# zju3dv/Mirror-NeRF

Hardware: AMD Instinct MI355X
Metric: rendered rays/sec (primary+reflected) (higher is better)
Workload: dtype f32 carried as hi/lo f16 pairs (f16 MFMA, f32 accumulate; max |diff| to the fp32 chain 3e-6)

## Files before the change

### include/mnrf.h

```cpp
#ifndef MNRF_H
#define MNRF_H

#include <stdint.h>

#ifdef __cplusplus
extern "C" {
#endif

#define MNRF_HOST

#define MNRF_OK 0
#define MNRF_ERR_ARG (-1)
#define MNRF_ERR_LAUNCH (-2)
#define MNRF_ERR_UNSUPPORTED (-3)

#define MNRF_N_PARAMS 32

#define MNRF_SIGMA_ONLY 1u
#define MNRF_GRAD_NORMAL 2u
#define MNRF_SPLIT_F16 4u

#define MNRF_TCNN_GRAD_F16 16u
#define MNRF_TCNN_GRAD_FIXED 512u
#define MNRF_TCNN_F16 256u
// ... 69 lines not shown
int mnrf_object_rays(const float* rays, int64_t n_rays, MNRF_HOST const float* pose, float scale, float tx, float ty, float tz,
                     float* out, void* stream);

int mnrf_object_merge(const float* obj_rgb, const float* obj_depth, const float* obj_opacity, int64_t n_rays, float scale,
                      float pose_scale0, float near, float* rgb, float* depth, float* mask, int32_t* n_used, void* stream);

#define MNRF_OBJECT_MAX_RES 1024

int mnrf_occupancy_bits(const float* volume, int Rx, int Ry, int Rz, float sigma_min, int dilate, uint32_t* bits,
                        int32_t* n_set, void* stream);

int mnrf_object_cull(const float* rays, int64_t n_rays, MNRF_HOST const float* pose, float scale, float tx, float ty, float tz,
                     MNRF_HOST const float* box_lo, MNRF_HOST const float* box_hi, int Rx, int Ry, int Rz, const uint32_t* bits,
                     float* out_rays, int32_t* index, int32_t* count, void* stream);

int mnrf_object_merge_indexed(const float* obj_rgb, const float* obj_depth, const float* obj_opacity, const int32_t* index,
                              const int32_t* count, int64_t capacity, float scale, float pose_scale0, float near, float* rgb,
                              float* depth, float* mask, int32_t* n_used, void* stream);

int mnrf_composite_backward(const float* rays, int64_t n_rays, int S, const float* sigma, const float* z_vals,
                            const float* noise, const float* rgb, const float* is_mirror,
                            const float* pred_normal, const float* normal, int white_back,
                            const float* weights, const float* depth,
                            const float* g_weights, const float* g_opacity, const float* g_rgb_map,
                            const float* g_depth, const float* g_mirror_mask, const float* g_surf_normal,
                            const float* g_surf_normal_grad, const float* g_normal_dif, const float* g_x_surface,
                            float* d_sigma, float* d_rgb, float* d_is_mirror, float* d_pred_normal,
                            float* d_normal, float* d_rays,
                            int detach ,
                            const float* keep_mirror ,
                            void* stream);

int mnrf_ray_grads(const float* d_xyz, const float* z_vals, const float* d_dir, int64_t n_rays, int spr, float* g_rays,
                   float* g_de, void* stream);

int mnrf_reflect_backward(const float* rays, const float* normal, const int32_t* index, int64_t n_sec,
                          const float* g_sec, int64_t n_rays, float* g_x_surface, float* g_normal, float* g_rays,
                          void* stream);
int mnrf_blend_backward(const float* g_out, const float* mask, const int32_t* index, int64_t n_sec, int64_t n, int c,
                        float* g_base, float* g_sec, void* stream);
int mnrf_embed_backward(const float* x, const float* g_out, int64_t n, int c, int n_freqs, float* g_x, void* stream);

int64_t mnrf_train_save_floats(int64_t B);
int64_t mnrf_train_mask_words(int64_t B);
int64_t mnrf_train_workspace_floats(int64_t B);

int mnrf_field_forward_train(float* packed, int64_t B, const float* xyz, int64_t xyz_stride,
                             const float* rays, const float* z_vals, int spr, const float* dir_emb,
                             int64_t dir_stride, float* sigma, float* rgb, float* pred_normal,
                             float* is_mirror, float* normal, float* save_x, uint64_t* save_mask,
                             float* save_inv, float* save_invj, unsigned flags , void* stream);

int mnrf_field_backward(float* packed, int64_t B, const float* xyz, int64_t xyz_stride,
                        const float* rays, const float* z_vals, int spr,
                        const float* g_sigma, const float* g_rgb, const float* g_pred_normal,
                        const float* g_is_mirror, const float* rgb, const float* pred_normal,
                        const float* is_mirror, const float* save_x, const uint64_t* save_mask,
                        const float* save_inv, float* workspace, float* const* d_params, float* d_xyz,
                        float* d_dir,
                        const float* keep_mirror ,
                        unsigned flags ,
                        void* stream);

int64_t mnrf_train_workspace2_floats(int64_t B);
int mnrf_field_backward2(float* packed, int64_t B, const float* xyz, int64_t xyz_stride,
                         const float* rays, const float* z_vals, int spr, const float* g_normal,
                         const float* normal, const float* save_invj, const uint64_t* save_mask,
                         float* workspace, float* const* d_params, float* d_xyz, unsigned flags , void* stream);

int mnrf_tcnn_encode(const float* table, MNRF_HOST const int64_t* offsets17_host, double log2_per_level_scale, int base_resolution,
                     float bound, int64_t B, const float* xyz, int64_t xyz_stride, const float* rays, const float* z_vals,
                     int spr, float* planes, void* stream);

int mnrf_tcnn_encode_flags(const float* table, MNRF_HOST const int64_t* offsets17_host, double log2_per_level_scale, int base_resolution,
                           float bound, int64_t B, const float* xyz, int64_t xyz_stride, const float* rays, const float* z_vals,
                           int spr, float* planes, unsigned flags, void* stream);
int mnrf_tcnn_table_half(const float* table, int64_t entries, void* table_half, void* stream);

int mnrf_bench_gather(const void* table, int64_t table_bytes, int bytes_per_gather, int64_t n_threads, int iters, float* out,
                      void* stream);

#define MNRF_FUSED_WHITE_BACK 1u
#define MNRF_FUSED_RGB_DEPTH 2u
int mnrf_fused_samples_per_ray(void);
int mnrf_field_composite_fused(float* packed, int64_t n_rays, const float* rays, const float* z_vals,
                               const float* dir_emb, int64_t dir_stride, int flags,
                               float* weights, float* opacity, float* rgb_map, float* depth, float* mirror_mask,
                               float* surf_normal, float* x_surface, void* stream);

#define MNRF_TRAIN_PLANES 256u
#define MNRF_PLANES_Y_HALF 0x100000u
int64_t mnrf_train_planes_bytes(int64_t B);
int64_t mnrf_train_dy_planes_bytes(int64_t B);

int mnrf_field_backward_planes(float* packed, int64_t B, const float* xyz, int64_t xyz_stride,
                               const float* rays, const float* z_vals, int spr,
                               const float* g_sigma, const float* g_rgb, const float* g_pred_normal,
                               const float* g_is_mirror, const float* rgb, const float* pred_normal,
                               const float* is_mirror, const uint64_t* save_mask, const float* save_inv,
                               void* dy_planes, uint32_t* seedmax, float* d_xyz, float* d_dir, const float* keep_mirror,
                               unsigned flags ,
                               void* stream);

int64_t mnrf_dw_planes_workspace_floats(int n_eval, MNRF_HOST const int64_t* B);
int mnrf_dw_planes(int n_eval, const void* const* x_planes, const void* const* dy_planes, MNRF_HOST const int64_t* B,
                   const uint32_t* const* seedmax, float* workspace, float* const* d_params, int accumulate, void* stream);

int64_t mnrf_train_planes2_bytes(int64_t B);
int64_t mnrf_train_dy_planes2_bytes(int64_t B);
int mnrf_field_backward2_planes(float* packed, int64_t B, const float* xyz, int64_t xyz_stride,
                                const float* rays, const float* z_vals, int spr, const float* g_normal,
                                const float* normal, const float* save_invj, const uint64_t* save_mask,
                                void* x2_planes, void* y2_planes, uint32_t* jmax, float* d_xyz, void* stream);
int64_t mnrf_dw_planes2_workspace_floats(int n_eval, MNRF_HOST const int64_t* B, MNRF_HOST const int* kinds);
int mnrf_dw_planes2(int n_eval, const void* const* x_planes, const void* const* dy_planes, MNRF_HOST const int64_t* B,
                    const uint32_t* const* seedmax, MNRF_HOST const int* kinds, float* workspace, float* const* d_params, int accumulate,
                    void* stream);

int mnrf_adam_step(float* param, const float* grad, float* exp_avg, float* exp_avg_sq, int64_t n, float lr, double beta1,
                   double beta2, float eps, float weight_decay, int64_t step, int32_t* skipped, const float* grad_scale,
                   const float* found_inf, void* stream);

int mnrf_embed_n(const float* x, int64_t n, int c, int n_freqs, float* out, const int32_t* n_live, void* stream);
int mnrf_embed_backward_n(const float* x, const float* g_out, int64_t n, int c, int n_freqs, float* g_x, const int32_t* n_live, void* stream);
int mnrf_sample_coarse_n(const float* rays, int64_t n_rays, const float* z_steps, int n_samples, int use_disp, float perturb,
                         const float* perturb_rand, float* z_vals, const int32_t* n_live, void* stream);
int mnrf_ray_prologue_n(const float* rays, int64_t n_rays, int n_freqs_dir, const float* z_steps, int n_samples, int use_disp,
                        float perturb, const float* perturb_rand, float* dir_emb, float* z_vals, const int32_t* n_live, void* stream);
int mnrf_ray_fan_backward_n(const float* g0, const float* g1, const float* g2, const float* g3, const float* rays,
                            const float* g_dir_a, const float* g_dir_b, int64_t n_rays, int n_freqs_dir, float* g_rays,
                            const int32_t* n_live, void* stream);
int mnrf_composite_n(const float* rays, int64_t n_rays, int S, const float* sigma, const float* z_vals,
                     const float* noise, const float* rgb, const float* is_mirror,
                     const float* pred_normal, const float* normal, int white_back,
                     float* weights, float* opacity, float* rgb_map, float* depth, float* mirror_mask,
                     float* surf_normal, float* surf_normal_grad, float* normal_dif, float* x_surface,
                     const int32_t* n_live, void* stream);
int mnrf_composite_sample_n(const float* rays, int64_t n_rays, int S, const float* sigma, const float* z_vals,
                            const float* noise, const float* rgb, const float* is_mirror,
                            const float* pred_normal, const float* normal, int white_back,
                            float* weights, float* opacity, float* rgb_map, float* depth, float* mirror_mask,
                            float* surf_normal, float* surf_normal_grad, float* normal_dif, float* x_surface,
                            const float* u, int u_per_ray, int n_importance, float* z_fine,
                            const int32_t* n_live, void* stream);
int mnrf_composite_backward_n(const float* rays, int64_t n_rays, int S, const float* sigma, const float* z_vals,
                              const float* noise, const float* rgb, const float* is_mirror,
                              const float* pred_normal, const float* normal, int white_back,
                              const float* weights, const float* depth,
                              const float* g_weights, const float* g_opacity, const float* g_rgb_map,
                              const float* g_depth, const float* g_mirror_mask, const float* g_surf_normal,
                              const float* g_surf_normal_grad, const float* g_normal_dif, const float* g_x_surface,
                              float* d_sigma, float* d_rgb, float* d_is_mirror, float* d_pred_normal,
                              float* d_normal, float* d_rays, int detach, const float* keep_mirror,
                              const int32_t* n_live, void* stream);
int mnrf_sample_fine_n(const float* z_coarse, const float* weights, int64_t n_rays, int S,
                       const float* u, int u_per_ray, int n_importance, float* z_fine, const int32_t* n_live, void* stream);
int mnrf_threshold_mask_n(float* mask, int64_t n, int32_t* any, const int32_t* n_live, void* stream);
int mnrf_reflect_compact_n(const float* rays, const float* x_surface, const float* normal,
                           const float* normal_noise, float noise_std, const float* mask,
                           int64_t n_rays, int compact, float near2, float* sec_rays, int32_t* index,
                           int32_t* count, float* reflect_dir, const int32_t* n_live,
                           int32_t* slot ,
                           void* stream);
int mnrf_reflect_backward_gather_n(const float* rays, const float* normal, const int32_t* slot, const float* g_sec, int64_t n_rays,
                                   float* g_x_surface, float* g_normal, float* g_rays, const int32_t* n_live, void* stream);
int mnrf_blend2_n(const float* base_a, const float* sec_a, const float* base_b, const float* sec_b, const int32_t* slot,
                  const float* mask, int64_t n, int c, float* out_a, float* out_b, const int32_t* n_live, void* stream);
int mnrf_blend2_backward_n(const float* g_out_a, const float* g_out_b, const int32_t* slot, const float* mask, int64_t n, int c,
                           float* g_base_a, float* g_sec_a, float* g_base_b, float* g_sec_b, const int32_t* n_live, void* stream);
int mnrf_blend_scatter_n(const float* base, const float* sec, const int32_t* index, int64_t n_sec,
                         const float* mask, int64_t n, int c, float* out, float* reflect_out,
// ... 218 lines not shown
```

### mirror_nerf_amd/csrc/mnrf_composite.inc

```
struct CompMaps {
    float* weights;
    float* opacity; float* rgb_map; float* depth; float* mirror_mask;
    float* surf_normal; float* surf_normal_grad; float* normal_dif; float* x_surface;
    const float* rays;
    int white_back;
};

template <class Src>
__device__ __forceinline__ void composite_ray(const Src& src, int S, int lane, long long ray, const CompMaps& A) {
    float carry = 1.f;
    float a_op = 0.f, a_d = 0.f, a_m = 0.f, a_nd = 0.f;
    float a_c[3] = {0.f, 0.f, 0.f}, a_n[3] = {0.f, 0.f, 0.f}, a_g[3] = {0.f, 0.f, 0.f};
    for (int base = 0; base < S; base += 64) {
        const int s = base + lane;
        const bool in = s < S;
        float alpha = 0.f, zv = 0.f;
        if (in) {
            zv = src.z(s);
            const float delta = s + 1 < S ? src.z(s + 1) - zv : 1e10f;
            float sv = src.sigma(s);
            if (src.has_noise()) sv = sv + src.noise(s);
            alpha = 1.f - expf(-delta * fmaxf(sv, 0.f));
        }
        const float t = in ? (1.f - alpha) + 1e-10f : 1.f;
        float incl = t;
#pragma unroll
        for (int o = 1; o < 64; o <<= 1) {
            const float up = __shfl_up(incl, o);
            if (lane >= o) incl *= up;
        }
        float excl = __shfl_up(incl, 1);
        if (lane == 0) excl = 1.f;
        const float w = alpha * (carry * excl);
        carry = carry * __shfl(incl, 63);
        if (in) {
            if (A.weights) A.weights[s] = w;
            a_op += w;
            a_d += w * zv;
            if (src.has_rgb()) { a_c[0] += w * src.rgb(s, 0); a_c[1] += w * src.rgb(s, 1); a_c[2] += w * src.rgb(s, 2); }
            if (src.has_mirror()) a_m += w * src.mirror(s);
            float pn[3] = {0.f, 0.f, 0.f}, gn[3] = {0.f, 0.f, 0.f};
            if (src.has_pn()) {
#pragma unroll
                for (int k = 0; k < 3; ++k) { pn[k] = src.pn(s, k); a_n[k] += pn[k] * w; }
            }
            if (src.has_gn()) {
#pragma unroll
                for (int k = 0; k < 3; ++k) { gn[k] = src.gn(s, k); a_g[k] += gn[k] * w; }
            }
            if (src.has_pn() && src.has_gn()) {
                const float d0 = gn[0] - pn[0], d1 = gn[1] - pn[1], d2 = gn[2] - pn[2];
                a_nd += w * (d0 * d0 + d1 * d1 + d2 * d2);
            }
        }
    }
    a_op = wave_sum(a_op);
    a_d = wave_sum(a_d);
    if (src.has_mirror()) a_m = wave_sum(a_m);
    if (src.has_pn() && src.has_gn()) a_nd = wave_sum(a_nd);
#pragma unroll
    for (int k = 0; k < 3; ++k) {
        if (src.has_rgb()) a_c[k] = wave_sum(a_c[k]);
        if (src.has_pn()) a_n[k] = wave_sum(a_n[k]);
        if (src.has_gn()) a_g[k] = wave_sum(a_g[k]);
    }
    if (lane == 0) {
        if (A.opacity) A.opacity[ray] = a_op;
        if (A.rgb_map) {
#pragma unroll
            for (int k = 0; k < 3; ++k) A.rgb_map[ray * 3 + k] = A.white_back ? a_c[k] + (1.f - a_op) : a_c[k];
        }
        if (A.depth) A.depth[ray] = a_d;
        if (A.mirror_mask) A.mirror_mask[ray] = a_m;
        if (A.surf_normal) { for (int k = 0; k < 3; ++k) A.surf_normal[ray * 3 + k] = a_n[k]; }
        if (A.surf_normal_grad) { for (int k = 0; k < 3; ++k) A.surf_normal_grad[ray * 3 + k] = a_g[k]; }
        if (A.normal_dif) A.normal_dif[ray] = a_nd;
        if (A.x_surface) {
            const float* r = A.rays + ray * 8;
            for (int k = 0; k < 3; ++k) A.x_surface[ray * 3 + k] = r[k] + r[3 + k] * a_d;
        }
    }
}
```

### mirror_nerf_amd/csrc/mnrf_field.hip

```cpp
#include <hip/hip_runtime.h>
#include <stdint.h>
#include <stdlib.h>

#include "mnrf_layout.h"
#include "mnrf_field_args.h"

namespace mnrf {

extern __shared__ __attribute__((aligned(16))) char smem[];

namespace s2 {
constexpr int S = 2;
constexpr int MIN_WAVES_PER_SIMD = 1;
constexpr int CHUNK_TILES = 16;
#include "mnrf_field_impl.inc"
#include "mnrf_field_bwd.inc"
}
namespace s1 {
constexpr int S = 1;
constexpr int MIN_WAVES_PER_SIMD = 2;
constexpr int CHUNK_TILES = 16;
#include "mnrf_field_impl.inc"
}

struct PackArgs {
    const float* params[32];
    float* packed;
};
constexpr int PACK_BATCH = 4;
struct PackBatch {
    PackArgs m[PACK_BATCH];
};

__global__ void pack_kernel(PackBatch PB, PartTable T) {
    const PackArgs& P = PB.m[blockIdx.y];
    const long long p = (long long)blockIdx.x * blockDim.x + threadIdx.x;
    if (p < DEVICE_STATE_WORDS) P.packed[OFF_REDUCE_PAIR + p] = 0.f;
    if (p >= PACKED_F32_FLOATS) return;
    float v = 0.f;
    if (p < OFF_BIAS) {
        const int tile = (int)(p / TILE_FLOATS);
        const int within = (int)(p % TILE_FLOATS);
        const int lane = within >> 2, j = within & 3, g = lane >> 4, i = lane & 15;
        int k = 0;
        while (k + 1 < N_FWD_PARTS && T.fwd[k + 1].tile0 <= tile) ++k;
        const Part pt = T.fwd[k];
        const int lt = tile - pt.tile0;
        const int tq = lt / pt.nb, nb = lt % pt.nb;
        const int n = 16 * nb + i;
        const int t = 4 * tq + j;
        int col;
        if (pt.kind == KIND_ENC) col = enc_col(t, g);
        else {
            col = 16 * (t >> 2) + 4 * g + (t & 3);
            if (pt.kind == KIND_DIR && col >= ENC_DIR) col = -1;
        }
        if (tq < pt.ntq && n < pt.n_true && col >= 0) v = P.params[pt.param][(long long)n * pt.ld + pt.col_off + col];
    } else if (p < OFF_BWD) {
        const int b = (int)(p - OFF_BIAS);
        if (b < 2048) v = P.params[2 * (b / 256) + 1][b % 256];
        else if (b < BIAS_FIN) { if (b - BIAS_SIG < 1) v = P.params[21][0]; }
        else if (b < BIAS_DIR) v = P.params[17][b - BIAS_FIN];
        else if (b < BIAS_RGB) v = P.params[19][b - BIAS_DIR];
        else if (b < BIAS_NRM1) { if (b - BIAS_RGB < 3) v = P.params[23][b - BIAS_RGB]; }
        else if (b < BIAS_NRM2) v = P.params[25][b - BIAS_NRM1];
        else if (b < BIAS_MIR1) { if (b - BIAS_NRM2 < 3) v = P.params[27][b - BIAS_NRM2]; }
        else if (b < BIAS_MIR2) v = P.params[29][b - BIAS_MIR1];
        else if (b < BIAS_WSIG) { if (b - BIAS_MIR2 < 1) v = P.params[31][0]; }
        else if (b < BIAS_WSIG + 256) v = P.params[20][b - BIAS_WSIG];
    } else {
        const bool heads = p >= OFF_HBWD;
        const long long q = p - (heads ? OFF_HBWD : OFF_BWD);
        const int tile = (int)(q / TILE_FLOATS);
        const int within = (int)(q % TILE_FLOATS);
        const int lane = within >> 2, j = within & 3, g = lane >> 4, i = lane & 15;
        const Part* parts = heads ? T.hbwd : T.bwd;
        const int nparts = heads ? N_HBWD_PARTS - 1 : N_BWD_PARTS;
        int k = 0;
        while (k + 1 < nparts && parts[k + 1].tile0 <= tile) ++k;
        const Part pt = parts[k];
        const int lt = tile - pt.tile0;
        const int tq = lt / pt.nb, nb = lt % pt.nb;
        const int rho = 16 * nb + i;
        const int c = 16 * tq + 4 * g + j;
// ... 15 lines not shown

#include "../../include/mnrf.h"
#include "mnrf_dw.h"
#include "mnrf_error.h"
#include "mnrf_fill.h"

using namespace mnrf;

extern "C" int64_t mnrf_packed_floats(void) { return PACKED_FLOATS; }

extern "C" int mnrf_pack_weights_n(int n_models, const float* const* params, float* const* packed, void* stream) {
    if (n_models < 0) return mnrf_fail(MNRF_ERR_ARG, "mnrf_pack_weights_n: negative model count");
    if (n_models == 0) return MNRF_OK;
    if (!params || !packed) return mnrf_fail(MNRF_ERR_ARG, "mnrf_pack_weights: null pointer");
    for (int i = 0; i < n_models * MNRF_N_PARAMS; ++i)
        if (!params[i]) return mnrf_fail(MNRF_ERR_ARG, "mnrf_pack_weights: null parameter pointer");
    for (int m = 0; m < n_models; ++m)
        if (!packed[m]) return mnrf_fail(MNRF_ERR_ARG, "mnrf_pack_weights: null image pointer");
    PartTable T;
    build_parts(T);
    const int threads = 256;
    const int blocks = (int)((PACKED_F32_FLOATS + threads - 1) / threads);
    for (int m0 = 0; m0 < n_models; m0 += PACK_BATCH) {
        const int nb = n_models - m0 < PACK_BATCH ? n_models - m0 : PACK_BATCH;
        PackBatch PB{};
        float* images[PACK_BATCH] = {};
        for (int m = 0; m < nb; ++m) {
            for (int i = 0; i < MNRF_N_PARAMS; ++i) PB.m[m].params[i] = params[(m0 + m) * MNRF_N_PARAMS + i];
            PB.m[m].packed = images[m] = packed[m0 + m];
        }
        hipLaunchKernelGGL(pack_kernel, dim3(blocks, nb), dim3(threads), 0, (hipStream_t)stream, PB, T);
        launch_split_pack(images, nb, (hipStream_t)stream);
    }
    return mnrf_check_launch("mnrf_pack_weights");
}

extern "C" int mnrf_fold_weights_n(int n_models, const float* const* params, float* const* packed, void* stream) {
    if (n_models < 0) return mnrf_fail(MNRF_ERR_ARG, "mnrf_fold_weights_n: negative model count");
    if (n_models == 0) return MNRF_OK;
    if (!params || !packed) return mnrf_fail(MNRF_ERR_ARG, "mnrf_fold_weights_n: null pointer");
    for (int i = 0; i < n_models * MNRF_N_PARAMS; ++i)
        if (!params[i]) return mnrf_fail(MNRF_ERR_ARG, "mnrf_fold_weights_n: null parameter pointer");
    for (int m = 0; m < n_models; ++m)
        if (!packed[m]) return mnrf_fail(MNRF_ERR_ARG, "mnrf_fold_weights_n: null image pointer");
    for (int m0 = 0; m0 < n_models; m0 += PACK_BATCH) {
        const int nb = n_models - m0 < PACK_BATCH ? n_models - m0 : PACK_BATCH;
        launch_split_fold(params + m0 * MNRF_N_PARAMS, packed + m0, nb, (hipStream_t)stream);
    }
    return mnrf_check_launch("mnrf_fold_weights");
}

extern "C" int mnrf_pack_weights(const float* const* params, float* packed, void* stream) {
    if (!params || !packed) return mnrf_fail(MNRF_ERR_ARG, "mnrf_pack_weights: null pointer");
    return mnrf_pack_weights_n(1, params, &packed, stream);
}

extern "C" int mnrf_field_forward(float* packed, unsigned flags, int64_t B, const float* xyz,
                                  int64_t xyz_stride, const float* rays, const float* z_vals, int spr,
                                  const float* dir_emb, int64_t dir_stride, float* sigma, float* rgb,
                                  float* pred_normal, float* is_mirror, float* normal, float* geo_feat,
                                  void* stream) {
    if (!packed) return mnrf_fail(MNRF_ERR_ARG, "mnrf_field_forward: packed weights are null");
    if (B < 0) return mnrf_fail(MNRF_ERR_ARG, "mnrf_field_forward: negative sample count");
    if (B == 0) return MNRF_OK;
    const bool sigma_only = flags & MNRF_SIGMA_ONLY;
    const bool grad = flags & MNRF_GRAD_NORMAL;
    if (!xyz && (!rays || !z_vals)) return mnrf_fail(MNRF_ERR_ARG, "mnrf_field_forward: need xyz or rays+z_vals");
    if (xyz && xyz_stride < 3) return mnrf_fail(MNRF_ERR_ARG, "mnrf_field_forward: xyz_stride < 3");
    if (spr < 1) return mnrf_fail(MNRF_ERR_ARG, "mnrf_field_forward: samples per ray must be >= 1");
    if (!xyz && B % spr != 0) return mnrf_fail(MNRF_ERR_ARG, "mnrf_field_forward: B not a multiple of spr");
    if (!sigma_only && !dir_emb) return mnrf_fail(MNRF_ERR_ARG, "mnrf_field_forward: dir_emb required unless SIGMA_ONLY");
    if (grad && !normal) return mnrf_fail(MNRF_ERR_ARG, "mnrf_field_forward: GRAD_NORMAL needs the normal output");
    FieldArgs A{packed, flags, (long long)B, xyz, (long long)xyz_stride, rays, z_vals, spr, dir_emb,
                (long long)dir_stride, sigma, rgb, pred_normal, is_mirror, normal, geo_feat};
    const int rc = (flags & MNRF_SPLIT_F16) ? launch_split(A, sigma_only, grad, (hipStream_t)stream)
                 : grad ? s1::launch(A, sigma_only, grad, (hipStream_t)stream)
                        : s2::launch(A, sigma_only, grad, (hipStream_t)stream);
    if (rc != 0) return mnrf_fail(MNRF_ERR_ARG, "mnrf_field_forward: too many samples for one launch");
    return mnrf_check_launch("mnrf_field_forward");
}

extern "C" int mnrf_fused_samples_per_ray(void) { return split48_ray_samples(); }

extern "C" int mnrf_field_composite_fused(float* packed, int64_t n_rays, const float* rays, const float* z_vals,
                                          const float* dir_emb, int64_t dir_stride, int flags,
                                          float* weights, float* opacity, float* rgb_map, float* depth, float* mirror_mask,
                                          float* surf_normal, float* x_surface, void* stream) {
    if (!packed || !rays || !z_vals || !dir_emb) return mnrf_fail(MNRF_ERR_ARG, "mnrf_field_composite_fused: null pointer");
    if (n_rays < 0) return mnrf_fail(MNRF_ERR_ARG, "mnrf_field_composite_fused: negative ray count");
    if (flags & ~(int)(MNRF_FUSED_WHITE_BACK | MNRF_FUSED_RGB_DEPTH)) return mnrf_fail(MNRF_ERR_ARG, "mnrf_field_composite_fused: unknown flag bits");
    const bool rgb_depth = flags & MNRF_FUSED_RGB_DEPTH;
    if (rgb_depth && (mirror_mask || surf_normal))
        return mnrf_fail(MNRF_ERR_ARG, "mnrf_field_composite_fused: MNRF_FUSED_RGB_DEPTH evaluates neither the mirror head nor the normal map");
    if (n_rays == 0) return MNRF_OK;
    if (!split48_enabled())
        return mnrf_fail(MNRF_ERR_UNSUPPORTED, "mnrf_field_composite_fused: needs the 48-samples-per-wave tuning (MNRF_SPLIT48 != 0)");
    const int spr = split48_ray_samples();
    FieldArgs A{packed, MNRF_SPLIT_F16, (long long)n_rays * spr, nullptr, 3, rays, z_vals, spr, dir_emb, (long long)dir_stride,
                nullptr, nullptr, nullptr, nullptr, nullptr, nullptr};
    A.fuse = rgb_depth ? 2 : 1;
    A.white_back = (flags & MNRF_FUSED_WHITE_BACK) != 0;
    A.f_weights = weights; A.f_opacity = opacity; A.f_rgb_map = rgb_map; A.f_depth = depth; A.f_mirror_mask = mirror_mask;
    A.f_surf_normal = surf_normal; A.f_x_surface = x_surface;
    if (launch_split48(A, false, (hipStream_t)stream) != 0)
        return mnrf_fail(MNRF_ERR_ARG, "mnrf_field_composite_fused: too many samples for one launch");
    return mnrf_check_launch("mnrf_field_composite_fused");
}

static inline int64_t train_tiles(int64_t B) { return (B + s2::WG_SAMPLES - 1) / s2::WG_SAMPLES; }

extern "C" int64_t mnrf_train_save_floats(int64_t B) { return (int64_t)SAVE_FLOATS * B; }
extern "C" int64_t mnrf_train_mask_words(int64_t B) { return train_tiles(B) * N_MASKS * s2::S * s2::WG_THREADS; }
extern "C" int64_t mnrf_train_workspace_floats(int64_t B) { return (int64_t)DY_FLOATS * B + dw_workspace_floats(B); }

static int field_forward_train_impl(float* packed, int64_t B, const float* xyz, int64_t xyz_stride,
                                    const float* rays, const float* z_vals, int spr, const float* dir_emb,
                                    int64_t dir_stride, float* sigma, float* rgb, float* pred_normal,
                                    float* is_mirror, float* normal, float* save_x, uint64_t* save_mask,
                                    float* save_inv, float* save_invj, unsigned flags, const int32_t* n_live, void* stream) {
    if (n_live && !(flags & MNRF_TRAIN_PLANES))
        return mnrf_fail(MNRF_ERR_UNSUPPORTED, "mnrf_field_forward_train_n: a live row count needs MNRF_TRAIN_PLANES (the fp32-row layout depends on B)");
    if (!packed || !save_x || !save_mask || !save_inv) return mnrf_fail(MNRF_ERR_ARG, "mnrf_field_forward_train: null pointer");
    const bool planes = flags & MNRF_TRAIN_PLANES;
    if (planes && !(flags & MNRF_SPLIT_F16))
        return mnrf_fail(MNRF_ERR_ARG, "mnrf_field_forward_train: MNRF_TRAIN_PLANES needs MNRF_SPLIT_F16 (the planes are the split kernel's operands)");
    if (B <= 0) return B == 0 ? MNRF_OK : mnrf_fail(MNRF_ERR_ARG, "mnrf_field_forward_train: negative sample count");
    if (!xyz && (!rays || !z_vals)) return mnrf_fail(MNRF_ERR_ARG, "mnrf_field_forward_train: need xyz or rays+z_vals");
    if (spr < 1 || !dir_emb) return mnrf_fail(MNRF_ERR_ARG, "mnrf_field_forward_train: bad spr / dir_emb");
    if (!sigma || !rgb || !pred_normal || !is_mirror)
        return mnrf_fail(MNRF_ERR_ARG, "mnrf_field_forward_train: the four head outputs are required (the backward reads them)");
    FieldArgs A{packed, MNRF_GRAD_NORMAL, (long long)B, xyz, (long long)xyz_stride, rays, z_vals, spr, dir_emb,
                (long long)dir_stride, sigma, rgb, pred_normal, is_mirror, normal, nullptr,
                planes ? nullptr : save_x, (unsigned long long*)save_mask, save_inv, save_invj, planes ? (char*)save_x : nullptr};
    A.n_live = n_live;
    const int rc = (flags & MNRF_SPLIT_F16) ? launch_split(A, false, true, (hipStream_t)stream)
                                            : s2::launch(A, false, true, (hipStream_t)stream);
    if (rc != 0)
        return mnrf_fail(MNRF_ERR_ARG, "mnrf_field_forward_train: too many samples for one launch");
    return mnrf_check_launch("mnrf_field_forward_train");
}
extern "C" int mnrf_field_forward_train(float* packed, int64_t B, const float* xyz, int64_t xyz_stride,
                                        const float* rays, const float* z_vals, int spr, const float* dir_emb,
                                        int64_t dir_stride, float* sigma, float* rgb, float* pred_normal,
                                        float* is_mirror, float* normal, float* save_x, uint64_t* save_mask,
                                        float* save_inv, float* save_invj, unsigned flags, void* stream) {
    return field_forward_train_impl(packed, B, xyz, xyz_stride, rays, z_vals, spr, dir_emb, dir_stride, sigma, rgb, pred_normal, is_mirror,
                                    normal, save_x, save_mask, save_inv, save_invj, flags, nullptr, stream);
}
extern "C" int mnrf_field_forward_train_n(float* packed, int64_t B, const float* xyz, int64_t xyz_stride,
                                          const float* rays, const float* z_vals, int spr, const float* dir_emb,
                                          int64_t dir_stride, float* sigma, float* rgb, float* pred_normal,
                                          float* is_mirror, float* normal, float* save_x, uint64_t* save_mask,
                                          float* save_inv, float* save_invj, unsigned flags, const int32_t* n_live, void* stream) {
    return field_forward_train_impl(packed, B, xyz, xyz_stride, rays, z_vals, spr, dir_emb, dir_stride, sigma, rgb, pred_normal, is_mirror,
                                    normal, save_x, save_mask, save_inv, save_invj, flags, n_live, stream);
}

extern "C" int mnrf_field_backward(float* packed, int64_t B, const float* xyz, int64_t xyz_stride,
                                   const float* rays, const float* z_vals, int spr,
                                   const float* g_sigma, const float* g_rgb, const float* g_pred_normal,
                                   const float* g_is_mirror, const float* rgb, const float* pred_normal,
                                   const float* is_mirror, const float* save_x, const uint64_t* save_mask,
                                   const float* save_inv, float* workspace, float* const* d_params, float* d_xyz,
                                   float* d_dir, const float* keep_mirror, unsigned flags, void* stream) {
    if (!packed || !save_x || !save_mask || !save_inv || !workspace || !d_params)
        return mnrf_fail(MNRF_ERR_ARG, "mnrf_field_backward: null pointer");
    if (B <= 0) return B == 0 ? MNRF_OK : mnrf_fail(MNRF_ERR_ARG, "mnrf_field_backward: negative sample count");
    if (!g_sigma || !g_rgb || !g_pred_normal || !g_is_mirror)
        return mnrf_fail(MNRF_ERR_ARG, "mnrf_field_backward: all four upstream gradients are required (pass zeros)");
    if (!rgb || !pred_normal || !is_mirror) return mnrf_fail(MNRF_ERR_ARG, "mnrf_field_backward: forward outputs missing");
    if (!xyz && (!rays || !z_vals)) return mnrf_fail(MNRF_ERR_ARG, "mnrf_field_backward: need xyz or rays+z_vals");
    for (int i = 0; i < MNRF_N_PARAMS; ++i)
        if (!d_params[i]) return mnrf_fail(MNRF_ERR_ARG, "mnrf_field_backward: null gradient pointer");
    float* dY = workspace;
    float* ws = workspace + (int64_t)DY_FLOATS * B;
    FieldBwdArgs A{packed, (long long)B, xyz, (long long)xyz_stride, rays, z_vals, spr, g_sigma, g_rgb, g_pred_normal,
                       g_is_mirror, rgb, pred_normal, is_mirror, (const unsigned long long*)save_mask, save_inv, dY, d_xyz, d_dir,
                       flags & (MNRF_CUT_NORMAL_HEAD | MNRF_CUT_MIRROR_HEAD), keep_mirror, nullptr, nullptr, 6};
    hipStream_t s = (hipStream_t)stream;
    if (((flags & MNRF_SPLIT_F16) ? launch_split_bwd(A, s) : s2::launch_bwd(A, s)) != 0)
        return mnrf_fail(MNRF_ERR_ARG, "mnrf_field_backward: too many samples for one launch");
    int rc = mnrf_check_launch("mnrf_field_backward (activation gradients)");
    if (rc != MNRF_OK) return rc;
    if (launch_dw(save_x, dY, g_sigma, (long long)B, ws, d_params, (flags & MNRF_DW_ACCUMULATE) ? 1 : 0, s) != 0)
        return mnrf_fail(MNRF_ERR_ARG, "mnrf_field_backward: workspace accounting error");
    return mnrf_check_launch("mnrf_field_backward (weight gradients)");
}

extern "C" int64_t mnrf_train_planes_bytes(int64_t B) { return B <= 0 ? 0 : dwp_sample_blocks(B) * PLX_SB_BYTES; }
// ... 173 lines not shown
```

### mirror_nerf_amd/csrc/mnrf_field_split.hip

```cpp
#include <hip/hip_runtime.h>
#include <stdint.h>
#include <type_traits>
#include <stdlib.h>

#include "mnrf_layout.h"
#include "mnrf_field_args.h"

namespace mnrf {

extern __shared__ __attribute__((aligned(16))) char smem[];

namespace h2 {
constexpr int S = 2;
constexpr int MIN_WAVES_PER_SIMD = 1;
constexpr int CHUNK_PAIRS = 8;
constexpr int RING_SLOTS = 4;
#include "mnrf_field_split.inc"
}
namespace h2x {
constexpr int S = 2;
constexpr int MIN_WAVES_PER_SIMD = 1;
constexpr int CHUNK_PAIRS = 16;
constexpr int RING_SLOTS = 3;
#include "mnrf_field_split.inc"
// ... 14 lines not shown
};
__global__ void split_pack_kernel(SplitPackImages I, PartTable T) {
    float* packed = I.packed[blockIdx.y];
    const long long q = (long long)blockIdx.x * blockDim.x + threadIdx.x;
    constexpr long long FWD_LANES = (long long)SPLIT_FWD_PAIRS * 64;
    constexpr long long BWD_LANES = (long long)SPLIT_BWD_PAIRS * 64;
    constexpr long long HBWD_LANES = (long long)SPLIT_HBWD_PAIRS * 64;
    if (q >= FWD_LANES + BWD_LANES + HBWD_LANES) return;
    const int region = q >= FWD_LANES + BWD_LANES ? 2 : (q >= FWD_LANES ? 1 : 0);
    const bool bwd = region != 0;
    const long long r = q - (region == 2 ? FWD_LANES + BWD_LANES : (region == 1 ? FWD_LANES : 0));
    const int pair = (int)(r >> 6);
    const int lane = (int)(r & 63);
    const Part* parts = region == 2 ? T.hbwd : (region == 1 ? T.bwd : T.fwd);
    int k = 0, half = -1, pair0 = 0;
    if (bwd) {
        const int nparts = region == 2 ? N_HBWD_PARTS - 1 : N_BWD_PARTS;
        for (;;) {
            const int np = (parts[k].ntq + 1) / 2 * parts[k].nb;
            if (k + 1 >= nparts || pair < pair0 + np) break;
            pair0 += np;
            ++k;
        }
    } else {
        const signed char seg_part[27] = {0, 0, 1, 1, 2, 2, 3, 3, 4, 5, 4, 5, 6, 6, 7, 7, 8, 8, 9, 10, 11, 12, 13, 14, 15, 16, 17};
        const signed char seg_half[27] = {0, 1, 0, 1, 0, 1, 0, 1, 0, 0, 1, 1, 0, 1, 0, 1, 0, 1, -1, -1, -1, -1, -1, -1, -1, -1, -1};
        for (int sg = 0;; ++sg) {
            k = seg_part[sg];
            half = seg_half[sg];
            const int np = parts[k].ntq / 2 * (half >= 0 ? 8 : parts[k].nb);
            if (sg + 1 >= 27 || pair < pair0 + np) break;
            pair0 += np;
        }
    }
    const Part pt = parts[k];
    const int lp = pair - pair0;
    const int rows = half >= 0 ? 8 : pt.nb;
    const int Tq = lp / rows, nb = (half >= 0 ? 8 * half : 0) + lp % rows;
    const float* src = packed + (region == 2 ? OFF_HBWD : (region == 1 ? OFF_BWD : OFF_FWD));
    float w[8];
#pragma unroll
    for (int h = 0; h < 2; ++h) {
        f32x4 v = f32x4{0.f, 0.f, 0.f, 0.f};
        if (2 * Tq + h < pt.ntq)
            v = *(const f32x4*)(src + (pt.tile0 + (long long)(2 * Tq + h) * pt.nb + nb) * TILE_FLOATS + lane * 4);
#pragma unroll
        for (int c = 0; c < 4; ++c) w[4 * h + c] = v[c];
    }
    typedef _Float16 h8v __attribute__((ext_vector_type(8)));
    h8v hi, lo;
    bool bad = false;
#pragma unroll
    for (int jj = 0; jj < 8; ++jj) {
        hi[jj] = (_Float16)w[jj];
        lo[jj] = (_Float16)(w[jj] - (float)hi[jj]);
        bad |= !(fabsf(w[jj]) < 65504.f);
    }
    if (bad) atomicOr((unsigned*)(packed + PACKED_FLOATS - 1), MNRF_GUARD_WEIGHT);
    char* dst = (char*)(packed + (region == 2 ? OFF_SPLIT_HBWD : (region == 1 ? OFF_SPLIT_BWD : OFF_SPLIT_FWD))) + (long long)pair * PAIR_BYTES + lane * 16;
    *(h8v*)dst = hi;
    *(h8v*)(dst + PAIR_BYTES / 2) = lo;
}

void launch_split_pack(float* const* packed, int n_images, hipStream_t s) {
    PartTable T;
    build_parts(T);
    SplitPackImages I{};
    for (int m = 0; m < n_images; ++m) I.packed[m] = packed[m];
    const long long n = (long long)(SPLIT_FWD_PAIRS + SPLIT_BWD_PAIRS + SPLIT_HBWD_PAIRS) * 64;
    hipLaunchKernelGGL(split_pack_kernel, dim3((unsigned)((n + 255) / 256), n_images), dim3(256), 0, s, I, T);
}

struct FoldImages {
    float* packed[4];
    const float* wfin[4];
    const float* wdir[4];
    const float* wn1[4];
    const float* wn2[4];
};
__global__ void split_fold_kernel(FoldImages I) {
    float* packed = I.packed[blockIdx.y];
    const long long q = (long long)blockIdx.x * blockDim.x + threadIdx.x;
    constexpr long long FOLD_LANES = (long long)SPLIT_FOLD_PAIRS * 64;
    if (q >= FOLD_LANES + BIAS_FLOATS) return;
    const float* bias = packed + OFF_BIAS;
    if (q >= FOLD_LANES) {
        const int b = (int)(q - FOLD_LANES);
        float v = bias[b];
        if (b > BIAS_SIG && b <= BIAS_SIG + 3) {
            const int i = b - BIAS_SIG - 1;
            const float* w2 = I.wn2[blockIdx.y] + i * 128;
            double a = 0.0;
            for (int k = 0; k < 128; ++k) a = fma((double)w2[k], (double)bias[BIAS_NRM1 + k], a);
            v = (float)(a + (double)bias[BIAS_NRM2 + i]);
        } else if (b >= BIAS_DIR && b < BIAS_DIR + 128) {
            const float* wd = I.wdir[blockIdx.y] + (b - BIAS_DIR) * (W + ENC_DIR);
            double a = 0.0;
            for (int k = 0; k < W; ++k) a = fma((double)wd[k], (double)bias[BIAS_FIN + k], a);
            v = (float)(a + (double)bias[b]);
        }
        packed[OFF_FOLD_BIAS + b] = v;
        return;
    }
    const int pair = (int)(q >> 6);
    const int lane = (int)(q & 63);
    const int row = lane & 15;
    typedef _Float16 h8v __attribute__((ext_vector_type(8)));
    h8v hi, lo;
    for (int j = 0; j < 8; ++j) hi[j] = lo[j] = (_Float16)0.f;
    const int sp = pair < FOLD_POS_DIR ? pair
                 : pair < FOLD_POS_VIEW ? -1
                 : pair < FOLD_POS_MIR1 ? pair + (1296 - FOLD_POS_VIEW)
                 : pair < SPLIT_FOLD_USED ? pair + (1036 - FOLD_POS_MIR1) : -1;
    if (sp >= 0) {
        const char* src = (const char*)(packed + OFF_SPLIT_FWD) + (long long)sp * PAIR_BYTES + lane * 16;
        hi = *(const h8v*)src;
        lo = *(const h8v*)(src + PAIR_BYTES / 2);
    }
    const bool fold_nrm = pair >= 960 && pair < 968 && row >= 1 && row <= 3;
    const bool fold_dir = pair >= FOLD_POS_DIR && pair < FOLD_POS_VIEW;
    if (fold_nrm || fold_dir) {
        const int T = fold_nrm ? pair - 960 : (pair - FOLD_POS_DIR) / 8;
        const int c0 = 32 * T + 4 * (lane >> 4);
        const float* a = fold_nrm ? I.wn2[blockIdx.y] + (row - 1) * 128 : I.wdir[blockIdx.y] + (16 * ((pair - FOLD_POS_DIR) % 8) + row) * (W + ENC_DIR);
        const float* bm = fold_nrm ? I.wn1[blockIdx.y] : I.wfin[blockIdx.y];
        const int K = fold_nrm ? 128 : W;
        double acc[8];
        for (int j = 0; j < 8; ++j) acc[j] = 0.0;
        for (int k = 0; k < K; ++k) {
            const double ak = (double)a[k];
            const float* bk = bm + (long long)k * W + c0;
#pragma unroll
            for (int c = 0; c < 4; ++c) {
                acc[c] = fma(ak, (double)bk[c], acc[c]);
                acc[4 + c] = fma(ak, (double)bk[16 + c], acc[4 + c]);
            }
        }
        bool bad = false;
#pragma unroll
        for (int j = 0; j < 8; ++j) {
            hi[j] = (_Float16)acc[j];
            lo[j] = (_Float16)(acc[j] - (double)hi[j]);
            bad |= !(fabs(acc[j]) < 65504.0);
        }
        if (bad) atomicOr((unsigned*)(packed + PACKED_FLOATS - 1), MNRF_GUARD_WEIGHT);
    }
    char* dst = (char*)(packed + OFF_FOLD_FWD) + (long long)pair * PAIR_BYTES + lane * 16;
    *(h8v*)dst = hi;
    *(h8v*)(dst + PAIR_BYTES / 2) = lo;
}

void launch_split_fold(const float* const* params, float* const* packed, int n_images, hipStream_t s) {
    FoldImages I{};
    for (int m = 0; m < n_images; ++m) {
        const float* const* p = params + m * 32;
        I.packed[m] = packed[m];
        I.wfin[m] = p[16];
        I.wdir[m] = p[18];
        I.wn1[m] = p[24];
        I.wn2[m] = p[26];
    }
    const long long n = (long long)SPLIT_FOLD_PAIRS * 64 + BIAS_FLOATS;
    hipLaunchKernelGGL(split_fold_kernel, dim3((unsigned)((n + 255) / 256), n_images), dim3(256), 0, s, I);
}

}
```

### mirror_nerf_amd/csrc/mnrf_field_split.inc

```
constexpr int CHUNK_BYTES = CHUNK_PAIRS * PAIR_BYTES;
constexpr int WAVES = 4;
constexpr int WG_THREADS = 64 * WAVES;
constexpr int WG_SAMPLES = WAVES * S * 16;
constexpr int PIECES = CHUNK_BYTES / TILE_BYTES / WAVES;
constexpr int U = 2;
constexpr int PF = S == 3 ? 2 : 4;
constexpr int NBUF = PF + U;
typedef unsigned u32x4 __attribute__((ext_vector_type(4)));
typedef unsigned u32x2 __attribute__((ext_vector_type(2)));
typedef _Float16 h2v __attribute__((ext_vector_type(2)));
struct StoreCtx {
    __amdgpu_buffer_rsrc_t rsrc;
    __amdgpu_buffer_rsrc_t rsrc_lo;
    char* base;
    int lane;
    int soff;
    h2v fac[S];
};
__device__ __forceinline__ __amdgpu_buffer_rsrc_t plane_rsrc(char* sample_block) {
    return __builtin_amdgcn_make_buffer_rsrc(sample_block, 0, 0x7fffffff, 0x00020000);
}
static_assert(CHUNK_PAIRS / U == PIECES, "one LDS-DMA piece per wave per unit");
constexpr int LDS_RING = RING_SLOTS * CHUNK_BYTES;
constexpr int LDS_BIAS = LDS_RING;
constexpr int LDS_MASK = LDS_BIAS + BIAS_FLOATS * 4;
constexpr int LDS_PARK = LDS_MASK;
constexpr int HEAD_PARK = 6;
constexpr int LDS_PARK_BYTES = S == 3 ? HEAD_PARK * S * WG_THREADS * 16 : 0;
static_assert(S != 3 || HEAD_PARK * S >= 2 * S * 2, "the encoding operands fit the same region");
constexpr int LDS_TILEQ = LDS_MASK + LDS_PARK_BYTES;
constexpr int LDS_BYTES = LDS_TILEQ + 16;
constexpr int LDS_BYTES_GRAD = LDS_MASK + 8 * S * WG_THREADS * 8;
static_assert(LDS_BYTES_GRAD <= 160 * 1024, "LDS budget");
constexpr int LDS_FUSE = LDS_BYTES;
constexpr int LDS_BYTES_FUSE = LDS_BYTES + 9 * WG_SAMPLES * 4;
static_assert(LDS_BYTES_FUSE <= 160 * 1024, "LDS budget");

#include "mnrf_field_split_common.inc"

__device__ __forceinline__ float wave_sum(float v) {
#pragma unroll
    for (int o = 32; o > 0; o >>= 1) v += __shfl_xor(v, o);
    return v;
}
#include "mnrf_composite.inc"
struct CompLdsSrc {
    const float* f;
    bool pn_on, mir_on;
    __device__ __forceinline__ bool has_noise() const { return false; }
    __device__ __forceinline__ bool has_rgb() const { return true; }
    __device__ __forceinline__ bool has_mirror() const { return mir_on; }
    __device__ __forceinline__ bool has_pn() const { return pn_on; }
    __device__ __forceinline__ bool has_gn() const { return false; }
    __device__ __forceinline__ float z(int s) const { return f[8 * WG_SAMPLES + s]; }
    __device__ __forceinline__ float sigma(int s) const { return f[s]; }
    __device__ __forceinline__ float noise(int) const { return 0.f; }
    __device__ __forceinline__ float rgb(int s, int k) const { return f[(1 + k) * WG_SAMPLES + s]; }
    __device__ __forceinline__ float mirror(int s) const { return f[7 * WG_SAMPLES + s]; }
    __device__ __forceinline__ float pn(int s, int k) const { return f[(4 + k) * WG_SAMPLES + s]; }
    __device__ __forceinline__ float gn(int, int) const { return 0.f; }
};
struct CompLdsSrcRgbDepth : CompLdsSrc {
    __device__ __forceinline__ bool has_mirror() const { return false; }
    __device__ __forceinline__ bool has_pn() const { return false; }
};

__device__ __forceinline__ unsigned long long enc_out_of_range(const float (&x)[S][3]) {
    bool big = false;
#pragma unroll
    for (int s = 0; s < S; ++s) big |= !(fabsf(x[s][0]) < ENC_RANGE_LIMIT && fabsf(x[s][1]) < ENC_RANGE_LIMIT && fabsf(x[s][2]) < ENC_RANGE_LIMIT);
    return __builtin_amdgcn_ballot_w64(big);
}

template <int N>
__device__ __forceinline__ void split_b(const float (&x)[S][N], u32x4 (&hi)[S][N / 8], u32x4 (&lo)[S][N / 8],
                                        unsigned long long& sat, float limit = F16_MAX) {
    float tmax = 0.f;
#pragma unroll
    for (int s = 0; s < S; ++s)
#pragma unroll
        for (int T = 0; T < N / 8; ++T)
#pragma unroll
            for (int e = 0; e < 4; ++e) {
                unsigned h, l;
                split2(x[s][8 * T + 2 * e], x[s][8 * T + 2 * e + 1], h, l);
                sat_track<false>(tmax, x[s][8 * T + 2 * e], x[s][8 * T + 2 * e + 1]);
                hi[s][T][e] = h;
                lo[s][T][e] = l;
            }
    sat_flush(sat, tmax, limit);
}

__device__ __forceinline__ f32x4 mfma_f16(const u32x4& a, const u32x4& b, const f32x4& c) {
    return __builtin_amdgcn_mfma_f32_16x16x32_f16(__builtin_bit_cast(h8, a), __builtin_bit_cast(h8, b), c, 0, 0, 0);
}

__device__ __forceinline__ float relu_(float x) {
    const int i = __builtin_bit_cast(int, x);
    return __builtin_bit_cast(float, i > 0 ? i : 0);
}

constexpr int NTASKS = 16 * S;
template <int ACT, bool WANT_MASK>
__device__ __forceinline__ void conv_task(int q, const f32x4 (&pacc)[S][8], u32x4 (&oh)[S][8], u32x4 (&ol)[S][8],
                                          int t0, int half, uint64_t (&mk)[S], float& tmax) {
    const int trel = q / (4 * S), s = (q / 4) % S, nb = 2 * trel + ((q >> 1) & 1), rp = q & 1;
    const float a0 = pacc[s][nb][2 * rp], a1 = pacc[s][nb][2 * rp + 1];
    if (WANT_MASK) {
        mk[s] |= (uint64_t)(a0 > 0.f) << (4 * (8 * half + nb) + 2 * rp);
        mk[s] |= (uint64_t)(a1 > 0.f) << (4 * (8 * half + nb) + 2 * rp + 1);
    }
    const float v0 = ACT == 1 ? relu_(a0) : a0, v1 = ACT == 1 ? relu_(a1) : a1;
    unsigned h, l;
    split2(v0, v1, h, l);
    sat_track<ACT == 1>(tmax, v0, v1);
    oh[s][t0 + trel][2 * (nb & 1) + rp] = h;
    ol[s][t0 + trel][2 * (nb & 1) + rp] = l;
}

template <int NT, int NB, int NACC, int NTA, int JOB, bool WANT_MASK, int USTART, int TPU, int POS, int NPARK = 0, int STB = -1,
          int STN = 4, bool SSCALE = false>
__device__ __forceinline__ void gemm_part_impl(f32x4 (&acc)[S][NACC], const u32x4 (&bh)[S][NTA], const u32x4 (&bl)[S][NTA],
                                               Stream& st, int wave, int lane16, const f32x4 (&pacc)[S][8],
                                               u32x4 (&oh)[S][8], u32x4 (&ol)[S][8], int t0, int half, uint64_t (&mk)[S],
                                               const StoreCtx& sc = StoreCtx{}) {
    static_assert(STB < 0 || (S == 2 && NT * NB / U >= 8 * STN && STB + STN <= NTA), "8 store tasks per operand ride on the part's first units");
    static_assert(NT <= NTA, "B operand count");
    static_assert(JOB < 0 || NTASKS % TPU == 0, "tasks per unit");
    static_assert(JOB < 0 || USTART + NTASKS / TPU <= NT * NB / U, "the job fits the part");
    constexpr int NPAIRS = NT * NB;
    static_assert(NPAIRS % U == 0, "pairs come in units");
    const unsigned ring = (unsigned)(size_t)(__attribute__((address_space(3))) char*)smem + (unsigned)lane16;
    u32x4 ah[NBUF], al[NBUF];
    constexpr int START = POS % CHUNK_PAIRS;
    static_assert(POS % U == 0, "parts start on a unit");
    static_assert(NPAIRS >= PF, "a part is at least as long as the read-ahead");
    unsigned base = ring + st.rd_slot * CHUNK_BYTES;
#pragma unroll
    for (int i = 0; i < PF; ++i) {
        ah[i] = st.ch[i];
        al[i] = st.cl[i];
    }
    constexpr int NUNITS = NPAIRS / U;
    constexpr int INNER = NUNITS < 16 ? NUNITS : 16;
    static_assert(NUNITS % INNER == 0, "unit count");
    constexpr int NSLOT = NB == 1 ? 4 : 2;
    u32x4 pk[NSLOT][S];
    const u32x4* const park = (const u32x4*)(smem + LDS_PARK + wave * 1024 + lane16);
    const auto park_load = [&](int T) {
#pragma unroll
        for (int s = 0; s < S; ++s) pk[T % NSLOT][s] = park[(T * S + s) * WG_THREADS];
    };
    if (NPARK > 0) {
        park_load(0);
        if (NB == 1 && NT > 1) park_load(1);
    }
#pragma unroll
    for (int uo = 0; uo < NUNITS / INNER; ++uo) {
#pragma unroll
    for (int ui = 0; ui < INNER; ++ui) {
        const int t = (uo * INNER + ui) * U;
        if (NPARK > 0) {
#pragma unroll
            for (int u = 0; u < U; ++u) {
                const int pnext = t + U + u;
                if (pnext < NPAIRS && pnext % NB == 0 && pnext / NB < NPARK) park_load(pnext / NB);
            }
        }
        __builtin_amdgcn_sched_barrier(0);
        const int younger = PF - U;
        u32x4& x0 = ah[t % NBUF];
        u32x4& y0 = al[t % NBUF];
        u32x4& x1 = ah[(t + 1) % NBUF];
        u32x4& y1 = al[(t + 1) % NBUF];
        if (younger == 0) wait_lds_reads_but<0>(x0, y0, x1, y1);
        else if (younger == 1) wait_lds_reads_but<2>(x0, y0, x1, y1);
        else wait_lds_reads_but<4>(x0, y0, x1, y1);
#pragma unroll
        for (int sg = 0; sg < 6; ++sg) {
            const int ph = sg / 2, u = sg % 2;
            const int T = (t + u) / NB, nb = (t + u) % NB;
#pragma unroll
            for (int s = 0; s < S; ++s) {
                const u32x4& a = ph == 1 ? al[(t + u) % NBUF] : ah[(t + u) % NBUF];
                const u32x4& b = ph == 2 ? (T < NPARK ? pk[T % NSLOT][s] : bl[s][T]) : bh[s][T];
                acc[s][nb] = mfma_f16(a, b, acc[s][nb]);
            }
            if (JOB >= 0 && (sg == 0 || sg == 2) && TPU == 2) {
                const int unit = t / U - USTART;
                if (unit >= 0 && unit < NTASKS / TPU) {
                    conv_task<(JOB < 0 ? 0 : JOB), WANT_MASK>(unit * TPU + sg / 2, pacc, oh, ol, t0, half, mk, st.tmax);
#pragma unroll
                    for (int k = 0; k < S; ++k) {
                        __builtin_amdgcn_sched_group_barrier(0x008, 1, 0);
                        __builtin_amdgcn_sched_group_barrier(0x002, 6, 0);
                    }
                }
            } else if (JOB >= 0 && TPU != 2 && sg < TPU) {
                const int unit = t / U - USTART;
                if (unit >= 0 && unit < NTASKS / TPU) {
                    conv_task<(JOB < 0 ? 0 : JOB), WANT_MASK>(unit * TPU + sg, pacc, oh, ol, t0, half, mk, st.tmax);
                    static_assert(JOB < 0 || TPU == 2 || TPU == 3 || TPU == 4 || TPU == 6, "one task behind each of the first TPU sub-groups");
                }
            }
            if (STB >= 0 && sg == 5 && t / U < 8 * STN) {
                const int k = t / U;
                const int T = (STB < 0 ? 0 : STB) + k / 8, h = (k / 4) & 1, sgp = (k / 2) & 1;
                const u32x4& w = (k & 1) ? bl[sgp][T < NTA ? T : 0] : bh[sgp][T < NTA ? T : 0];
                __builtin_amdgcn_sched_barrier(0);
                unsigned w0 = w[2 * h], w1 = w[2 * h + 1];
                if (SSCALE) {
                    w0 = __builtin_bit_cast(unsigned, __builtin_bit_cast(h2v, w0) * sc.fac[sgp]);
                    w1 = __builtin_bit_cast(unsigned, __builtin_bit_cast(h2v, w1) * sc.fac[sgp]);
                }
                __builtin_amdgcn_raw_buffer_store_b64(u32x2{w0, w1}, (k & 1) ? sc.rsrc_lo : sc.rsrc, sc.lane,
                                                      sc.soff + ((2 * (T - (STB < 0 ? 0 : STB)) + h) * PL_FB_BYTES + (k & 1) * PL_TILE_BYTES + sgp * 512), PL_STORE_AUX);
                __builtin_amdgcn_sched_barrier(0);
            }
            if (sg < 5) {
                __builtin_amdgcn_sched_barrier(0);
                if (sg < 4) {
                    const int r = t + PF + sg / 2;
                    if (sg % 2 == 0 && (START + r) % CHUNK_PAIRS == 0) {
                        constexpr int Y = PIECES - PF / U;
                        const int lu = t / U;
                        const int hi_u = lu < 8 * STN ? lu : 8 * STN, lo_u = lu - Y - 1 > 0 ? lu - Y - 1 : 0;
                        const int nst = STB >= 0 && hi_u > lo_u ? hi_u - lo_u : 0;
                        if (nst == 0) seam<Y>(st);
                        else if (nst == 1) seam<Y + 1>(st);
                        else if (nst == 2) seam<Y + 2>(st);
                        else if (nst == 3) seam<Y + 3>(st);
                        else if (nst == 4) seam<Y + 4>(st);
                        else if (nst == 5) seam<Y + 5>(st);
                        else if (nst == 6) seam<Y + 6>(st);
                        else if (nst == 7) seam<Y + 7>(st);
                        else seam<Y + 7>(st);
                        static_assert(PIECES - PF / U + 1 <= 7, "store tasks younger than a chunk");
                        base = ring + st.rd_slot * CHUNK_BYTES;
                    }
                    u32x4& d_ = sg % 2 == 0 ? (r < NPAIRS ? ah[r % NBUF] : st.ch[(r - NPAIRS) % PF])
                                            : (r < NPAIRS ? al[r % NBUF] : st.cl[(r - NPAIRS) % PF]);
                    lds_read_half_tile(d_, base, ((START + r) % CHUNK_PAIRS) * PAIR_BYTES + (sg % 2) * TILE_BYTES);
                } else {
                    const int piece = ((POS + t) / U) % PIECES;
                    if (piece == 0) issue_piece<0>(st);
                    else if (piece == 1) issue_piece<1>(st);
                    else if (piece == 2) issue_piece<2>(st);
                    else if (piece == 3) issue_piece<3>(st);
                    else if (piece == 4) issue_piece<(PIECES == 8 ? 4 : 0)>(st);
                    else if (piece == 5) issue_piece<(PIECES == 8 ? 5 : 0)>(st);
                    else if (piece == 6) issue_piece<(PIECES == 8 ? 6 : 0)>(st);
                    else issue_piece<(PIECES == 8 ? 7 : 0)>(st);
                }
                __builtin_amdgcn_sched_barrier(0);
            }
        }
    }
    }
    carry_wait(st, std::integral_constant<int, PF>{});
    if (JOB >= 0) sat_flush(st.sat, st.tmax);
}

template <int NT, int NB, int POS, int NPARK = 0, int STB = -1, int STN = 4, bool SSCALE = false, int NACC, int NTA>
__device__ __forceinline__ void gemm_part(f32x4 (&acc)[S][NACC], const u32x4 (&bh)[S][NTA], const u32x4 (&bl)[S][NTA],
                                          Stream& st, int wave, int lane16, const StoreCtx& sc = StoreCtx{}) {
    f32x4 pacc[S][8];
    u32x4 oh[S][8], ol[S][8];
    uint64_t mk[S];
    gemm_part_impl<NT, NB, NACC, NTA, -1, false, 0, S, POS, NPARK, STB, STN, SSCALE>(acc, bh, bl, st, wave, lane16, pacc, oh, ol, 0, 0,
                                                                                      mk, sc);
}

template <int NT, int NTA, bool WANT_MASK, int USTART, int TPU, int POS, int STB = -1>
__device__ __forceinline__ void gemm_half(f32x4 (&acc)[S][8], const u32x4 (&bh)[S][NTA], const u32x4 (&bl)[S][NTA], Stream& st,
                                          int wave, int lane16, const f32x4 (&pacc)[S][8], u32x4 (&hh)[S][8], u32x4 (&hl)[S][8],
                                          int t0, int half, uint64_t (&mk)[S], const StoreCtx& sc = StoreCtx{}) {
    gemm_part_impl<NT, 8, 8, NTA, 1, WANT_MASK, USTART, TPU, POS, 0, STB>(acc, bh, bl, st, wave, lane16, pacc, hh, hl, t0, half, mk, sc);
}

template <bool WANT_MASK>
__device__ __forceinline__ void conv_half(const f32x4 (&pacc)[S][8], u32x4 (&hh)[S][8], u32x4 (&hl)[S][8], int t0, int half,
                                          uint64_t (&mk)[S], unsigned long long& sat) {
    float tmax = 0.f;
#pragma unroll
    for (int q = 0; q < NTASKS; ++q) conv_task<1, WANT_MASK>(q, pacc, hh, hl, t0, half, mk, tmax);
    sat_flush(sat, tmax);
}

__device__ __forceinline__ void init_bias_half(f32x4 (&acc)[S][8], int bias_off, int half, int g) {
    const f32x4* bl = (const f32x4*)(smem + LDS_BIAS) + (bias_off >> 2) + 32 * half;
#pragma unroll
    for (int nb = 0; nb < 8; ++nb) {
        const f32x4 v = bl[nb * 4 + g];
#pragma unroll
        for (int s = 0; s < S; ++s) acc[s][nb] = v;
    }
}

__device__ __forceinline__ void store_mask(const uint64_t (&mk)[S], int layer, int tid, unsigned long long* gmask) {
#pragma unroll
    for (int s = 0; s < S; ++s) {
        ((uint64_t*)(smem + LDS_MASK))[(layer * S + s) * WG_THREADS + tid] = mk[s];
        if (gmask) gmask[(layer * S + s) * WG_THREADS + tid] = mk[s];
    }
}

__device__ __forceinline__ void out_store(float* p, float v) {
    *p = v;
}

__device__ __forceinline__ void row_store(f32x4* p, const f32x4 v) {
    __builtin_nontemporal_store(v, p);
}

template <int NT>
__device__ __forceinline__ void save_bform(float* sec, int width, const float (&x)[S][NT], const int (&idx)[S],
                                           const bool (&valid)[S], int g) {
#pragma unroll
    for (int s = 0; s < S; ++s) {
        if (!valid[s]) continue;
        f32x4* o = (f32x4*)(sec + (long long)idx[s] * width);
#pragma unroll
        for (int nb = 0; nb < NT / 4; ++nb)
            row_store(o + nb * 4 + g, f32x4{x[s][4 * nb], x[s][4 * nb + 1], x[s][4 * nb + 2], x[s][4 * nb + 3]});
    }
}

template <int NB, int ACT>
__device__ __forceinline__ void save_acc(float* sec, int width, int nb0, const f32x4 (&acc)[S][NB], const int (&idx)[S],
                                         const bool (&valid)[S], int g, uint64_t (&bits)[S]) {
#pragma unroll
    for (int s = 0; s < S; ++s) {
        uint64_t m = 0;
        f32x4* o = (f32x4*)(sec + (long long)idx[s] * width);
#pragma unroll
        for (int nb = 0; nb < NB; ++nb) {
            f32x4 v;
#pragma unroll
            for (int r = 0; r < 4; ++r) {
                const float a = acc[s][nb][r];
                m |= (uint64_t)(a > 0.f) << (4 * nb + r);
                v[r] = ACT == 1 ? relu_(a) : (ACT == 2 ? (a > 0.f ? a : 0.01f * a) : a);
            }
            if (valid[s]) row_store(o + (nb0 + nb) * 4 + g, v);
        }
        bits[s] = m;
    }
}

template <int NT, int NTA>
__device__ __forceinline__ void store_planes(const StoreCtx& sc, int fb0, const u32x4 (&hi)[S][NTA], const u32x4 (&lo)[S][NTA]) {
    static_assert(S == 2, "a sample block is one wave of two 16-sample groups");
#pragma unroll
    for (int T = 0; T < NT; ++T)
#pragma unroll
        for (int h = 0; h < 2; ++h)
#pragma unroll
            for (int s = 0; s < S; ++s) {
                const int off = (fb0 + 2 * T + h) * PL_FB_BYTES + s * 512;
                __builtin_amdgcn_raw_buffer_store_b64(u32x2{hi[s][T][2 * h], hi[s][T][2 * h + 1]}, sc.rsrc, sc.lane, off, PL_STORE_AUX);
                __builtin_amdgcn_raw_buffer_store_b64(u32x2{lo[s][T][2 * h], lo[s][T][2 * h + 1]}, sc.rsrc_lo, sc.lane, off + PL_TILE_BYTES, PL_STORE_AUX);
            }
}

template <int NB>
__device__ __forceinline__ void store_sign_mask(const f32x4 (&acc)[S][NB], unsigned long long* dst) {
#pragma unroll
    for (int s = 0; s < S; ++s) {
        uint64_t m = 0;
#pragma unroll
        for (int nb = 0; nb < NB; ++nb)
#pragma unroll
            for (int r = 0; r < 4; ++r) m |= (uint64_t)(acc[s][nb][r] > 0.f) << (4 * nb + r);
        dst[s * WG_THREADS] = m;
    }
}

template <int NB, int NACC>
__device__ __forceinline__ void init_bias(f32x4 (&acc)[S][NACC], int bias_off, int g) {
    const f32x4* bl = (const f32x4*)(smem + LDS_BIAS) + (bias_off >> 2);
#pragma unroll
    for (int nb = 0; nb < NB; ++nb) {
        const f32x4 v = bl[nb * 4 + g];
#pragma unroll
        for (int s = 0; s < S; ++s) acc[s][nb] = v;
    }
}

template <int NB, int NACC>
__device__ __forceinline__ void zero_acc(f32x4 (&acc)[S][NACC]) {
#pragma unroll
    for (int nb = 0; nb < NB; ++nb)
#pragma unroll
        for (int s = 0; s < S; ++s) acc[s][nb] = f32x4{0.f, 0.f, 0.f, 0.f};
}

template <int NB, int ACT, bool WANT_MASK>
__device__ __forceinline__ void acc_to_b(u32x4 (&hi)[S][NB / 2], u32x4 (&lo)[S][NB / 2], const f32x4 (&acc)[S][NB],
                                         int layer, int tid, unsigned long long& sat) {
    float tmax = 0.f;
#pragma unroll
    for (int s = 0; s < S; ++s) {
        uint64_t m = 0;
#pragma unroll
        for (int nb = 0; nb < NB; ++nb) {
            float v[4];
#pragma unroll
            for (int r = 0; r < 4; ++r) {
                const float a = acc[s][nb][r];
                if (WANT_MASK) m |= (uint64_t)(a > 0.f) << (4 * nb + r);
                v[r] = ACT == 1 ? relu_(a) : (ACT == 2 ? (a > 0.f ? a : 0.01f * a) : a);
            }
            unsigned h0, l0, h1, l1;
            split2(v[0], v[1], h0, l0);
            split2(v[2], v[3], h1, l1);
            sat_track<ACT == 1>(tmax, v[0], v[1]);
            sat_track<ACT == 1>(tmax, v[2], v[3]);
            hi[s][nb >> 1][2 * (nb & 1)] = h0;
            hi[s][nb >> 1][2 * (nb & 1) + 1] = h1;
            lo[s][nb >> 1][2 * (nb & 1)] = l0;
            lo[s][nb >> 1][2 * (nb & 1) + 1] = l1;
        }
        if (WANT_MASK) ((uint64_t*)(smem + LDS_MASK))[(layer * S + s) * WG_THREADS + tid] = m;
    }
    sat_flush(sat, tmax);
}

__device__ __forceinline__ float sigmoidf_(float x) { return 1.f / (1.f + expf(-x)); }



template <bool SIGMA_ONLY, bool GRAD, bool PLANES, bool FUSE, bool RGB_DEPTH>
__device__ __forceinline__ void field_split_body(FieldArgs A) {
    static_assert(!PLANES || (GRAD && !SIGMA_ONLY && S == 2), "operand planes: the training forward (32 samples per wave)");
    static_assert(!FUSE || (S == 3 && !SIGMA_ONLY && !GRAD), "ray-fused compositing: the 192-sample fine pass");
    static_assert(!RGB_DEPTH || FUSE, "rgb / depth only: a variant of the ray-fused pass");
    constexpr bool FOLD = !SIGMA_ONLY && !GRAD;
    float* const fz = (float*)(smem + LDS_FUSE);
    constexpr bool PERSIST = S == 3;
    if constexpr (PLANES) {
        if (A.n_live) {
            long long bl = (long long)*A.n_live * A.spr;
            bl = bl < 0 ? 0 : bl;
            if (bl < A.B) A.B = bl;
        }
        if ((long long)blockIdx.x * WG_SAMPLES >= A.B) return;
    }
    const bool queued = PERSIST && A.tile_queue != nullptr;
    const int wave = __builtin_amdgcn_readfirstlane(threadIdx.x >> 6);
    int tile = blockIdx.x;
    int round = 0;
    unsigned long long sat_all = 0, enc_all = 0;
    {
        const f32x4* src = (const f32x4*)(A.packed + (FOLD ? OFF_FOLD_BIAS : OFF_BIAS));
        f32x4* dst = (f32x4*)(smem + LDS_BIAS);
        for (int i = threadIdx.x; i < BIAS_FLOATS / 4; i += WG_THREADS) dst[i] = src[i];
    }
    for (;;) {
    int lane_;
    if (PERSIST) asm volatile("v_mbcnt_lo_u32_b32 %0, -1, 0\n\tv_mbcnt_hi_u32_b32 %0, -1, %0" : "=v"(lane_));
    else lane_ = threadIdx.x & 63;
    const int lane = lane_;
    const int tid = PERSIST ? wave * 64 + lane : (int)threadIdx.x;
    const int g = lane >> 4;
    const int m = lane & 15;
    const int lane16 = lane * 16;
    constexpr int HP = (S == 3 && !SIGMA_ONLY && !GRAD) ? HEAD_PARK : 0;
    char* const pl = (PLANES || (GRAD && S == 2 && A.save_planes))
                         ? A.save_planes + ((long long)blockIdx.x * WAVES + wave) * PLX_SB_BYTES : nullptr;
    constexpr bool WEAVE = PLANES;
    constexpr int ST0 = WEAVE ? 0 : -1, ST4 = WEAVE ? 4 : -1;
    StoreCtx sc;
    sc.rsrc = plane_rsrc(pl);
    sc.rsrc_lo = sc.rsrc;
    sc.base = pl;
    sc.lane = 32 * m + 8 * g;
    sc.soff = 0;
    const auto at_h = [&](int sec, int T0) -> const StoreCtx& {
        sc.soff = (SEC_H / 16 + 16 * sec + 2 * T0) * PL_FB_BYTES;
        return sc;
    };

    Stream st;
    st.sat = 0;
    st.tmax = 0.f;
    open_stream<true>(st, A.packed + (FOLD ? OFF_FOLD_FWD : OFF_SPLIT_FWD), wave, lane);
    int next_tile = 0;
    if (queued && tid == 0) next_tile = (int)gridDim.x + atomicAdd(A.tile_queue, 1);

    int idx[S];
    bool valid[S];
#pragma unroll
    for (int s = 0; s < S; ++s) {
        long long i = (long long)tile * WG_SAMPLES + wave * (S * 16) + s * 16 + m;
        valid[s] = i < A.B;
        if (!valid[s]) i = A.B - 1;
        idx[s] = (int)i;
    }
    const auto m15 = [&]() -> unsigned {
        unsigned r;
        asm volatile("v_mbcnt_lo_u32_b32 %0, -1, 0\n\tv_mbcnt_hi_u32_b32 %0, -1, %0\n\tv_and_b32 %0, 15, %0" : "=v"(r));
        return r;
    };
    const auto gq = [&]() -> int {
        if (S != 3) return g;
        unsigned r;
        asm volatile("v_mbcnt_lo_u32_b32 %0, -1, 0\n\tv_mbcnt_hi_u32_b32 %0, -1, %0\n\tv_lshrrev_b32 %0, 4, %0" : "=v"(r));
        return (int)r;
    };
    const auto sidx = [&](int s) -> int {
        if (S != 3) return idx[s];
        const unsigned i = tile * (unsigned)WG_SAMPLES + (unsigned)(wave * (S * 16) + s * 16) + m15();
        const unsigned last = (unsigned)A.B - 1u;
        return (int)(i < last ? i : last);
    };
    const auto sval = [&](int s) -> bool {
        if (S != 3) return valid[s];
        return tile * (unsigned)WG_SAMPLES + (unsigned)(wave * (S * 16) + s * 16) + m15() < (unsigned)A.B;
    };
// ... 66 lines not shown
                }
        }
    }
    unsigned long long* gmask = (GRAD && A.save_mask) ? A.save_mask + (long long)tile * (N_MASKS * S * WG_THREADS) : nullptr;
    const bool keep = !PLANES && GRAD && A.save_x != nullptr;
    uint64_t unused_bits[S];

    u32x4 hh[S][8], hl[S][8];
    f32x4 accA[S][8], accB[S][8];
    {
        uint64_t mk[S];
        const auto zero_mask = [&]() {
#pragma unroll
            for (int s = 0; s < S; ++s) mk[s] = 0;
        };
        __syncthreads();
        prime_stream(st, lane16);
        zero_mask();
        init_bias_half(accA, BIAS_L, 0, gq());
        gemm_part<2, 8, 0>(accA, eh, el, st, wave, lane16);
        if (keep) save_acc<8, 1>(A.save_x + (long long)SEC_H * A.B, 256, 0, accA, idx, valid, g, unused_bits);
        init_bias_half(accB, BIAS_L, 1, gq());
        gemm_half<2, 2, GRAD, 0, 2 * S, 16>(accB, eh, el, st, wave, lane16, accA, hh, hl, 0, 0, mk);
        if (keep) save_acc<8, 1>(A.save_x + (long long)SEC_H * A.B, 256, 8, accB, idx, valid, g, unused_bits);
#pragma unroll 1
        for (int l = 0; l < 3; ++l) {
            init_bias_half(accA, BIAS_L + 256 * (1 + l), 0, gq());
            gemm_half<8, 8, GRAD, 0, S, 32, ST0>(accA, hh, hl, st, wave, lane16, accB, hh, hl, 4, 1, mk, at_h(l, 0));
            if (GRAD) { store_mask(mk, l, tid, gmask); zero_mask(); }
            if (keep) save_acc<8, 1>(A.save_x + (long long)(SEC_H + 256 * (1 + l)) * A.B, 256, 0, accA, idx, valid, g, unused_bits);
            if constexpr (S == 2 && !WEAVE) { if (pl) store_planes<8, 8>(sc, SEC_H / 16 + 16 * l, hh, hl); }
            init_bias_half(accB, BIAS_L + 256 * (1 + l), 1, gq());
            gemm_half<8, 8, GRAD, 4, S, 96, ST4>(accB, hh, hl, st, wave, lane16, accA, hh, hl, 0, 0, mk, at_h(l, 4));
            if (keep) save_acc<8, 1>(A.save_x + (long long)(SEC_H + 256 * (1 + l)) * A.B, 256, 8, accB, idx, valid, g, unused_bits);
        }
        init_bias_half(accA, BIAS_L + 256 * 4, 0, gq());
        if (S == 3) {
#pragma unroll
            for (int T = 0; T < 2; ++T) {
                u32x4 ph[S][1], pl[S][1];
                const u32x4* park = (const u32x4*)(smem + LDS_PARK);
#pragma unroll
                for (int s = 0; s < S; ++s) {
                    ph[s][0] = park[((T * S + s) * 2 + 0) * WG_THREADS + tid];
                    pl[s][0] = park[((T * S + s) * 2 + 1) * WG_THREADS + tid];
                }
                if (T == 0) gemm_part<1, 8, 416>(accA, ph, pl, st, wave, lane16);
                else gemm_part<1, 8, 424>(accA, ph, pl, st, wave, lane16);
            }
        } else {
            gemm_part<2, 8, 416>(accA, eh, el, st, wave, lane16);
        }
        gemm_half<8, 8, GRAD, 0, S, 432, ST0>(accA, hh, hl, st, wave, lane16, accB, hh, hl, 4, 1, mk, at_h(3, 0));
        if (GRAD) { store_mask(mk, 3, tid, gmask); zero_mask(); }
        if (keep) save_acc<8, 1>(A.save_x + (long long)(SEC_H + 256 * 4) * A.B, 256, 0, accA, idx, valid, g, unused_bits);
        if constexpr (S == 2 && !WEAVE) { if (pl) store_planes<8, 8>(sc, SEC_H / 16 + 16 * 3, hh, hl); }
        init_bias_half(accB, BIAS_L + 256 * 4, 1, gq());
        if (S == 3) {
#pragma unroll
            for (int T = 0; T < 2; ++T) {
                u32x4 ph[S][1], pl[S][1];
                const u32x4* park = (const u32x4*)(smem + LDS_PARK);
#pragma unroll
                for (int s = 0; s < S; ++s) {
                    ph[s][0] = park[((T * S + s) * 2 + 0) * WG_THREADS + tid];
                    pl[s][0] = park[((T * S + s) * 2 + 1) * WG_THREADS + tid];
                }
                if (T == 0) gemm_part<1, 8, 496>(accB, ph, pl, st, wave, lane16);
                else gemm_part<1, 8, 504>(accB, ph, pl, st, wave, lane16);
            }
        } else {
            gemm_part<2, 8, 496>(accB, eh, el, st, wave, lane16);
        }
        gemm_half<8, 8, GRAD, 4, S, 512, ST4>(accB, hh, hl, st, wave, lane16, accA, hh, hl, 0, 0, mk, at_h(3, 4));
        if (keep) save_acc<8, 1>(A.save_x + (long long)(SEC_H + 256 * 4) * A.B, 256, 8, accB, idx, valid, g, unused_bits);
#pragma unroll 1
        for (int l = 0; l < 3; ++l) {
            init_bias_half(accA, BIAS_L + 256 * (5 + l), 0, gq());
            gemm_half<8, 8, GRAD, 0, S, 576, ST0>(accA, hh, hl, st, wave, lane16, accB, hh, hl, 4, 1, mk, at_h(4 + l, 0));
            if (GRAD) { store_mask(mk, 4 + l, tid, gmask); zero_mask(); }
            if (keep) save_acc<8, 1>(A.save_x + (long long)(SEC_H + 256 * (5 + l)) * A.B, 256, 0, accA, idx, valid, g, unused_bits);
            if constexpr (S == 2 && !WEAVE) { if (pl) store_planes<8, 8>(sc, SEC_H / 16 + 16 * (4 + l), hh, hl); }
            init_bias_half(accB, BIAS_L + 256 * (5 + l), 1, gq());
            gemm_half<8, 8, GRAD, 4, S, 640, ST4>(accB, hh, hl, st, wave, lane16, accA, hh, hl, 0, 0, mk, at_h(4 + l, 4));
            if (keep) save_acc<8, 1>(A.save_x + (long long)(SEC_H + 256 * (5 + l)) * A.B, 256, 8, accB, idx, valid, g, unused_bits);
        }
        conv_half<GRAD>(accB, hh, hl, 4, 1, mk, st.sat);
        if constexpr (S == 2 && !WEAVE) { if (pl) store_planes<8, 8>(sc, SEC_H / 16 + 16 * 7, hh, hl); }
        if (HP > 0) {
            u32x4* park = (u32x4*)(smem + LDS_PARK);
#pragma unroll
            for (int T = 0; T < HP; ++T)
#pragma unroll
                for (int s = 0; s < S; ++s) park[(T * S + s) * WG_THREADS + tid] = hl[s][T];
        }
        if (GRAD) store_mask(mk, 7, tid, gmask);
        if (S != 3 && A.geo_feat) {
#pragma unroll
            for (int s = 0; s < S; ++s) {
                if (valid[s]) {
                    f32x4* o = (f32x4*)(A.geo_feat + (long long)idx[s] * 256);
#pragma unroll
                    for (int nb = 0; nb < 16; ++nb) {
                        const f32x4 v = nb < 8 ? accA[s][nb & 7] : accB[s][nb & 7];
                        o[nb * 4 + g] = f32x4{fmaxf(v[0], 0.f), fmaxf(v[1], 0.f), fmaxf(v[2], 0.f), fmaxf(v[3], 0.f)};
                    }
                }
            }
        }
    }
    const auto put_normal = [&](const f32x4 (&acc)[S][1], auto r0) {
        constexpr int R0 = decltype(r0)::value;
        if (FUSE) {
            if (gq() == 0) {
#pragma unroll
                for (int s = 0; s < S; ++s) {
                    const float a0 = acc[s][0][R0], a1 = acc[s][0][R0 + 1], a2 = acc[s][0][R0 + 2];
                    const float inv = 1.f / sqrtf(fmaxf(a0 * a0 + a1 * a1 + a2 * a2, 1.1920928955078125e-07f));
                    const int q = wave * (S * 16) + s * 16 + (int)m15();
                    fz[4 * WG_SAMPLES + q] = a0 * inv; fz[5 * WG_SAMPLES + q] = a1 * inv; fz[6 * WG_SAMPLES + q] = a2 * inv;
                }
            }
        } else if (A.pred_normal && g == 0) {
#pragma unroll
            for (int s = 0; s < S; ++s)
                if (sval(s)) {
                    const float a0 = acc[s][0][R0], a1 = acc[s][0][R0 + 1], a2 = acc[s][0][R0 + 2];
                    const float inv = 1.f / sqrtf(fmaxf(a0 * a0 + a1 * a1 + a2 * a2, 1.1920928955078125e-07f));
                    float* o = A.pred_normal + (long long)sidx(s) * 3;
                    out_store(o, a0 * inv); out_store(o + 1, a1 * inv); out_store(o + 2, a2 * inv);
                    if (GRAD && A.save_inv)
                        A.save_inv[idx[s]] = (a0 * a0 + a1 * a1 + a2 * a2) > 1.1920928955078125e-07f ? inv : -inv;
                }
        }
    };
    {
        f32x4 acc[S][1];
        init_bias<1>(acc, BIAS_SIG, gq());
        gemm_part<8, 1, 960, HP>(acc, hh, hl, st, wave, lane16);
        if (FUSE) {
            if (gq() == 0) {
#pragma unroll
                for (int s = 0; s < S; ++s) fz[wave * (S * 16) + s * 16 + m15()] = acc[s][0][0];
            }
        } else if (A.sigma && g == 0) {
#pragma unroll
            for (int s = 0; s < S; ++s)
                if (sval(s)) out_store(A.sigma + sidx(s), acc[s][0][0]);
        }
        if constexpr (FOLD && !RGB_DEPTH) put_normal(acc, std::integral_constant<int, 1>{});
    }

    if (!SIGMA_ONLY) {
        if constexpr (!FOLD) {
            u32x4 nh[S][4], nl[S][4];
            {
                f32x4 acc[S][8];
                init_bias<8>(acc, BIAS_NRM1, gq());
                gemm_part<8, 8, 968, HP, ST0>(acc, hh, hl, st, wave, lane16, at_h(7, 0));
                if (keep) save_acc<8, 0>(A.save_x + (long long)SEC_HN * A.B, 128, 0, acc, idx, valid, g, unused_bits);
                acc_to_b<8, 0, false>(nh, nl, acc, 0, tid, st.sat);
                if constexpr (S == 2) { if (pl) store_planes<4, 4>(sc, SEC_HN / 16, nh, nl); }
            }
            f32x4 acc[S][1];
            init_bias<1>(acc, BIAS_NRM2, gq());
            gemm_part<4, 1, 1032>(acc, nh, nl, st, wave, lane16);
            put_normal(acc, std::integral_constant<int, 0>{});
        }
        const auto mirror_head = [&]() {
            u32x4 mh[S][4], ml[S][4];
            {
                f32x4 acc[S][8];
                init_bias<8>(acc, BIAS_MIR1, gq());
                gemm_part<8, 8, FOLD ? FOLD_POS_MIR1 : 1036, HP, ST4>(acc, hh, hl, st, wave, lane16, at_h(7, 4));
                if (keep) {
                    uint64_t bits[S];
                    save_acc<8, 2>(A.save_x + (long long)SEC_HM * A.B, 128, 0, acc, idx, valid, g, bits);
#pragma unroll
                    for (int s = 0; s < S; ++s) gmask[(9 * S + s) * WG_THREADS + tid] = bits[s];
                } else if (GRAD && pl) {
                    store_sign_mask<8>(acc, gmask + (9 * S) * WG_THREADS + tid);
                }
                acc_to_b<8, 2, false>(mh, ml, acc, 0, tid, st.sat);
                if constexpr (S == 2) { if (pl) store_planes<4, 4>(sc, SEC_HM / 16, mh, ml); }
            }
            f32x4 acc[S][1];
            init_bias<1>(acc, BIAS_MIR2, gq());
            gemm_part<4, 1, FOLD ? FOLD_POS_MIR2 : 1100>(acc, mh, ml, st, wave, lane16);
            if (FUSE) {
                if (gq() == 0) {
#pragma unroll
                    for (int s = 0; s < S; ++s) fz[7 * WG_SAMPLES + wave * (S * 16) + s * 16 + m15()] = sigmoidf_(acc[s][0][0]);
                }
            } else if (A.is_mirror && g == 0) {
#pragma unroll
                for (int s = 0; s < S; ++s)
                    if (sval(s)) out_store(A.is_mirror + sidx(s), sigmoidf_(acc[s][0][0]));
            }
        };
        if constexpr (!FOLD) mirror_head();
        const auto view_operands = [&](u32x4 (&vh)[S][1], u32x4 (&vl)[S][1]) {
            float de[S][8];
            const int gv = gq();
            const int spr = opaque_spr();
#pragma unroll
            for (int s = 0; s < S; ++s) {
                const float* dp = A.dir_emb + (long long)(sidx(s) / spr) * A.dir_stride;
#pragma unroll
                for (int t = 0; t < 8; ++t) {
                    const int e = 16 * (t >> 2) + 4 * gv + (t & 3);
                    de[s][t] = e < ENC_DIR ? dp[e] : 0.f;
                }
            }
            if (keep) save_bform<8>(A.save_x + (long long)SEC_DIRE * A.B, 32, de, idx, valid, g);
            split_b<8>(de, vh, vl, st.sat);
            if constexpr (S == 2) { if (pl) store_planes<1, 1>(sc, SEC_DIRE / 16, vh, vl); }
        };
        {
            u32x4 dh[S][4], dl[S][4];
            if constexpr (FOLD) {
                u32x4 vh[S][1], vl[S][1];
                view_operands(vh, vl);
                f32x4 acc[S][8];
                init_bias<8>(acc, BIAS_DIR, gq());
                gemm_part<8, 8, FOLD_POS_DIR, HP>(acc, hh, hl, st, wave, lane16);
                gemm_part<1, 8, FOLD_POS_VIEW>(acc, vh, vl, st, wave, lane16);
                acc_to_b<8, 1, false>(dh, dl, acc, 0, tid, st.sat);
            } else {
                u32x4 fh[S][8], fl[S][8];
                {
                    f32x4 acc[S][16];
                    init_bias<16>(acc, BIAS_FIN, gq());
                    gemm_part<8, 16, 1104, HP>(acc, hh, hl, st, wave, lane16);
                    if (keep) save_acc<16, 0>(A.save_x + (long long)SEC_FIN * A.B, 256, 0, acc, idx, valid, g, unused_bits);
                    acc_to_b<16, 0, false>(fh, fl, acc, 0, tid, st.sat);
                    if constexpr (S == 2) { if (pl) store_planes<8, 8>(sc, SEC_FIN / 16, fh, fl); }
                }
                u32x4 vh[S][1], vl[S][1];
                view_operands(vh, vl);
                f32x4 acc[S][8];
                init_bias<8>(acc, BIAS_DIR, gq());
                gemm_part<8, 8, 1232>(acc, fh, fl, st, wave, lane16);
                gemm_part<1, 8, 1296>(acc, vh, vl, st, wave, lane16);
                if (keep) {
                    uint64_t bits[S];
                    save_acc<8, 1>(A.save_x + (long long)SEC_HD * A.B, 128, 0, acc, idx, valid, g, bits);
#pragma unroll
                    for (int s = 0; s < S; ++s) gmask[(8 * S + s) * WG_THREADS + tid] = bits[s];
                } else if (GRAD && pl) {
                    store_sign_mask<8>(acc, gmask + (8 * S) * WG_THREADS + tid);
                }
                acc_to_b<8, 1, false>(dh, dl, acc, 0, tid, st.sat);
                if constexpr (S == 2) { if (pl) store_planes<4, 4>(sc, SEC_HD / 16, dh, dl); }
            }
            f32x4 acc[S][1];
            init_bias<1>(acc, BIAS_RGB, gq());
            gemm_part<4, 1, FOLD ? FOLD_POS_RGB : 1304>(acc, dh, dl, st, wave, lane16);
            if (FUSE) {
                if (gq() == 0) {
#pragma unroll
                    for (int s = 0; s < S; ++s) {
                        const int q = wave * (S * 16) + s * 16 + (int)m15();
                        fz[1 * WG_SAMPLES + q] = sigmoidf_(acc[s][0][0]);
                        fz[2 * WG_SAMPLES + q] = sigmoidf_(acc[s][0][1]);
                        fz[3 * WG_SAMPLES + q] = sigmoidf_(acc[s][0][2]);
                    }
                }
            } else if (A.rgb && g == 0) {
#pragma unroll
                for (int s = 0; s < S; ++s)
                    if (sval(s)) {
                        float* o = A.rgb + (long long)sidx(s) * 3;
                        out_store(o, sigmoidf_(acc[s][0][0]));
                        out_store(o + 1, sigmoidf_(acc[s][0][1]));
                        out_store(o + 2, sigmoidf_(acc[s][0][2]));
                    }
            }
        }
        if constexpr (FOLD && !RGB_DEPTH) mirror_head();
    }

    if (GRAD) {
        open_stream<false>(st, A.packed + OFF_SPLIT_BWD, wave, lane);
        prime_stream(st, lane16);
        float gr[S][64];
        {
            const f32x4* ws = (const f32x4*)(smem + LDS_BIAS) + (BIAS_WSIG >> 2);
#pragma unroll
            for (int nb = 0; nb < 16; ++nb) {
                const f32x4 v = ws[nb * 4 + g];
#pragma unroll
                for (int s = 0; s < S; ++s)
#pragma unroll
                    for (int r = 0; r < 4; ++r) gr[s][4 * nb + r] = v[r];
            }
        }
        float genc[S][16];
#pragma unroll
        for (int s = 0; s < S; ++s)
#pragma unroll
            for (int t = 0; t < 16; ++t) genc[s][t] = 0.f;

#pragma unroll 1
        for (int layer = 7; layer >= 0; --layer) {
            u32x4 gh[S][8], gl[S][8];
#pragma unroll
            for (int s = 0; s < S; ++s) {
                const uint64_t mk = ((const uint64_t*)(smem + LDS_MASK))[(layer * S + s) * WG_THREADS + tid];
#pragma unroll
                for (int t = 0; t < 64; ++t) gr[s][t] = ((mk >> t) & 1ull) ? gr[s][t] : 0.f;
            }
            split_b<64>(gr, gh, gl, st.sat);
            if (layer == 4 || layer == 0) {
                f32x4 acc[S][4];
                zero_acc<4>(acc);
                gemm_part<8, 4, 0>(acc, gh, gl, st, wave, lane16);
#pragma unroll
                for (int s = 0; s < S; ++s)
#pragma unroll
                    for (int nb = 0; nb < 4; ++nb)
#pragma unroll
                        for (int r = 0; r < 4; ++r) genc[s][4 * nb + r] += acc[s][nb][r];
            }
            if (layer != 0) {
                f32x4 acc[S][16];
                zero_acc<16>(acc);
                gemm_part<8, 16, 0>(acc, gh, gl, st, wave, lane16);
#pragma unroll
                for (int s = 0; s < S; ++s)
#pragma unroll
                    for (int nb = 0; nb < 16; ++nb)
#pragma unroll
                        for (int r = 0; r < 4; ++r) gr[s][4 * nb + r] = acc[s][nb][r];
            }
        }
        float x[S][3];
        fetch_positions(x);
#pragma unroll
        for (int s = 0; s < S; ++s) {
            float d0 = 0.f, d1 = 0.f, d2 = 0.f;
#pragma unroll
            for (int pp = 0; pp < 8; ++pp) {
                const int P = 8 * g + pp;
                const int f = P / 3;
                const int a = P - 3 * f;
                const float gs = genc[s][2 * pp], gc = genc[s][2 * pp + 1];
                if (P < 30) {
                    const float xa = a == 0 ? x[s][0] : (a == 1 ? x[s][1] : x[s][2]);
                    float sn, cs;
                    fast_sincos(ldexpf(xa, f), sn, cs);
                    const float c = ldexpf(gs * cs - gc * sn, f);
                    d0 += a == 0 ? c : 0.f;
                    d1 += a == 1 ? c : 0.f;
                    d2 += a == 2 ? c : 0.f;
                } else if (P == 30) {
                    d0 += gs;
                    d1 += gc;
                } else {
                    d2 += gs;
                }
            }
            d0 += __shfl_xor(d0, 16); d1 += __shfl_xor(d1, 16); d2 += __shfl_xor(d2, 16);
            d0 += __shfl_xor(d0, 32); d1 += __shfl_xor(d1, 32); d2 += __shfl_xor(d2, 32);
            if (A.normal && g == 0 && valid[s]) {
                const float n0 = -d0, n1 = -d1, n2 = -d2;
                const float sq = n0 * n0 + n1 * n1 + n2 * n2;
                const float inv = 1.f / sqrtf(fmaxf(sq, 1.1920928955078125e-07f));
                float* o = A.normal + (long long)idx[s] * 3;
                o[0] = n0 * inv; o[1] = n1 * inv; o[2] = n2 * inv;
                if (A.save_invj) A.save_invj[idx[s]] = sq > 1.1920928955078125e-07f ? inv : -inv;
            }
        }
    }
    sat_all |= st.sat;
    enc_all |= enc_range;
    if (FUSE) {
        __syncthreads();
        if (wave == 0) {
            const long long ray = tile;
            int cl;
            asm volatile("v_mbcnt_lo_u32_b32 %0, -1, 0\n\tv_mbcnt_hi_u32_b32 %0, -1, %0" : "=v"(cl));
            if constexpr (RGB_DEPTH) {
                const CompMaps out{A.f_weights ? A.f_weights + ray * WG_SAMPLES : nullptr, A.f_opacity, A.f_rgb_map, A.f_depth, nullptr,
                                   nullptr, nullptr, nullptr, A.f_x_surface, A.rays, A.white_back};
                composite_ray(CompLdsSrcRgbDepth{fz, false, false}, WG_SAMPLES, cl, ray, out);
            } else {
                const CompLdsSrc src{fz, A.f_surf_normal != nullptr, A.f_mirror_mask != nullptr};
                const CompMaps out{A.f_weights ? A.f_weights + ray * WG_SAMPLES : nullptr, A.f_opacity, A.f_rgb_map, A.f_depth, A.f_mirror_mask,
                                   A.f_surf_normal, nullptr, nullptr, A.f_x_surface, A.rays, A.white_back};
                composite_ray(src, WG_SAMPLES, cl, ray, out);
            }
        }
    }
    if (!queued) break;
    close_stream();
    __syncthreads();
    tile = __builtin_amdgcn_readfirstlane(((volatile int*)(smem + LDS_TILEQ))[round & 1]);
    ++round;
    if (tile >= A.n_tiles) break;
    }
    guard_report(A.packed, sat_all, enc_all, MNRF_GUARD_IN_FORWARD);
    close_stream();
    int last_lane;
    asm volatile("v_mbcnt_lo_u32_b32 %0, -1, 0\n\tv_mbcnt_hi_u32_b32 %0, -1, %0" : "=v"(last_lane));
    if (queued && wave == 0 && last_lane == 0) {
        if (atomicAdd(A.tile_queue + 1, 1) == (int)gridDim.x - 1) {
            atomicExch(A.tile_queue, 0);
            atomicExch(A.tile_queue + 1, 0);
        }
    }
}

template <bool SIGMA_ONLY, bool GRAD, bool PLANES = false, bool FUSE = false>
__global__ __launch_bounds__(WG_THREADS, MIN_WAVES_PER_SIMD) void field_split_kernel(FieldArgs A) {
    field_split_body<SIGMA_ONLY, GRAD, PLANES, FUSE, false>(A);
}
template <bool ON = true>
__global__ __launch_bounds__(WG_THREADS, MIN_WAVES_PER_SIMD) void field_split_kernel_rgb_depth(FieldArgs A) {
    field_split_body<false, false, false, ON, ON>(A);
}

template <bool UNUSED = false>
inline int launch(const FieldArgs& A, bool sigma_only, bool grad, hipStream_t s) {
    const long long blocks64 = (A.B + WG_SAMPLES - 1) / WG_SAMPLES;
    if (blocks64 > 0x7fffffff || A.B > 0x7fffffffLL) return -1;
    dim3 grid((unsigned)blocks64);
    const dim3 block(WG_THREADS);
    if (S == 3 && A.tile_queue) {
        if (A.n_tiles != (int)blocks64 || A.resident < 1 || A.resident > A.n_tiles) return -1;
        grid = dim3((unsigned)A.resident);
    }
    if (sigma_only && !grad) hipLaunchKernelGGL((field_split_kernel<true, false>), grid, block, LDS_BYTES, s, A);
    else if (!sigma_only && !grad && S == 3 && A.fuse == 2) {
        if constexpr (S == 3) hipLaunchKernelGGL((field_split_kernel_rgb_depth<>), grid, block, LDS_BYTES_FUSE, s, A);
    } else if (!sigma_only && !grad && S == 3 && A.fuse)
        hipLaunchKernelGGL((field_split_kernel<false, false, false, S == 3>), grid, block, LDS_BYTES_FUSE, s, A);
    else if (!sigma_only && !grad) hipLaunchKernelGGL((field_split_kernel<false, false>), grid, block, LDS_BYTES, s, A);
#ifndef MNRF_SPLIT_NO_GRAD
    else if (sigma_only && grad) hipLaunchKernelGGL((field_split_kernel<true, true>), grid, block, LDS_BYTES_GRAD, s, A);
    else if (S == 2 && A.save_planes) hipLaunchKernelGGL((field_split_kernel<false, true, S == 2>), grid, block, LDS_BYTES_GRAD, s, A);
    else hipLaunchKernelGGL((field_split_kernel<false, true>), grid, block, LDS_BYTES_GRAD, s, A);
#else
    else return -1;
#endif
    return 0;
}
```

### mirror_nerf_amd/csrc/mnrf_field_split3.hip

```cpp
#include <hip/hip_runtime.h>
#include <stdint.h>
#include <type_traits>
#include <stdlib.h>

#include "mnrf_layout.h"
#include "mnrf_field_args.h"

namespace mnrf {

extern __shared__ __attribute__((aligned(16))) char smem[];

namespace h3 {
constexpr int S = 3;
constexpr int MIN_WAVES_PER_SIMD = 1;
constexpr int CHUNK_PAIRS = 8;
constexpr int RING_SLOTS = 4;
#define MNRF_SPLIT_NO_GRAD
#include "mnrf_field_split.inc"
#undef MNRF_SPLIT_NO_GRAD
}

bool split48_enabled() {
    static const bool v = [] { const char* e = getenv("MNRF_SPLIT48"); return !(e && atoi(e) == 0); }();
    return v;
}

namespace {
constexpr int TQ_DEVICES = 64;
int g_resident[TQ_DEVICES];
unsigned g_next_pair = 0;
}

static bool tile_queue_slot(FieldArgs& A) {
    int dev = 0;
    if (hipGetDevice(&dev) != hipSuccess || dev < 0 || dev >= TQ_DEVICES) return false;
    int resident = __atomic_load_n(&g_resident[dev], __ATOMIC_RELAXED);
    if (!resident) {
        if (hipDeviceGetAttribute(&resident, hipDeviceAttributeMultiprocessorCount, dev) != hipSuccess || resident <= 0) return false;
        __atomic_store_n(&g_resident[dev], resident, __ATOMIC_RELAXED);
    }
    const long long tiles = (A.B + h3::WG_SAMPLES - 1) / h3::WG_SAMPLES;
    if (tiles <= resident || tiles > 0x7fffffff) return false;
    A.tile_queue = (int*)(const_cast<float*>(A.packed) + OFF_TILE_QUEUE) + 2 * (__atomic_fetch_add(&g_next_pair, 1u, __ATOMIC_RELAXED) % TQ_PAIRS);
    A.n_tiles = (int)tiles;
    A.resident = resident;
    return true;
}

int launch_split48(const FieldArgs& A0, bool sigma_only, hipStream_t s) {
    FieldArgs A = A0;
    A.tile_queue = nullptr;
    if (tile_queue_slot(A)) {
        if (hipMemsetAsync(A.tile_queue, 0, 2 * sizeof(int), s) != hipSuccess) A.tile_queue = nullptr;
    }
    static const bool once = [] {
        (void)hipFuncSetAttribute((const void*)h3::field_split_kernel<true, false>, hipFuncAttributeMaxDynamicSharedMemorySize, h3::LDS_BYTES);
        (void)hipFuncSetAttribute((const void*)h3::field_split_kernel<false, false>, hipFuncAttributeMaxDynamicSharedMemorySize, h3::LDS_BYTES);
        (void)hipFuncSetAttribute((const void*)h3::field_split_kernel<false, false, false, true>, hipFuncAttributeMaxDynamicSharedMemorySize,
                                   h3::LDS_BYTES_FUSE);
        (void)hipFuncSetAttribute((const void*)h3::field_split_kernel_rgb_depth<>, hipFuncAttributeMaxDynamicSharedMemorySize, h3::LDS_BYTES_FUSE);
        return true;
    }();
    (void)once;
    return h3::launch(A, sigma_only, false, s);
}

int split48_ray_samples() { return h3::WG_SAMPLES; }

}
```

### mirror_nerf_amd/csrc/mnrf_layout.h

```cpp
#pragma once
#include <stdint.h>

namespace mnrf {

constexpr int W = 256;
constexpr int ENC_XYZ = 63;
constexpr int ENC_DIR = 27;
constexpr int NFREQ_XYZ = 10;
constexpr int NFREQ_DIR = 4;

constexpr int TILE_FLOATS = 256;
constexpr int TILE_BYTES = 1024;
constexpr int PAD_TILES = 16;

enum PartKind : int {
    KIND_H = 0,
    KIND_ENC = 1,
    KIND_DIR = 2,
};

__host__ __device__ inline int enc_col(int t, int g) {
    const int P = 8 * g + (t >> 1);
    const int s = t & 1;
    if (P < 30) return 3 + 6 * (P / 3) + 3 * s + (P % 3);
    if (P == 30) return s;
    return s == 0 ? 2 : -1;
}

struct Part {
    int param;
    int n_true;
    int ld;
    int ntq;
    int nb;
    int col_off;
    int kind;
    int tile0;
};

__host__ __device__ constexpr int padded_tiles(int n) { return (n + PAD_TILES - 1) / PAD_TILES * PAD_TILES; }

constexpr int N_FWD_PARTS = 18;
constexpr int N_BWD_PARTS = 9;
constexpr int FWD_TILES_SIGMA = 64 + 3 * 256 + 320 + 3 * 256 + 16;
constexpr int FWD_TILES = FWD_TILES_SIGMA + 128 + 16 + 128 + 16 + 256 + 144 + 16;
constexpr int BWD_TILES = 3 * 256 + 320 + 3 * 256 + 64;

constexpr int BIAS_L = 0;
constexpr int BIAS_SIG = 2048;
constexpr int BIAS_FIN = 2064;
constexpr int BIAS_DIR = 2320;
constexpr int BIAS_RGB = 2448;
constexpr int BIAS_NRM1 = 2464;
constexpr int BIAS_NRM2 = 2592;
constexpr int BIAS_MIR1 = 2608;
constexpr int BIAS_MIR2 = 2736;
constexpr int BIAS_WSIG = 2752;
constexpr int BIAS_FLOATS = 3072;

constexpr int N_HBWD_PARTS = 9;
constexpr int HBWD_TILES = 16 + 128 + 16 + 256 + 16 + 128 + 16 + 128;

constexpr int64_t OFF_FWD = 0;
constexpr int64_t OFF_BIAS = (int64_t)FWD_TILES * TILE_FLOATS;
constexpr int64_t OFF_BWD = OFF_BIAS + BIAS_FLOATS;
constexpr int64_t OFF_HBWD = OFF_BWD + (int64_t)BWD_TILES * TILE_FLOATS;
constexpr int64_t PACKED_F32_FLOATS = OFF_HBWD + (int64_t)HBWD_TILES * TILE_FLOATS;

constexpr int PAIR_BYTES = 2048;
constexpr int SPLIT_END_PAD = 16;
__host__ __device__ constexpr int padded_pairs(int n) { return (n + SPLIT_END_PAD - 1) / SPLIT_END_PAD * SPLIT_END_PAD; }
constexpr int SPLIT_FWD_USED_SIGMA = 960 + 8;
constexpr int SPLIT_FWD_USED = SPLIT_FWD_USED_SIGMA + 64 + 4 + 64 + 4 + 128 + 64 + 8 + 4;
constexpr int SPLIT_FWD_PAIRS = padded_pairs(SPLIT_FWD_USED);
constexpr int SPLIT_BWD_PAIRS = 3 * 128 + 32 + 128 + 3 * 128 + 32;
constexpr int SPLIT_HBWD_PAIRS = padded_pairs(8 + 64 + 8 + 128 + 8 + 64 + 8 + 64);
constexpr int64_t OFF_SPLIT_FWD = PACKED_F32_FLOATS;
constexpr int64_t OFF_SPLIT_BWD = OFF_SPLIT_FWD + (int64_t)SPLIT_FWD_PAIRS * (PAIR_BYTES / 4);
constexpr int64_t OFF_SPLIT_HBWD = OFF_SPLIT_BWD + (int64_t)SPLIT_BWD_PAIRS * (PAIR_BYTES / 4);
constexpr int64_t SPLIT_TAIL_FLOATS = 2 * 16 * (PAIR_BYTES / 4);
constexpr int FOLD_REGION_PAIRS = 1328;
constexpr int FOLD_POS_DIR = 960 + 8;
constexpr int FOLD_POS_VIEW = FOLD_POS_DIR + 64;
constexpr int FOLD_POS_RGB = FOLD_POS_VIEW + 8;
constexpr int FOLD_POS_MIR1 = FOLD_POS_RGB + 4;
constexpr int FOLD_POS_MIR2 = FOLD_POS_MIR1 + 64;
constexpr int SPLIT_FOLD_USED = FOLD_POS_MIR2 + 4;
constexpr int SPLIT_FOLD_PAIRS = padded_pairs(SPLIT_FOLD_USED);
static_assert(SPLIT_FOLD_USED == 960 + 8 + 64 + 4 + 64 + 8 + 4, "the folded stream holds every folded part once");
constexpr int64_t OFF_FOLD_FWD = OFF_SPLIT_HBWD + (int64_t)SPLIT_HBWD_PAIRS * (PAIR_BYTES / 4);
constexpr int64_t OFF_FOLD_BIAS = OFF_FOLD_FWD + (int64_t)SPLIT_FOLD_PAIRS * (PAIR_BYTES / 4) + SPLIT_TAIL_FLOATS;
constexpr int64_t PACKED_FLOATS = OFF_FOLD_FWD + (int64_t)FOLD_REGION_PAIRS * (PAIR_BYTES / 4) + SPLIT_TAIL_FLOATS;
constexpr int TQ_PAIRS = 8;
constexpr int64_t OFF_TILE_QUEUE = PACKED_FLOATS - 1 - 2 * TQ_PAIRS;
constexpr int64_t OFF_REDUCE_PAIR = OFF_TILE_QUEUE - 2;
constexpr int DEVICE_STATE_WORDS = 2 + 2 * TQ_PAIRS + 1;
static_assert(OFF_FOLD_BIAS + BIAS_FLOATS <= OFF_REDUCE_PAIR, "the folded stream, its read-ahead tail and its bias block fit the reserved region");

constexpr int SEC_ENC = 0;
constexpr int SEC_H = 64;
constexpr int SEC_FIN = 2112;
constexpr int SEC_DIRE = 2368;
constexpr int SEC_HD = 2400;
constexpr int SEC_HN = 2528;
constexpr int SEC_HM = 2656;
constexpr int SAVE_FLOATS = 2784;
constexpr int N_MASKS = 10;
constexpr int DY_L = 0;
constexpr int DY_FIN = 2048;
constexpr int DY_DIR = 2304;
constexpr int DY_NRM1 = 2432;
constexpr int DY_MIR1 = 2560;
constexpr int DY_RGB = 2688;
constexpr int DY_NRM2 = 2704;
constexpr int DY_MIR2 = 2720;
constexpr int DY_FLOATS = 2736;
constexpr int TA_ENC = 0;
constexpr int TA_H = 64;
constexpr int BS_L = 2112;
constexpr int SO_FLOATS = 4160;
constexpr int TRUNK_FWD_TILES = 64 + 3 * 256 + 320 + 3 * 256;

static_assert(FWD_TILES % PAD_TILES == 0 && FWD_TILES_SIGMA % PAD_TILES == 0, "chunking");
static_assert(BWD_TILES % PAD_TILES == 0 && HBWD_TILES % PAD_TILES == 0, "chunking");

struct PartTable {
    Part fwd[N_FWD_PARTS];
    Part bwd[N_BWD_PARTS];
    Part hbwd[N_HBWD_PARTS];
};

__host__ __device__ inline void build_parts(PartTable& T) {
    int n = 0, tile = 0;
    auto add = [&](Part* arr, int& cnt, int param, int n_true, int ld, int ntq, int nb, int col_off, int kind) {
        arr[cnt] = Part{param, n_true, ld, ntq, nb, col_off, kind, tile};
        tile += padded_tiles(ntq * nb);
        cnt++;
    };
    add(T.fwd, n, 0, 256, 63, 4, 16, 0, KIND_ENC);
    for (int i = 1; i < 4; ++i) add(T.fwd, n, 2 * i, 256, 256, 16, 16, 0, KIND_H);
    add(T.fwd, n, 8, 256, 319, 4, 16, 0, KIND_ENC);
    add(T.fwd, n, 8, 256, 319, 16, 16, 63, KIND_H);
    for (int i = 5; i < 8; ++i) add(T.fwd, n, 2 * i, 256, 256, 16, 16, 0, KIND_H);
    add(T.fwd, n, 20, 1, 256, 16, 1, 0, KIND_H);
    add(T.fwd, n, 24, 128, 256, 16, 8, 0, KIND_H);
    add(T.fwd, n, 26, 3, 128, 8, 1, 0, KIND_H);
    add(T.fwd, n, 28, 128, 256, 16, 8, 0, KIND_H);
    add(T.fwd, n, 30, 1, 128, 8, 1, 0, KIND_H);
    add(T.fwd, n, 16, 256, 256, 16, 16, 0, KIND_H);
    add(T.fwd, n, 18, 128, 283, 16, 8, 0, KIND_H);
    add(T.fwd, n, 18, 128, 283, 2, 8, 256, KIND_DIR);
    add(T.fwd, n, 22, 3, 128, 8, 1, 0, KIND_H);
    n = 0;
    tile = 0;
    for (int i = 7; i >= 5; --i) add(T.bwd, n, 2 * i, 256, 256, 16, 16, 0, KIND_H);
    add(T.bwd, n, 8, 256, 319, 16, 4, 0, KIND_ENC);
    add(T.bwd, n, 8, 256, 319, 16, 16, ENC_XYZ, KIND_H);
    for (int i = 3; i >= 1; --i) add(T.bwd, n, 2 * i, 256, 256, 16, 16, 0, KIND_H);
    add(T.bwd, n, 0, 256, 63, 16, 4, 0, KIND_ENC);
    n = 0;
    tile = 0;
    add(T.hbwd, n, 22, 3, 128, 1, 8, 0, KIND_H);
    add(T.hbwd, n, 18, 128, 283, 8, 16, 0, KIND_H);
    add(T.hbwd, n, 18, 128, 283, 8, 2, 256, KIND_DIR);
    add(T.hbwd, n, 16, 256, 256, 16, 16, 0, KIND_H);
    add(T.hbwd, n, 26, 3, 128, 1, 8, 0, KIND_H);
    add(T.hbwd, n, 24, 128, 256, 8, 16, 0, KIND_H);
    add(T.hbwd, n, 30, 1, 128, 1, 8, 0, KIND_H);
    add(T.hbwd, n, 28, 128, 256, 8, 16, 0, KIND_H);
}

}
```

### mirror_nerf_amd/csrc/mnrf_render.hip

```cpp
#include <hip/hip_runtime.h>
#include <stdint.h>
#include <stdio.h>
#include <string.h>

#include "../../include/mnrf.h"
#include "mnrf_error.h"
#include "mnrf_fill.h"
#include "mnrf_rays.h"

static thread_local char g_err[512] = "";

int mnrf_fail(int code, const char* msg) {
    snprintf(g_err, sizeof(g_err), "%s", msg);
    return code;
}

int mnrf_check_launch(const char* where) {
    hipError_t e = hipGetLastError();
    if (e != hipSuccess) {
        snprintf(g_err, sizeof(g_err), "%s: %s", where, hipGetErrorString(e));
        return MNRF_ERR_LAUNCH;
    }
    return MNRF_OK;
}

extern "C" const char* mnrf_last_error(void) { return g_err; }
extern "C" int mnrf_version(void) { return 1; }

namespace {

constexpr float EPS32 = 1.1920928955078125e-07f;

__device__ __forceinline__ long long live_rows(long long cap, const int* __restrict__ n_live) {
    if (!n_live) return cap;
    const long long v = *n_live;
    return v < 0 ? 0 : (v < cap ? v : cap);
}

__device__ __forceinline__ float wave_sum(float v) {
#pragma unroll
    for (int o = 32; o > 0; o >>= 1) v += __shfl_xor(v, o);
    return v;
}
#include "mnrf_composite.inc"

__global__ void embed_kernel(const float* __restrict__ x, long long n, int c, int n_freqs, float* __restrict__ out,
                             const int* __restrict__ n_live) {
    const long long i = (long long)blockIdx.x * blockDim.x + threadIdx.x;
    if (i >= live_rows(n, n_live) * c) return;
    const long long row = i / c;
    const int ch = (int)(i % c);
    const int ld = c * (2 * n_freqs + 1);
    const float v = x[i];
    float* o = out + row * ld;
    o[ch] = v;
    for (int f = 0; f < n_freqs; ++f) {
        float s, co;
        sincosf(ldexpf(v, f), &s, &co);
        o[c * (1 + 2 * f) + ch] = s;
        o[c * (2 + 2 * f) + ch] = co;
    }
}

__global__ void sample_coarse_kernel(const float* __restrict__ rays, long long n_rays, const float* __restrict__ z_steps,
                                     int ns, int use_disp, float perturb, const float* __restrict__ prand,
                                     float* __restrict__ z_out, const int* __restrict__ n_live) {
    const long long i = (long long)blockIdx.x * blockDim.x + threadIdx.x;
    if (i >= live_rows(n_rays, n_live) * ns) return;
    const long long r = i / ns;
    const int s = (int)(i % ns);
    const float near = rays[r * 8 + 6], far = rays[r * 8 + 7];
    auto zat = [&](int k) -> float {
        const float t = z_steps[k];
        if (!use_disp) return near * (1.f - t) + far * t;
        return 1.f / (1.f / near * (1.f - t) + 1.f / far * t);
    };
    float z = zat(s);
    if (perturb > 0.f) {
        const float lower = s == 0 ? z : 0.5f * (zat(s - 1) + z);
        const float upper = s == ns - 1 ? z : 0.5f * (z + zat(s + 1));
        z = lower + (upper - lower) * (perturb * prand[i]);
    }
    z_out[i] = z;
}

struct CompArgs {
    const float* rays; long long n_rays; int S;
    const float* sigma; const float* z; const float* noise; const float* rgb; const float* is_mirror;
    const float* pred_normal; const float* normal; int white_back;
    float* weights; float* opacity; float* rgb_map; float* depth; float* mirror_mask;
    float* surf_normal; float* surf_normal_grad; float* normal_dif; float* x_surface;
    const int* n_live;
};

struct CompGlobalSrc {
    const CompArgs& A;
    long long ray;
    __device__ __forceinline__ bool has_noise() const { return A.noise != nullptr; }
    __device__ __forceinline__ bool has_rgb() const { return A.rgb != nullptr; }
    __device__ __forceinline__ bool has_mirror() const { return A.is_mirror != nullptr; }
    __device__ __forceinline__ bool has_pn() const { return A.pred_normal != nullptr; }
    __device__ __forceinline__ bool has_gn() const { return A.normal != nullptr; }
    __device__ __forceinline__ float z(int s) const { return A.z[ray * A.S + s]; }
    __device__ __forceinline__ float sigma(int s) const { return A.sigma[ray * A.S + s]; }
    __device__ __forceinline__ float noise(int s) const { return A.noise[ray * A.S + s]; }
    __device__ __forceinline__ float rgb(int s, int k) const { return A.rgb[(ray * A.S + s) * 3 + k]; }
    __device__ __forceinline__ float mirror(int s) const { return A.is_mirror[ray * A.S + s]; }
    __device__ __forceinline__ float pn(int s, int k) const { return A.pred_normal[(ray * A.S + s) * 3 + k]; }
    __device__ __forceinline__ float gn(int s, int k) const { return A.normal[(ray * A.S + s) * 3 + k]; }
};

__global__ __launch_bounds__(256) void composite_kernel(CompArgs A) {
    const int lane = threadIdx.x & 63;
    const long long ray = (long long)blockIdx.x * 4 + (threadIdx.x >> 6);
    if (ray >= live_rows(A.n_rays, A.n_live)) return;
    const CompGlobalSrc src{A, ray};
    const CompMaps out{A.weights ? A.weights + ray * A.S : nullptr, A.opacity, A.rgb_map, A.depth, A.mirror_mask, A.surf_normal,
                       A.surf_normal_grad, A.normal_dif, A.x_surface, A.rays, A.white_back};
    composite_ray(src, A.S, lane, ray, out);
}


struct CompBwdArgs {
    const float* rays; long long n_rays; int S;
    const float* sigma; const float* z; const float* noise; const float* rgb; const float* is_mirror;
    const float* pred_normal; const float* normal; int white_back;
    const float* depth;
    const float* g_w; const float* g_op; const float* g_rgb; const float* g_depth; const float* g_mask;
    const float* g_sn; const float* g_sng; const float* g_nd; const float* g_xs;
    float* d_sigma; float* d_rgb; float* d_mirror; float* d_pn; float* d_n; float* d_rays;
    int detach;
    const float* keep_mirror;
    const int* n_live;
};
constexpr int CB_MAXB = 4;

__global__ __launch_bounds__(256) void composite_backward_kernel(CompBwdArgs A) {
    const int lane = threadIdx.x & 63;
    const long long ray = (long long)blockIdx.x * 4 + (threadIdx.x >> 6);
    if (ray >= live_rows(A.n_rays, A.n_live)) return;
    const int S = A.S;
    const float* r8 = A.rays ? A.rays + ray * 8 : nullptr;
    float gop = A.g_op ? A.g_op[ray] : 0.f;
    float gc[3] = {0.f, 0.f, 0.f}, gsn[3] = {0.f, 0.f, 0.f}, gsg[3] = {0.f, 0.f, 0.f}, gxs[3] = {0.f, 0.f, 0.f};
    if (A.g_rgb) { for (int k = 0; k < 3; ++k) gc[k] = A.g_rgb[ray * 3 + k]; }
    if (A.g_sn) { for (int k = 0; k < 3; ++k) gsn[k] = A.g_sn[ray * 3 + k]; }
    if (A.g_sng) { for (int k = 0; k < 3; ++k) gsg[k] = A.g_sng[ray * 3 + k]; }
    if (A.g_xs) { for (int k = 0; k < 3; ++k) gxs[k] = A.g_xs[ray * 3 + k]; }
    float gd = A.g_depth ? A.g_depth[ray] : 0.f;
    const float gm = A.g_mask ? A.g_mask[ray] : 0.f;
    const float gnd = A.g_nd ? A.g_nd[ray] : 0.f;
    const bool w_mask = !(A.detach & MNRF_DETACH_W_MASK) && !(A.keep_mirror && A.keep_mirror[ray] == 0.f);
    const bool w_nrm = !(A.detach & MNRF_DETACH_W_NORMAL);
    const float gm_w = w_mask ? gm : 0.f;
    const float gnd_w = w_nrm ? gnd : 0.f;
    float gsn_w[3], gsg_w[3];
    for (int k = 0; k < 3; ++k) { gsn_w[k] = w_nrm ? gsn[k] : 0.f; gsg_w[k] = w_nrm ? gsg[k] : 0.f; }
    if (A.g_xs && r8) gd += gxs[0] * r8[3] + gxs[1] * r8[4] + gxs[2] * r8[5];
    if (A.white_back) gop -= gc[0] + gc[1] + gc[2];
    if (A.d_rays && lane == 0) {
        float* o = A.d_rays + ray * 8;
        const float dep = A.depth ? A.depth[ray] : 0.f;
        for (int k = 0; k < 3; ++k) { o[k] = gxs[k]; o[3 + k] = gxs[k] * dep; }
        o[6] = 0.f; o[7] = 0.f;
    }
    float Tn[CB_MAXB], Gw[CB_MAXB], Gv[CB_MAXB], tv[CB_MAXB], dads[CB_MAXB];
    float carry = 1.f;
#pragma unroll
    for (int blk = 0; blk < CB_MAXB; ++blk) {
        Tn[blk] = 0.f; Gw[blk] = 0.f; Gv[blk] = 0.f; tv[blk] = 1.f; dads[blk] = 0.f;
        if (blk * 64 >= S) continue;
        const int s = blk * 64 + lane;
        const bool in = s < S;
        const long long i1 = ray * S + s, i3 = i1 * 3;
        float alpha = 0.f, G = 0.f, delta = 0.f, sv = 0.f, ex = 1.f;
        float pn[3] = {0.f, 0.f, 0.f}, gn[3] = {0.f, 0.f, 0.f};
        if (in) {
            const float zv = A.z[i1];
            delta = s + 1 < S ? A.z[i1 + 1] - zv : 1e10f;
            sv = A.sigma[i1];
// ... 983 lines not shown
```

### mirror_nerf_amd/recursion.py

```python
import ctypes
import os
from collections import defaultdict
from types import SimpleNamespace

import torch
from torch import nn

from . import _lib
from .mirror_nerf import Embedding, MirrorNeRF
from .dnerf import render_rays_dnerf
from .rendering import render_rays

RAY_FORWARD_OFFSET = 0.1
JITTER_RAYS = 262144

PLACE_MIRROR_PRESETS = {
    "plane_x": (
        ("livingroom", dict(position=0.0, normal=(-1.0, 0.0, 0.0), rect=(-1.0, 1.0, -0.5, 0.5))),
        ("washroom", dict(position=-1.0, normal=(1.0, 0.0, 0.0), rect=(-1.0, 1.0, -1.0, 0.75))),
        ("office", dict(position=1.0, normal=(1.0, 0.0, 0.0), rect=(-1.0, 1.0, -1.0, 0.75))),
        (None, dict(position=-1.0, normal=(1.0, 0.0, 0.0), rect=(-1.0, 1.0, -0.5, 0.5))),
    ),
    "plane_y": (
        ("washroom", dict(position=1.3, normal=(0.0, -1.0, 0.0), rect=(-1.0, 1.0, -1.0, 1.0))),
        ("livingroom", dict(position=1.65, normal=(0.0, -1.0, 0.0), rect=(-0.3, 1.5, -0.5, 1.0))),
        ("office", dict(position=0.0, normal=(0.0, -1.0, 0.0), rect=(-1.0, 1.0, -0.5, 0.5))),
        (None, dict(position=1.0, normal=(0.0, -1.0, 0.0), rect=(-1.0, 1.0, -0.5, 0.5))),
    ),
}
SUBSTITUTION_PRESETS = (
    ("office", dict(rotation=None, scale=1.0, translation=(0.0, 1.0, 0.0))),
    ("market", dict(rotation=((0.0, 1.0, 0.0), (-1.0, 0.0, 0.0), (0.0, 0.0, 1.0)), scale=1.0,
                    translation=(0.0, 0.0, 0.0))),
    (None, dict(rotation=None, scale=1.0, translation=(0.0, 0.0, 0.0))),
)
OBJECT_PRESETS = (
    ("livingroom", dict(pose_align=None, scale=2.0, translation=(0.0, 0.0, 0.0))),
    ("washroom", dict(pose_align=None, scale=2.0, translation=(-0.5, -0.5, 0.0))),
    ("office", dict(pose_align=None, scale=2.0, translation=(0.0, 3.0, 0.5))),
    (None, dict(pose_align=None, scale=1.0, translation=(0.0, 0.0, 0.0))),
)


def _preset(table, root_dir):
    for key, value in table:
        if key is None or key in (root_dir or ""):
            return dict(value)
    raise AssertionError("preset tables end with a default entry")


def resolve_new_mirror(args, new_mirror=None):
    if new_mirror is not None:
        nm = dict(new_mirror)
        missing = {"axis", "position", "normal", "rect"} - set(nm)
        if missing:
            raise ValueError(f"new_mirror needs the keys axis, position, normal, rect (missing: {sorted(missing)})")
        if nm["axis"] not in ("x", "y"):
            raise ValueError(f"new_mirror axis must be 'x' or 'y', not {nm['axis']!r}")
        if len(nm["normal"]) != 3 or len(nm["rect"]) != 4:
            raise ValueError("new_mirror normal has 3 entries and rect 4 (u0, u1, w0, w1)")
        return dict(axis=nm["axis"], position=float(nm["position"]), normal=tuple(float(v) for v in nm["normal"]),
                    rect=tuple(float(v) for v in nm["rect"]))
    plane_pos = getattr(args, "plane_pos", "plane_x")
    if plane_pos not in PLACE_MIRROR_PRESETS:
        raise ValueError(f"args.plane_pos must be 'plane_x' or 'plane_y', not {plane_pos!r}")
    p = _preset(PLACE_MIRROR_PRESETS[plane_pos], getattr(args, "root_dir", ""))
    return dict(axis=plane_pos[-1], **p)


def resolve_substitution(args):
    return _preset(SUBSTITUTION_PRESETS, getattr(args, "root_dir", ""))


def resolve_new_object(args, new_object=None):
    if new_object is not None:
        cfg = dict(new_object)
        missing = {"pose_align", "scale", "translation"} - set(cfg)
        if missing:
            raise ValueError(f"new_object needs the keys pose_align, scale, translation (missing: {sorted(missing)})")
    else:
        cfg = _preset(OBJECT_PRESETS, getattr(args, "root_dir", ""))
    if len(cfg["translation"]) != 3:
        raise ValueError("new_object translation has 3 entries")
    scale = float(cfg["scale"])
    if not scale > 0.0:
        raise ValueError(f"new_object scale must be positive, not {cfg['scale']!r}")
    pose, pose_scale0 = None, 1.0
    if cfg["pose_align"] is not None:
        m = torch.as_tensor(cfg["pose_align"], dtype=torch.float32)
        if tuple(m.shape) not in ((3, 4), (4, 4)):
            raise ValueError(f"new_object pose_align must be None, 3x4 or 4x4, not {tuple(m.shape)}")
        pose = tuple(float(v) for v in m[:3, :4].reshape(-1))
        pose_scale0 = float(torch.norm(m[:3, 0]))
        if not pose_scale0 > 0.0:
            raise ValueError("new_object pose_align: the first column of its 3x3 is zero")
    return dict(pose=pose, scale=scale, translation=tuple(float(v) for v in cfg["translation"]), pose_scale0=pose_scale0)
# ... 426 lines not shown
    def forward(self, rays, extra=dict()):
        out = self._forward(rays, extra)
        from .mirror_nerf import check_guard, release_transient
        if rays.shape[0] and extra.get("_guard", True) and check_guard(self):
            try:
                out = self._forward(rays, extra)
            finally:
                release_transient(self)
        return out

    def _forward(self, rays, extra):
        from .weights import validated
        with validated(self.models.values()):
            return self._forward_chunks(rays, extra)

    def _forward_chunks(self, rays, extra):
        hp = self.hparams
        results = defaultdict(list)
        for i in range(0, rays.shape[0], hp.chunk):
            ex = {k: (v[i:i + hp.chunk] if isinstance(v, torch.Tensor) else v) for k, v in extra.items() if k != "_guard"}
            rc = rays[i:i + hp.chunk].contiguous()
            out = render_rays_chunk_recursively(self.models, self.embeddings, hp, rc, None, 0, ex,
                                                self.white_back, self.train_geometry_stage)
            for k, v in out.items():
                results[k] += [v]
        return {k: (v[0] if len(v) == 1 else torch.cat(v, 0)) for k, v in results.items()}


_COPY_STREAMS, _PINNED = {}, {}


def _copy_stream(device):
    s = _COPY_STREAMS.get(device)
    if s is None:
        s = _COPY_STREAMS[device] = torch.cuda.Stream(device=device)
    return s


def _pinned(key, rows, tail, dtype):
    k = (key, tail, dtype)
    buf = _PINNED.get(k)
    if buf is None or buf.shape[0] < rows:
        buf = _PINNED[k] = torch.empty((rows,) + tail, dtype=dtype).pin_memory()
    return buf


@torch.no_grad()
def batched_inference(models, embeddings, rays, N_samples, N_importance, use_disp, chunk, **kwargs):
    args = kwargs.get("args")
    if isinstance(args, dict):
        args = SimpleNamespace(**args)
    _refuse_apps(args, models, dict(kwargs, _N_importance=N_importance))
    objects = bool(getattr(args, "app_reflect_newly_placed_objects", False))
    obj_xform = resolve_new_object(args, kwargs.get("new_object")) if objects else None
    obj_dnerf = kwargs.get("render_kwargs_test_d_nerf") if objects and getattr(args, "obj_model_type", "d_nerf") == "d_nerf" else None
    obj_models, obj_embeddings = _object_system(kwargs["system_obj"]) if objects and obj_dnerf is None else (None, None)
    frame_time = float(kwargs["frame_time"]) if obj_dnerf is not None else None
    obj_used = kwargs.get("object_used") if objects else None
    obj_bounds = resolve_object_bounds(kwargs, objects, obj_dnerf, frame_time, rays.device)
    if obj_used is not None:
        obj_used.zero_()
    place = bool(getattr(args, "app_place_new_mirror", False))
    subst = bool(getattr(args, "app_reflection_substitution", False))
    plane = resolve_new_mirror(args, kwargs.get("new_mirror")) if place else None
    xform = resolve_substitution(args) if subst else None
    system_sub = kwargs.get("system_substitution") if subst else None
    trace_flag = kwargs.get("trace_secondary_rays", False)
    test_time = kwargs.get("test_time", True)
    white_back = kwargs.get("white_back", False)
    noise_std = kwargs.get("normal_noise_std", 0)
    noise_iter = kwargs.get("_normal_noise")
    if noise_iter is not None and not isinstance(noise_iter, (list, tuple)):
        kwargs = dict(kwargs, _normal_noise=list(noise_iter))
        noise_iter = kwargs["_normal_noise"]
    if noise_iter is not None:
        noise_iter = iter(noise_iter)
    to_cpu = kwargs.get("to_cpu", True)
    maps_only = bool(kwargs.get("maps_only", to_cpu == "maps"))
    rough = getattr(args, "app_control_mirror_roughness", False)
    batch_jitter = kwargs.get("batch_jitter", noise_iter is None)
    one_field = getattr(args, "only_one_field", False)
    fine_epoch = getattr(args, "only_one_field_fine_epoch", 2)
    sel = "fine" if (N_importance > 0 and not one_field) else "coarse"

    def draw(n, dev):
        if noise_iter is not None:
            return next(noise_iter).to(dev).float().contiguous()
        return torch.randn(n, 3, device=dev)

    def stage_a(rays_chunk, level, host_flags=None, slot=0):
        rgb_depth = 1 <= level == args.max_recursive_level and not rough
        r = render_rays(models, embeddings, rays_chunk, N_samples, use_disp, 0, 0, N_importance, chunk,
                        white_back, test_time=test_time,
                        compute_normal=trace_flag and (not args.predict_normal),
                        only_one_field=one_field, only_one_field_fine_epoch=fine_epoch,
                        current_epoch=fine_epoch + 1, _guard=False, _maps_only=maps_only or rgb_depth,
                        _rgb_depth_only=rgb_depth)
        r[f"rgb_{sel}_reflect"] = torch.zeros_like(r[f"rgb_{sel}"])
        r[f"depth_{sel}_reflect"] = torch.zeros_like(r[f"depth_{sel}"])
        if objects:
            _merge_object(r, rays_chunk, obj_xform, args.near, obj_used, render_object, obj_bounds)
        mask = None
        for key in (f"mirror_mask_{sel}", "mirror_mask_fine", "mirror_mask_coarse"):
            if key in r:
                mask = r[key]
                break
        last = level >= args.max_recursive_level or not (trace_flag or place)
        edit = None
        if place and not last:
            edit = lambda flag: _place_mirror(r, rays_chunk, sel, plane, args.near, flag)
        pending, any_mirror = None, False
        if mask is not None:
            if host_flags is not None and not last and rays_chunk.shape[0]:
                pending = _threshold_async(mask, host_flags, slot, edit)
            else:
                any_mirror = _threshold_(mask, want_any=not last, edit=edit)
        return r, rays_chunk, level, mask, any_mirror, pending

    def render_object(obj_rays):
        if obj_dnerf is not None:
            d = obj_rays[:, 3:6]
            batch = torch.cat([obj_rays, torch.full_like(obj_rays[:, :1], frame_time), d / torch.norm(d, dim=-1, keepdim=True)], -1)
            o = render_rays_dnerf(batch, **dict(obj_dnerf, _frame_time=frame_time))
            return {"rgb_fine": o["rgb_map"], "depth_fine": o["depth_map"], "opacity_fine": o["acc_map"]}
        return render_rays(obj_models, obj_embeddings, obj_rays, N_samples, use_disp, 0, 0, N_importance, chunk, white_back,
                           test_time=True, compute_normal=False, _guard=False, _maps_only=True, _rgb_depth_only=True)

    def recurse(rays_chunk, level):
        return stage_b(stage_a(rays_chunk, level))

    def stage_b(state):
        r, rays_chunk, level, mask, any_mirror, pending = state
        if pending is not None:
            any_mirror = _flag_ready(pending)
        N = rays_chunk.shape[0]
        dev = rays_chunk.device
        only_in = not (level < 1)
        trace = bool(mask is not None and any_mirror and (trace_flag or place))
        if level >= args.max_recursive_level:
            trace = False
        if not trace or N == 0:
            return r
        mask = (mask != 0).float()
        normal = _pick_normal(r, sel)
        nn0 = draw(N, dev) if rough else None
        sec, index, rdir = _reflect(rays_chunk, r[f"x_surface_{sel}"], normal, mask, only_in, nn0, noise_std)
        r["reflect_direction"] = rdir
        if sec.shape[0] > 0:
            if subst:
                _transform_rays(sec, xform)
                r2 = render_rays(system_sub.models, system_sub.embeddings, sec.contiguous(), N_samples, use_disp, 0, 0,
                                 N_importance, chunk, white_back, test_time=test_time, compute_normal=False,
                                 only_one_field=one_field, only_one_field_fine_epoch=fine_epoch,
                                 current_epoch=fine_epoch + 1, _guard=False, _maps_only=True, _rgb_depth_only=True)
            else:
                r2 = recurse(sec.contiguous(), level + 1)
            if rough:
                times = args.trace_ray_times
                if batch_jitter and times > 0:
                    mj = max(1, r2[f"rgb_{sel}"].shape[0])
                    g = 0
                    while g < times:
                        n_g = max(1, min(times - g, JITTER_RAYS // mj))
                        secs = [_reflect(rays_chunk, r[f"x_surface_{sel}"], normal, mask, True, draw(N, dev), noise_std,
                                         want_dir=False)[0] for _ in range(n_g)]
                        r3 = recurse(torch.cat(secs, 0).contiguous(), level + 1)
                        for typ in ("coarse", "fine"):
                            if f"rgb_{typ}" in r2:
                                for piece in r3[f"rgb_{typ}"].view(n_g, -1, 3).unbind(0):
                                    r2[f"rgb_{typ}"] = r2[f"rgb_{typ}"] + piece
                        g += n_g
                else:
                    for _ in range(times):
                        s2, _, _ = _reflect(rays_chunk, r[f"x_surface_{sel}"], normal, mask, True, draw(N, dev),
                                            noise_std, want_dir=False)
                        r3 = recurse(s2.contiguous(), level + 1)
                        for typ in ("coarse", "fine"):
                            if f"rgb_{typ}" in r2:
                                r2[f"rgb_{typ}"] = r2[f"rgb_{typ}"] + r3[f"rgb_{typ}"]
                for typ in ("coarse", "fine"):
                    if f"rgb_{typ}" in r2:
                        r2[f"rgb_{typ}"] = r2[f"rgb_{typ}"] / (times + 1)
            r[f"rgb_{sel}"], refl = _blend(r[f"rgb_{sel}"], r2[f"rgb_{sel}"], index, mask, True)
            r[f"rgb_{sel}_reflect"] = refl
            if only_in:
                d = torch.zeros_like(r[f"depth_{sel}"])
                d[index.long()] = r2[f"depth_{sel}"]
                r[f"depth_{sel}_reflect"] = d
            else:
                r[f"depth_{sel}_reflect"] = r2[f"depth_{sel}"]
        return r

    results = defaultdict(list)
    stage_maps = to_cpu == "maps" and rays.is_cuda
    staged, staged_rows, hold = {}, defaultdict(int), []
    copy_stream = _copy_stream(rays.device) if stage_maps else None
    starts = list(range(0, rays.shape[0], chunk))
    pipelined = rays.is_cuda and not rough and len(starts) > 1 and os.environ.get("MNRF_EVAL_PIPELINE", "1") != "0"
    host_flags = torch.zeros(2, dtype=torch.int32).pin_memory() if pipelined else None
    ahead = stage_a(rays[:chunk].contiguous(), 0, host_flags, 0) if (pipelined and starts) else None
    for n_c, i in enumerate(starts):
        if pipelined:
            state = ahead
            ahead = stage_a(rays[starts[n_c + 1]:starts[n_c + 1] + chunk].contiguous(), 0, host_flags, (n_c + 1) % 2) \
                if n_c + 1 < len(starts) else None
            out = stage_b(state)
        else:
            out = recurse(rays[i:i + chunk].contiguous(), 0)
        if stage_maps:
            done = torch.cuda.Event()
            done.record()
            copy_stream.wait_event(done)
        for k, v in out.items():
            if to_cpu == "maps" or maps_only:
                if v.dim() <= 2 and (v.dim() == 1 or v.shape[1] <= 3):
                    if stage_maps:
                        buf = staged.get(k)
                        if buf is None:
                            buf = staged[k] = _pinned(k, rays.shape[0], tuple(v.shape[1:]), v.dtype)
                        r0 = staged_rows[k]
                        with torch.cuda.stream(copy_stream):
                            buf[r0:r0 + v.shape[0]].copy_(v, non_blocking=True)
                        staged_rows[k] = r0 + v.shape[0]
                        hold.append(v)
                    else:
                        results[k] += [v.to("cpu", non_blocking=True) if to_cpu == "maps" else (v.cpu() if to_cpu else v)]
            else:
                results[k] += [v.cpu() if to_cpu else v]
    if stage_maps:
        copy_stream.synchronize()
        hold.clear()
        for k, buf in staged.items():
            results[k] = [buf[:staged_rows[k]].clone()]
    elif to_cpu == "maps" and rays.is_cuda:
        torch.cuda.current_stream().synchronize()
    from .mirror_nerf import check_guard, release_transient
    guarded = list(models.values()) + (list(system_sub.models.values()) if system_sub is not None else []) + \
        (list(obj_models.values()) if obj_models is not None else [])
    if rays.shape[0] and not kwargs.get("_guard_retry") and check_guard(guarded):
        try:
            return batched_inference(models, embeddings, rays, N_samples, N_importance, use_disp, chunk,
                                     **dict(kwargs, _guard_retry=True))
        finally:
            release_transient(guarded)
    return {k: torch.cat(v, 0) for k, v in results.items()}
```

### mirror_nerf_amd/rendering.py

```python
import torch

from . import _lib
from .autograd import CompositeFn, EmbedFn, FieldFn
from .mirror_nerf import field_forward
from .weights import params_of

__all__ = ["render_rays", "sample_pdf"]

_LINSPACE = {}


def _linspace01(n, device):
    key = (n, str(device))
    t = _LINSPACE.get(key)
    if t is None:
        t = torch.linspace(0, 1, n).to(device)
        _LINSPACE[key] = t
    return t


def _n_freqs(emb):
    n = getattr(emb, "N_freqs", None)
    if n is None:
        raise RuntimeError("embeddings must expose N_freqs (Embedding modules)")
# ... 42 lines not shown
        for mdl in models.values():
            if (n_fx, n_fd) != (getattr(mdl, "n_freqs_xyz", 10), getattr(mdl, "n_freqs_dir", 4)):
                raise NotImplementedError(f"embeddings Embedding({n_fx}) / Embedding({n_fd}) do not match the model's "
                                          f"{getattr(mdl, 'in_channels_xyz', 63)} / {getattr(mdl, 'in_channels_dir', 27)} input channels")
        n_fd = 4
    f = lambda *s: torch.empty(*s, dtype=torch.float32, device=dev)

    train = torch.is_grad_enabled() and (rays.requires_grad or any(
        q.requires_grad for mdl in models.values() for q in params_of(mdl)))
    n_live = kwargs.get("_n_live")
    if n_live is not None and (not train or test_time):
        raise NotImplementedError("_n_live (device-side ray count) is a feature of the training path")

    comp_detach, cut_heads, keep_mirror = 0, 0, None
    if train:
        if kwargs.get("detach_density_for_mask_loss", False):
            comp_detach |= _lib.MNRF_DETACH_W_MASK
            cut_heads |= _lib.MNRF_CUT_MIRROR_HEAD
        elif kwargs.get("detach_density_outside_mirror_for_mask_loss", False) and kwargs.get("mirror_mask") is not None:
            mm = kwargs["mirror_mask"]
            gv = kwargs.get("_gt_valid")
            if (gv if gv is not None else not bool((mm < 0).any().item())):
                if mm.shape[0] != N or kwargs.get("_compacted"):
                    raise IndexError(f"detach_density_outside_mirror_for_mask_loss: mirror_mask has {mm.shape[0]} entries "
                                     f"for {N} rays (compacted reflected rays: use only_trace_rays_in_mirrors=False)")
                keep_mirror = mm.bool().float().contiguous()
        if kwargs.get("detach_density_for_normal_loss", False):
            comp_detach |= _lib.MNRF_DETACH_W_NORMAL
            cut_heads |= _lib.MNRF_CUT_NORMAL_HEAD

    fan = bool(train and not test_time and not hashgrid and N and N_samples >= 3 and "view_dir" not in kwargs and rays.shape[1] == 8)
    view = kwargs.get("view_dir", rays[:, 3:6])
    if fan:
        dir_emb = None
    elif hashgrid:
        dir_emb = view.float().contiguous()
    else:
        dir_emb = EmbedFn.apply(view, n_fd, n_live) if (train and view.requires_grad) else _embed(view.detach(), n_fd, n_live)

    z_steps = kwargs.get("_z_steps")
    z_steps = _linspace01(N_samples, dev) if z_steps is None else z_steps.float().contiguous()
    S_fine = N_samples + N_importance
    two_pass = train and N and N_importance > 0 and not kwargs.get("only_one_field", False) and kwargs.get("_z_fine") is None
    pool_u = pool_n = None
    share, box = kwargs.get("_rng_share") or (1, None)

    def pooled(kind, need, make):
        have = box.get(kind) if box is not None else None
        if have is None or have.numel() < need:
            have = make(need * (share if box is not None else 1))
        if box is not None:
            box[kind] = have[need:]
        return have[:need]
    if two_pass and perturb > 0 and kwargs.get("_perturb_rand") is None and kwargs.get("_u") is None:
        pool_u = pooled("u", N * (N_samples + N_importance), lambda k: torch.rand(k, device=dev))
    auto_noise = {}
    if two_pass and noise_std != 0 and kwargs.get("_noise_coarse") is None and kwargs.get("_noise_fine") is None:
        pool_n = pooled("n", N * (N_samples + S_fine), lambda k: torch.randn(k, device=dev))
        if noise_std != 1:
            pool_n = pool_n * noise_std
        auto_noise = {"_noise_coarse": pool_n[:N * N_samples].view(N, N_samples), "_noise_fine": pool_n[N * N_samples:].view(N, S_fine)}
    prand = None
    if perturb > 0:
        prand = kwargs.get("_perturb_rand")
        if prand is None:
            prand = pool_u[:N * N_samples].view(N, N_samples) if pool_u is not None else torch.rand(N, N_samples, device=dev)
        else:
            prand = prand.float().contiguous()
    per_pass = {}
    if fan:
        from .autograd import RayFanFn
        r_cf, r_ff, r_cc, r_fc, de_c, de_f, z_vals = RayFanFn.apply(rays, n_fd, z_steps, N_samples, bool(use_disp), float(perturb),
                                                                   prand, n_live)
        per_pass = {"_noise_coarse": (r_fc, r_cc, de_c), "_noise_fine": (r_ff, r_cf, de_f)}
    else:
        z_vals = f(N, N_samples)
        if N:
            _lib.check(L.mnrf_sample_coarse_n(p(rays), N, p(z_steps), N_samples, int(bool(use_disp)), float(perturb),
                                              p(prand), p(z_vals), p(n_live), _lib.stream()), "mnrf_sample_coarse")

    has_fine = "fine" in models
    results = {}

    def inference_fused(model, typ, z):
        from . import mirror_nerf as _mn
        from .weights import folded_of
        if _mn.precision_of(model) != "split" or z.shape[1] != L.mnrf_fused_samples_per_ray():
            return False
        rgb_depth = bool(kwargs.get("_rgb_depth_only"))
        has_m = not rgb_depth and getattr(model, "predict_mirror_mask", True)
        has_n = not rgb_depth and getattr(model, "predict_normal", True)
        opacity, rgb_map, depth = f(N), f(N, 3), f(N)
        xs = None if rgb_depth else f(N, 3)
        mask = f(N) if has_m else None
        sn = f(N, 3) if has_n else None
        flags = (_lib.MNRF_FUSED_WHITE_BACK if white_back else 0) | (_lib.MNRF_FUSED_RGB_DEPTH if rgb_depth else 0)
        if _mn.LAUNCH_LOG is not None:
            e0, e1 = torch.cuda.Event(enable_timing=True), torch.cuda.Event(enable_timing=True)
            e0.record()
        rc = L.mnrf_field_composite_fused(p(folded_of(model)), N, p(rays), p(z), p(dir_emb), dir_emb.shape[1], flags,
                                          None, p(opacity), p(rgb_map), p(depth), p(mask), p(sn), p(xs), _lib.stream())
        if rc == _lib.MNRF_ERR_UNSUPPORTED:
            return False
        _lib.check(rc, "mnrf_field_composite_fused")
        if _mn.LAUNCH_LOG is not None:
            e1.record()
            _mn.LAUNCH_LOG.append((_lib.MNRF_SPLIT_F16 | 0x2000 | (0x4000 if rgb_depth else 0), N * z.shape[1], e0, e1))
        results[f"opacity_{typ}"] = opacity
        results[f"z_vals_{typ}"] = z
        results[f"rgb_{typ}"] = rgb_map
        results[f"depth_{typ}"] = depth
        if has_m:
            results[f"mirror_mask_{typ}"] = mask
        if has_n:
            results[f"surface_normal_{typ}"] = sn
        if xs is not None:
            results[f"_x_surface_{typ}"] = xs
        return True

    def inference(model, typ, z, noise_key):
        S = z.shape[1]
        sigma_only = typ == "coarse" and test_time and has_fine
        B = N * S
        if train and not sigma_only and N:
            return inference_train(model, typ, z, noise_key)
        if (kwargs.get("_maps_only") and test_time and not sigma_only and N and not hashgrid and not compute_normal
                and noise_std == 0 and kwargs.get(noise_key) is None and inference_fused(model, typ, z)):
            return
        if N and hashgrid:
            o = model.field(B, rays=rays, z_vals=z, spr=S, dirs=dir_emb, sigma_only=sigma_only,
                            grad_normal=compute_normal and not sigma_only)
        elif N:
            o = field_forward(model, B, rays=rays, z_vals=z, spr=S, dir_emb=dir_emb, dir_stride=dir_emb.shape[1],
                              sigma_only=sigma_only, grad_normal=compute_normal and not sigma_only)
        else:
            o = {"sigma": f(0)}
            if not sigma_only:
                o["rgb"] = f(0, 3)
                if getattr(model, "predict_normal", True):
                    o["pred_normal"] = f(0, 3)
                if getattr(model, "predict_mirror_mask", True):
                    o["is_mirror"] = f(0)
                if compute_normal:
                    o["normal"] = f(0, 3)
        noise = kwargs.get(noise_key)
        if noise is not None:
            noise = (noise.float() * noise_std).contiguous()
        elif noise_std != 0:
            noise = torch.randn(N, S, device=dev)
            if noise_std != 1:
                noise = noise * noise_std
        weights, opacity = f(N, S), f(N)
        full = not sigma_only
        has_m, has_n = full and "is_mirror" in o, full and "pred_normal" in o
        rgb_map = f(N, 3) if full else None
        depth = f(N) if full else None
        mask = f(N) if has_m else None
        sn = f(N, 3) if has_n else None
        sng = f(N, 3) if (full and compute_normal) else None
        nd = f(N) if (has_n and compute_normal) else None
        xs = f(N, 3) if full else None
        if N:
            _lib.check(L.mnrf_composite(
                p(rays), N, S, p(o["sigma"]), p(z), p(noise), p(o.get("rgb")), p(o.get("is_mirror")),
                p(o.get("pred_normal")), p(o.get("normal")) if full else None, int(bool(white_back)),
                p(weights), p(opacity), p(rgb_map), p(depth), p(mask), p(sn), p(sng), p(nd), p(xs),
                _lib.stream()), "mnrf_composite")
        results[f"weights_{typ}"] = weights
        results[f"opacity_{typ}"] = opacity
        results[f"z_vals_{typ}"] = z
        if sigma_only:
            return
        results[f"rgb_{typ}"] = rgb_map
        results[f"depth_{typ}"] = depth
        if has_m:
            results[f"mirror_mask_{typ}"] = mask
        if compute_normal:
            results[f"normal_{typ}"] = o["normal"].view(N, S, 3)
            results[f"surface_normal_grad_{typ}"] = sng
        if has_n:
            results[f"pred_normal_{typ}"] = o["pred_normal"].view(N, S, 3)
            results[f"surface_normal_{typ}"] = sn
        if compute_normal and has_n:
            results[f"normal_dif_{typ}"] = nd
        results[f"_x_surface_{typ}"] = xs

    def inference_train(model, typ, z, noise_key):
        S = z.shape[1]
        rays_f, rays_c, dir_emb_p = per_pass.get(noise_key, (rays, rays, dir_emb))
        if hashgrid:
            from .mirror_nerf_tcnn import TcnnFieldFn
            want = bool(compute_normal)
            if cut_heads or keep_mirror is not None or n_live is not None:
                want = (want, cut_heads, keep_mirror, n_live)
            sigma, rgb, pn, mir, normal, _geo = TcnnFieldFn.apply(model, S, None, rays, z, dir_emb, want,
                                                                  model.encoder.embeddings, *model.mlp_params())
        else:
            want = bool(compute_normal)
            if cut_heads or keep_mirror is not None or n_live is not None:
                want = (want, cut_heads, keep_mirror, n_live)
            sigma, rgb, pn, mir, normal = FieldFn.apply(model, S, None, rays_f, z, dir_emb_p, want, *params_of(model))
        noise = kwargs.get(noise_key)
        if noise is not None:
            noise = (noise.float() * noise_std).contiguous()
        elif noise_key in auto_noise and auto_noise[noise_key].shape == (N, S):
            noise = auto_noise[noise_key]
        elif noise_std != 0:
            noise = torch.randn(N, S, device=dev)
            if noise_std != 1:
                noise = noise * noise_std
# ... 80 lines not shown
```

Measured before the change: 1.905 million.

## Add blended-level fused composite that decides per ray from mirror weight

Adds a fused field+composite mode for intermediate recursion levels. The mirror head is evaluated first and its composited mask decides per ray; colour GEMM work is skipped (fill pointer jumps) for rays that do not need it. Mirror-head weights are folded into a new packed region, and the sample weights are kept in LDS so the final composite can reuse them. On the host side the mirror fraction is tracked per level, and the mode is enabled automatically above a break-even fraction. This adds complexity, an extra host sync for counting, and a heuristic threshold.

```diff
diff --git a/include/mnrf.h b/include/mnrf.h
--- a/include/mnrf.h
+++ b/include/mnrf.h
@@ -175,11 +175,16 @@
 
 #define MNRF_FUSED_WHITE_BACK 1u
 #define MNRF_FUSED_RGB_DEPTH 2u
+#define MNRF_FUSED_BLENDED_LEVEL 8u
 int mnrf_fused_samples_per_ray(void);
 int mnrf_field_composite_fused(float* packed, int64_t n_rays, const float* rays, const float* z_vals,
                                const float* dir_emb, int64_t dir_stride, int flags,
                                float* weights, float* opacity, float* rgb_map, float* depth, float* mirror_mask,
                                float* surf_normal, float* x_surface, void* stream);
+int mnrf_field_composite_fused_pn(float* packed, int64_t n_rays, const float* rays, const float* z_vals,
+                                  const float* dir_emb, int64_t dir_stride, int flags,
+                                  float* weights, float* opacity, float* rgb_map, float* depth, float* mirror_mask,
+                                  float* surf_normal, float* x_surface, float* pred_normal, void* stream);
 
 #define MNRF_TRAIN_PLANES 256u
 #define MNRF_PLANES_Y_HALF 0x100000u
diff --git a/mirror_nerf_amd/csrc/mnrf_composite.inc b/mirror_nerf_amd/csrc/mnrf_composite.inc
--- a/mirror_nerf_amd/csrc/mnrf_composite.inc
+++ b/mirror_nerf_amd/csrc/mnrf_composite.inc
@@ -7,6 +7,49 @@
 };
 
 template <class Src>
+__device__ __forceinline__ float composite_weight(const Src& src, int S, int s, bool in, int lane, float& carry, float& zv) {
+    float alpha = 0.f;
+    zv = 0.f;
+    if (in) {
+        zv = src.z(s);
+        const float delta = s + 1 < S ? src.z(s + 1) - zv : 1e10f;
+        float sv = src.sigma(s);
+        if (src.has_noise()) sv = sv + src.noise(s);
+        alpha = 1.f - expf(-delta * fmaxf(sv, 0.f));
+    }
+    const float t = in ? (1.f - alpha) + 1e-10f : 1.f;
+    float incl = t;
+#pragma unroll
+    for (int o = 1; o < 64; o <<= 1) {
+        const float up = __shfl_up(incl, o);
+        if (lane >= o) incl *= up;
+    }
+    float excl = __shfl_up(incl, 1);
+    if (lane == 0) excl = 1.f;
+    const float w = alpha * (carry * excl);
+    carry = carry * __shfl(incl, 63);
+    return w;
+}
+
+template <class Src>
+__device__ __forceinline__ float composite_mirror_value(const Src& src, int S, int lane, float* w_keep) {
+    float carry = 1.f;
+    float a_m = 0.f;
+#pragma unroll
+    for (int base = 0; base < S; base += 64) {
+        const int s = base + lane;
+        const bool in = s < S;
+        float zv;
+        const float w = composite_weight(src, S, s, in, lane, carry, zv);
+        if (in) {
+            if (w_keep) w_keep[s] = w;
+            a_m += w * src.mirror(s);
+        }
+    }
+    return wave_sum(a_m);
+}
+
+template <class Src>
 __device__ __forceinline__ void composite_ray(const Src& src, int S, int lane, long long ray, const CompMaps& A) {
     float carry = 1.f;
     float a_op = 0.f, a_d = 0.f, a_m = 0.f, a_nd = 0.f;
@@ -14,25 +57,13 @@
     for (int base = 0; base < S; base += 64) {
         const int s = base + lane;
         const bool in = s < S;
-        float alpha = 0.f, zv = 0.f;
-        if (in) {
-            zv = src.z(s);
-            const float delta = s + 1 < S ? src.z(s + 1) - zv : 1e10f;
-            float sv = src.sigma(s);
-            if (src.has_noise()) sv = sv + src.noise(s);
-            alpha = 1.f - expf(-delta * fmaxf(sv, 0.f));
+        float zv, w;
+        if (src.has_w()) {
+            zv = in ? src.z(s) : 0.f;
+            w = in ? src.w(s) : 0.f;
+        } else {
+            w = composite_weight(src, S, s, in, lane, carry, zv);
         }
-        const float t = in ? (1.f - alpha) + 1e-10f : 1.f;
-        float incl = t;
-#pragma unroll
-        for (int o = 1; o < 64; o <<= 1) {
-            const float up = __shfl_up(incl, o);
-            if (lane >= o) incl *= up;
-        }
-        float excl = __shfl_up(incl, 1);
-        if (lane == 0) excl = 1.f;
-        const float w = alpha * (carry * excl);
-        carry = carry * __shfl(incl, 63);
         if (in) {
             if (A.weights) A.weights[s] = w;
             a_op += w;
diff --git a/mirror_nerf_amd/csrc/mnrf_field.hip b/mirror_nerf_amd/csrc/mnrf_field.hip
--- a/mirror_nerf_amd/csrc/mnrf_field.hip
+++ b/mirror_nerf_amd/csrc/mnrf_field.hip
@@ -1,5 +1,6 @@
 #include <hip/hip_runtime.h>
 #include <stdint.h>
+#include <stdio.h>
 #include <stdlib.h>
 
 #include "mnrf_layout.h"
@@ -181,29 +182,53 @@
 
 extern "C" int mnrf_fused_samples_per_ray(void) { return split48_ray_samples(); }
 
+static int composite_fused(const char* who, float* packed, int64_t n_rays, const float* rays, const float* z_vals,
+                           const float* dir_emb, int64_t dir_stride, int flags,
+                           float* weights, float* opacity, float* rgb_map, float* depth, float* mirror_mask,
+                           float* surf_normal, float* x_surface, float* pred_normal, void* stream) {
+    const auto fail = [&](int code, const char* what) {
+        static thread_local char msg[256];
+        snprintf(msg, sizeof msg, "%s: %s", who, what);
+        return mnrf_fail(code, msg);
+    };
+    if (!packed || !rays || !z_vals || !dir_emb) return fail(MNRF_ERR_ARG, "null pointer");
+    if (n_rays < 0) return fail(MNRF_ERR_ARG, "negative ray count");
+    if (flags & ~(int)(MNRF_FUSED_WHITE_BACK | MNRF_FUSED_RGB_DEPTH | MNRF_FUSED_BLENDED_LEVEL)) return fail(MNRF_ERR_ARG, "unknown flag bits");
+    const bool rgb_depth = flags & MNRF_FUSED_RGB_DEPTH;
+    const bool blended = flags & MNRF_FUSED_BLENDED_LEVEL;
+    if (rgb_depth && (mirror_mask || surf_normal || pred_normal))
+        return fail(MNRF_ERR_ARG, "MNRF_FUSED_RGB_DEPTH evaluates neither the mirror head nor the normal map");
+    if (blended && rgb_depth)
+        return fail(MNRF_ERR_ARG, "MNRF_FUSED_BLENDED_LEVEL decides from the mirror head, which MNRF_FUSED_RGB_DEPTH does not evaluate");
+    if (blended && !mirror_mask)
+        return fail(MNRF_ERR_ARG, "MNRF_FUSED_BLENDED_LEVEL needs the mirror_mask output: the caller blends with it");
+    if (n_rays == 0) return MNRF_OK;
+    if (!split48_enabled()) return fail(MNRF_ERR_UNSUPPORTED, "needs the 48-samples-per-wave tuning (MNRF_SPLIT48 != 0)");
+    const int spr = split48_ray_samples();
+    FieldArgs A{packed, MNRF_SPLIT_F16, (long long)n_rays * spr, nullptr, 3, rays, z_vals, spr, dir_emb, (long long)dir_stride,
+                nullptr, nullptr, pred_normal, nullptr, nullptr, nullptr};
+    A.fuse = rgb_depth ? 2 : blended ? 3 : pred_normal ? 4 : 1;
+    A.white_back = (flags & MNRF_FUSED_WHITE_BACK) != 0;
+    A.f_weights = weights; A.f_opacity = opacity; A.f_rgb_map = rgb_map; A.f_depth = depth; A.f_mirror_mask = mirror_mask;
+    A.f_surf_normal = surf_normal; A.f_x_surface = x_surface;
+    if (launch_split48(A, false, (hipStream_t)stream) != 0) return fail(MNRF_ERR_ARG, "too many samples for one launch");
+    return mnrf_check_launch(who);
+}
+
 extern "C" int mnrf_field_composite_fused(float* packed, int64_t n_rays, const float* rays, const float* z_vals,
                                           const float* dir_emb, int64_t dir_stride, int flags,
                                           float* weights, float* opacity, float* rgb_map, float* depth, float* mirror_mask,
                                           float* surf_normal, float* x_surface, void* stream) {
-    if (!packed || !rays || !z_vals || !dir_emb) return mnrf_fail(MNRF_ERR_ARG, "mnrf_field_composite_fused: null pointer");
-    if (n_rays < 0) return mnrf_fail(MNRF_ERR_ARG, "mnrf_field_composite_fused: negative ray count");
-    if (flags & ~(int)(MNRF_FUSED_WHITE_BACK | MNRF_FUSED_RGB_DEPTH)) return mnrf_fail(MNRF_ERR_ARG, "mnrf_field_composite_fused: unknown flag bits");
-    const bool rgb_depth = flags & MNRF_FUSED_RGB_DEPTH;
-    if (rgb_depth && (mirror_mask || surf_normal))
-        return mnrf_fail(MNRF_ERR_ARG, "mnrf_field_composite_fused: MNRF_FUSED_RGB_DEPTH evaluates neither the mirror head nor the normal map");
-    if (n_rays == 0) return MNRF_OK;
-    if (!split48_enabled())
-        return mnrf_fail(MNRF_ERR_UNSUPPORTED, "mnrf_field_composite_fused: needs the 48-samples-per-wave tuning (MNRF_SPLIT48 != 0)");
-    const int spr = split48_ray_samples();
-    FieldArgs A{packed, MNRF_SPLIT_F16, (long long)n_rays * spr, nullptr, 3, rays, z_vals, spr, dir_emb, (long long)dir_stride,
-                nullptr, nullptr, nullptr, nullptr, nullptr, nullptr};
-    A.fuse = rgb_depth ? 2 : 1;
-    A.white_back = (flags & MNRF_FUSED_WHITE_BACK) != 0;
-    A.f_weights = weights; A.f_opacity = opacity; A.f_rgb_map = rgb_map; A.f_depth = depth; A.f_mirror_mask = mirror_mask;
-    A.f_surf_normal = surf_normal; A.f_x_surface = x_surface;
-    if (launch_split48(A, false, (hipStream_t)stream) != 0)
-        return mnrf_fail(MNRF_ERR_ARG, "mnrf_field_composite_fused: too many samples for one launch");
-    return mnrf_check_launch("mnrf_field_composite_fused");
+    return composite_fused("mnrf_field_composite_fused", packed, n_rays, rays, z_vals, dir_emb, dir_stride, flags, weights, opacity,
+                           rgb_map, depth, mirror_mask, surf_normal, x_surface, nullptr, stream);
+}
+
+extern "C" int mnrf_field_composite_fused_pn(float* packed, int64_t n_rays, const float* rays, const float* z_vals,
+                                             const float* dir_emb, int64_t dir_stride, int flags,
+                                             float* weights, float* opacity, float* rgb_map, float* depth, float* mirror_mask,
+                                             float* surf_normal, float* x_surface, float* pred_normal, void* stream) {
+    return composite_fused("mnrf_field_composite_fused_pn", packed, n_rays, rays, z_vals, dir_emb, dir_stride, flags, weights, opacity,
+                           rgb_map, depth, mirror_mask, surf_normal, x_surface, pred_normal, stream);
 }
 
 static inline int64_t train_tiles(int64_t B) { return (B + s2::WG_SAMPLES - 1) / s2::WG_SAMPLES; }
diff --git a/mirror_nerf_amd/csrc/mnrf_field_split.hip b/mirror_nerf_amd/csrc/mnrf_field_split.hip
--- a/mirror_nerf_amd/csrc/mnrf_field_split.hip
+++ b/mirror_nerf_amd/csrc/mnrf_field_split.hip
@@ -120,7 +120,22 @@
     float* packed = I.packed[blockIdx.y];
     const long long q = (long long)blockIdx.x * blockDim.x + threadIdx.x;
     constexpr long long FOLD_LANES = (long long)SPLIT_FOLD_PAIRS * 64;
-    if (q >= FOLD_LANES + BIAS_FLOATS) return;
+    if (q >= FOLD_LANES + BIAS_FLOATS + (long long)FOLD_MIRB_PAIRS * 64) return;
+    if (q >= FOLD_LANES + BIAS_FLOATS) {
+        const int j = (int)((q - FOLD_LANES - BIAS_FLOATS) >> 6), l = (int)(q & 63);
+        typedef _Float16 h8c __attribute__((ext_vector_type(8)));
+        h8c hi, lo;
+        for (int e = 0; e < 8; ++e) hi[e] = lo[e] = (_Float16)0.f;
+        if (j < 64 + 4) {
+            const char* src = (const char*)(packed + OFF_SPLIT_FWD) + (long long)(1036 + j) * PAIR_BYTES + l * 16;
+            hi = *(const h8c*)src;
+            lo = *(const h8c*)(src + PAIR_BYTES / 2);
+        }
+        char* dst = (char*)(packed + OFF_FOLD_FWD) + (long long)(FOLD_POS_MIRB + j) * PAIR_BYTES + l * 16;
+        *(h8c*)dst = hi;
+        *(h8c*)(dst + PAIR_BYTES / 2) = lo;
+        return;
+    }
     const float* bias = packed + OFF_BIAS;
     if (q >= FOLD_LANES) {
         const int b = (int)(q - FOLD_LANES);
@@ -198,7 +213,7 @@
         I.wn1[m] = p[24];
         I.wn2[m] = p[26];
     }
-    const long long n = (long long)SPLIT_FOLD_PAIRS * 64 + BIAS_FLOATS;
+    const long long n = (long long)SPLIT_FOLD_PAIRS * 64 + BIAS_FLOATS + (long long)FOLD_MIRB_PAIRS * 64;
     hipLaunchKernelGGL(split_fold_kernel, dim3((unsigned)((n + 255) / 256), n_images), dim3(256), 0, s, I);
 }
 
diff --git a/mirror_nerf_amd/csrc/mnrf_field_split.inc b/mirror_nerf_amd/csrc/mnrf_field_split.inc
--- a/mirror_nerf_amd/csrc/mnrf_field_split.inc
+++ b/mirror_nerf_amd/csrc/mnrf_field_split.inc
@@ -33,7 +33,7 @@
 constexpr int LDS_BYTES_GRAD = LDS_MASK + 8 * S * WG_THREADS * 8;
 static_assert(LDS_BYTES_GRAD <= 160 * 1024, "LDS budget");
 constexpr int LDS_FUSE = LDS_BYTES;
-constexpr int LDS_BYTES_FUSE = LDS_BYTES + 9 * WG_SAMPLES * 4;
+constexpr int LDS_BYTES_FUSE = LDS_BYTES + 10 * WG_SAMPLES * 4;
 static_assert(LDS_BYTES_FUSE <= 160 * 1024, "LDS budget");
 
 #include "mnrf_field_split_common.inc"
@@ -47,6 +47,8 @@
 struct CompLdsSrc {
     const float* f;
     bool pn_on, mir_on;
+    __device__ __forceinline__ bool has_w() const { return false; }
+    __device__ __forceinline__ float w(int) const { return 0.f; }
     __device__ __forceinline__ bool has_noise() const { return false; }
     __device__ __forceinline__ bool has_rgb() const { return true; }
     __device__ __forceinline__ bool has_mirror() const { return mir_on; }
@@ -60,6 +62,12 @@
     __device__ __forceinline__ float pn(int s, int k) const { return f[(4 + k) * WG_SAMPLES + s]; }
     __device__ __forceinline__ float gn(int, int) const { return 0.f; }
 };
+struct CompLdsSrcBlended : CompLdsSrc {
+    bool colour;
+    __device__ __forceinline__ bool has_rgb() const { return colour; }
+    __device__ __forceinline__ bool has_w() const { return true; }
+    __device__ __forceinline__ float w(int s) const { return f[9 * WG_SAMPLES + s]; }
+};
 struct CompLdsSrcRgbDepth : CompLdsSrc {
     __device__ __forceinline__ bool has_mirror() const { return false; }
     __device__ __forceinline__ bool has_pn() const { return false; }
@@ -119,11 +127,13 @@
 }
 
 template <int NT, int NB, int NACC, int NTA, int JOB, bool WANT_MASK, int USTART, int TPU, int POS, int NPARK = 0, int STB = -1,
-          int STN = 4, bool SSCALE = false>
+          int STN = 4, bool SSCALE = false, int JUMP_T = -1, long long JUMP = 0, bool SKIP = false>
 __device__ __forceinline__ void gemm_part_impl(f32x4 (&acc)[S][NACC], const u32x4 (&bh)[S][NTA], const u32x4 (&bl)[S][NTA],
                                                Stream& st, int wave, int lane16, const f32x4 (&pacc)[S][8],
                                                u32x4 (&oh)[S][8], u32x4 (&ol)[S][8], int t0, int half, uint64_t (&mk)[S],
-                                               const StoreCtx& sc = StoreCtx{}) {
+                                               const StoreCtx& sc = StoreCtx{}, bool jump_on = true) {
+    static_assert(JUMP == 0 || (JUMP_T >= 0 && JUMP_T % U == 0 && JUMP_T < NT * NB && ((POS + JUMP_T) / U) % PIECES == PIECES - 1 && JUMP % CHUNK_BYTES == 0),
+                  "the fill pointer jumps between two chunks");
     static_assert(STB < 0 || (S == 2 && NT * NB / U >= 8 * STN && STB + STN <= NTA), "8 store tasks per operand ride on the part's first units");
     static_assert(NT <= NTA, "B operand count");
     static_assert(JOB < 0 || NTASKS % TPU == 0, "tasks per unit");
@@ -184,7 +194,7 @@
             for (int s = 0; s < S; ++s) {
                 const u32x4& a = ph == 1 ? al[(t + u) % NBUF] : ah[(t + u) % NBUF];
                 const u32x4& b = ph == 2 ? (T < NPARK ? pk[T % NSLOT][s] : bl[s][T]) : bh[s][T];
-                acc[s][nb] = mfma_f16(a, b, acc[s][nb]);
+                if (!SKIP) acc[s][nb] = mfma_f16(a, b, acc[s][nb]);
             }
             if (JOB >= 0 && (sg == 0 || sg == 2) && TPU == 2) {
                 const int unit = t / U - USTART;
@@ -251,6 +261,7 @@
                     else if (piece == 5) issue_piece<(PIECES == 8 ? 5 : 0)>(st);
                     else if (piece == 6) issue_piece<(PIECES == 8 ? 6 : 0)>(st);
                     else issue_piece<(PIECES == 8 ? 7 : 0)>(st);
+                    if (JUMP != 0 && t == JUMP_T) st.fill_src += jump_on ? (unsigned long long)JUMP : 0ull;
                 }
                 __builtin_amdgcn_sched_barrier(0);
             }
@@ -261,21 +272,31 @@
     if (JOB >= 0) sat_flush(st.sat, st.tmax);
 }
 
-template <int NT, int NB, int POS, int NPARK = 0, int STB = -1, int STN = 4, bool SSCALE = false, int NACC, int NTA>
+template <int NT, int NB, int POS, int NPARK = 0, int STB = -1, int STN = 4, bool SSCALE = false, int JUMP_T = -1, long long JUMP = 0,
+          int NACC, int NTA>
 __device__ __forceinline__ void gemm_part(f32x4 (&acc)[S][NACC], const u32x4 (&bh)[S][NTA], const u32x4 (&bl)[S][NTA],
                                           Stream& st, int wave, int lane16, const StoreCtx& sc = StoreCtx{}) {
     f32x4 pacc[S][8];
     u32x4 oh[S][8], ol[S][8];
     uint64_t mk[S];
-    gemm_part_impl<NT, NB, NACC, NTA, -1, false, 0, S, POS, NPARK, STB, STN, SSCALE>(acc, bh, bl, st, wave, lane16, pacc, oh, ol, 0, 0,
-                                                                                      mk, sc);
-}
-
-template <int NT, int NTA, bool WANT_MASK, int USTART, int TPU, int POS, int STB = -1>
+    gemm_part_impl<NT, NB, NACC, NTA, -1, false, 0, S, POS, NPARK, STB, STN, SSCALE, JUMP_T, JUMP>(acc, bh, bl, st, wave, lane16, pacc,
+                                                                                                  oh, ol, 0, 0, mk, sc);
+}
+
+template <int POS>
+__device__ __forceinline__ void skip_pairs4(Stream& st, int wave, int lane16) {
+    f32x4 acc[S][1], pacc[S][8];
+    u32x4 b[S][4], oh[S][8], ol[S][8];
+    uint64_t mk[S];
+    gemm_part_impl<4, 1, 1, 4, -1, false, 0, S, POS, 0, -1, 4, false, -1, 0, true>(acc, b, b, st, wave, lane16, pacc, oh, ol, 0, 0, mk);
+}
+
+template <int NT, int NTA, bool WANT_MASK, int USTART, int TPU, int POS, int STB = -1, int JUMP_T = -1, long long JUMP = 0>
 __device__ __forceinline__ void gemm_half(f32x4 (&acc)[S][8], const u32x4 (&bh)[S][NTA], const u32x4 (&bl)[S][NTA], Stream& st,
                                           int wave, int lane16, const f32x4 (&pacc)[S][8], u32x4 (&hh)[S][8], u32x4 (&hl)[S][8],
-                                          int t0, int half, uint64_t (&mk)[S], const StoreCtx& sc = StoreCtx{}) {
-    gemm_part_impl<NT, 8, 8, NTA, 1, WANT_MASK, USTART, TPU, POS, 0, STB>(acc, bh, bl, st, wave, lane16, pacc, hh, hl, t0, half, mk, sc);
+                                          int t0, int half, uint64_t (&mk)[S], const StoreCtx& sc = StoreCtx{}, bool jump_on = true) {
+    gemm_part_impl<NT, 8, 8, NTA, 1, WANT_MASK, USTART, TPU, POS, 0, STB, 4, false, JUMP_T, JUMP>(acc, bh, bl, st, wave, lane16, pacc, hh,
+                                                                                                 hl, t0, half, mk, sc, jump_on);
 }
 
 template <bool WANT_MASK>
@@ -430,11 +451,15 @@
 
 
 
-template <bool SIGMA_ONLY, bool GRAD, bool PLANES, bool FUSE, bool RGB_DEPTH>
+template <bool SIGMA_ONLY, bool GRAD, bool PLANES, bool FUSE, bool RGB_DEPTH, bool BLENDED = false>
 __device__ __forceinline__ void field_split_body(FieldArgs A) {
     static_assert(!PLANES || (GRAD && !SIGMA_ONLY && S == 2), "operand planes: the training forward (32 samples per wave)");
     static_assert(!FUSE || (S == 3 && !SIGMA_ONLY && !GRAD), "ray-fused compositing: the 192-sample fine pass");
     static_assert(!RGB_DEPTH || FUSE, "rgb / depth only: a variant of the ray-fused pass");
+    static_assert(!BLENDED || (FUSE && !RGB_DEPTH && CHUNK_PAIRS == 8), "blended level: a variant of the ray-fused pass; its jumps are whole 8-pair chunks");
+    constexpr long long JUMP_TO_MIRB = BLENDED ? (long long)(FOLD_POS_MIRB - FOLD_POS_DIR) * PAIR_BYTES : 0;
+    constexpr long long JUMP_FROM_MIRB = BLENDED ? (long long)(FOLD_POS_DIR - (FOLD_POS_MIRB + FOLD_MIRB_PAIRS)) * PAIR_BYTES : 0;
+    constexpr int JT = BLENDED ? 54 : -1;
     constexpr bool FOLD = !SIGMA_ONLY && !GRAD;
     float* const fz = (float*)(smem + LDS_FUSE);
     constexpr bool PERSIST = S == 3;
@@ -667,7 +692,7 @@
             if (keep) save_acc<8, 1>(A.save_x + (long long)(SEC_H + 256 * (5 + l)) * A.B, 256, 0, accA, idx, valid, g, unused_bits);
             if constexpr (S == 2 && !WEAVE) { if (pl) store_planes<8, 8>(sc, SEC_H / 16 + 16 * (4 + l), hh, hl); }
             init_bias_half(accB, BIAS_L + 256 * (5 + l), 1, gq());
-            gemm_half<8, 8, GRAD, 4, S, 640, ST4>(accB, hh, hl, st, wave, lane16, accA, hh, hl, 0, 0, mk, at_h(4 + l, 4));
+            gemm_half<8, 8, GRAD, 4, S, 640, ST4, JT, JUMP_TO_MIRB>(accB, hh, hl, st, wave, lane16, accA, hh, hl, 0, 0, mk, at_h(4 + l, 4), l == 2);
             if (keep) save_acc<8, 1>(A.save_x + (long long)(SEC_H + 256 * (5 + l)) * A.B, 256, 8, accB, idx, valid, g, unused_bits);
         }
         conv_half<GRAD>(accB, hh, hl, 4, 1, mk, st.sat);
@@ -704,6 +729,12 @@
                     const float inv = 1.f / sqrtf(fmaxf(a0 * a0 + a1 * a1 + a2 * a2, 1.1920928955078125e-07f));
                     const int q = wave * (S * 16) + s * 16 + (int)m15();
                     fz[4 * WG_SAMPLES + q] = a0 * inv; fz[5 * WG_SAMPLES + q] = a1 * inv; fz[6 * WG_SAMPLES + q] = a2 * inv;
+                    if constexpr (BLENDED) {
+                        if (A.pred_normal && sval(s)) {
+                            float* o = A.pred_normal + (long long)sidx(s) * 3;
+                            out_store(o, a0 * inv); out_store(o + 1, a1 * inv); out_store(o + 2, a2 * inv);
+                        }
+                    }
                 }
             }
         } else if (A.pred_normal && g == 0) {
@@ -736,6 +767,7 @@
         if constexpr (FOLD && !RGB_DEPTH) put_normal(acc, std::integral_constant<int, 1>{});
     }
 
+    bool colour = true;
     if (!SIGMA_ONLY) {
         if constexpr (!FOLD) {
             u32x4 nh[S][4], nl[S][4];
@@ -757,7 +789,7 @@
             {
                 f32x4 acc[S][8];
                 init_bias<8>(acc, BIAS_MIR1, gq());
-                gemm_part<8, 8, FOLD ? FOLD_POS_MIR1 : 1036, HP, ST4>(acc, hh, hl, st, wave, lane16, at_h(7, 4));
+                gemm_part<8, 8, BLENDED ? 968 : FOLD ? FOLD_POS_MIR1 : 1036, HP, ST4, 4, false, JT, JUMP_FROM_MIRB>(acc, hh, hl, st, wave, lane16, at_h(7, 4));
                 if (keep) {
                     uint64_t bits[S];
                     save_acc<8, 2>(A.save_x + (long long)SEC_HM * A.B, 128, 0, acc, idx, valid, g, bits);
@@ -771,7 +803,7 @@
             }
             f32x4 acc[S][1];
             init_bias<1>(acc, BIAS_MIR2, gq());
-            gemm_part<4, 1, FOLD ? FOLD_POS_MIR2 : 1100>(acc, mh, ml, st, wave, lane16);
+            gemm_part<4, 1, BLENDED ? 1032 : FOLD ? FOLD_POS_MIR2 : 1100>(acc, mh, ml, st, wave, lane16);
             if (FUSE) {
                 if (gq() == 0) {
 #pragma unroll
@@ -784,6 +816,17 @@
             }
         };
         if constexpr (!FOLD) mirror_head();
+        if constexpr (BLENDED) {
+            mirror_head();
+            skip_pairs4<1036>(st, wave, lane16);
+            asm volatile("s_waitcnt lgkmcnt(0)" ::: "memory");
+            __builtin_amdgcn_s_barrier();
+            asm volatile("" ::: "memory");
+            int dl;
+            asm volatile("v_mbcnt_lo_u32_b32 %0, -1, 0\n\tv_mbcnt_hi_u32_b32 %0, -1, %0" : "=v"(dl));
+            const float mv = composite_mirror_value(CompLdsSrc{fz, false, true}, WG_SAMPLES, dl, wave == 0 ? fz + 9 * WG_SAMPLES : nullptr);
+            colour = __builtin_amdgcn_readfirstlane((int)(mv < 0.5f)) != 0 || A.fuse == 4;
+        }
         const auto view_operands = [&](u32x4 (&vh)[S][1], u32x4 (&vl)[S][1]) {
             float de[S][8];
             const int gv = gq();
@@ -801,15 +844,15 @@
             split_b<8>(de, vh, vl, st.sat);
             if constexpr (S == 2) { if (pl) store_planes<1, 1>(sc, SEC_DIRE / 16, vh, vl); }
         };
-        {
+        if (colour) {
             u32x4 dh[S][4], dl[S][4];
             if constexpr (FOLD) {
                 u32x4 vh[S][1], vl[S][1];
                 view_operands(vh, vl);
                 f32x4 acc[S][8];
                 init_bias<8>(acc, BIAS_DIR, gq());
-                gemm_part<8, 8, FOLD_POS_DIR, HP>(acc, hh, hl, st, wave, lane16);
-                gemm_part<1, 8, FOLD_POS_VIEW>(acc, vh, vl, st, wave, lane16);
+                gemm_part<8, 8, BLENDED ? 1040 : FOLD_POS_DIR, HP>(acc, hh, hl, st, wave, lane16);
+                gemm_part<1, 8, BLENDED ? 1104 : FOLD_POS_VIEW>(acc, vh, vl, st, wave, lane16);
                 acc_to_b<8, 1, false>(dh, dl, acc, 0, tid, st.sat);
             } else {
                 u32x4 fh[S][8], fl[S][8];
@@ -840,7 +883,7 @@
             }
             f32x4 acc[S][1];
             init_bias<1>(acc, BIAS_RGB, gq());
-            gemm_part<4, 1, FOLD ? FOLD_POS_RGB : 1304>(acc, dh, dl, st, wave, lane16);
+            gemm_part<4, 1, BLENDED ? 1112 : FOLD ? FOLD_POS_RGB : 1304>(acc, dh, dl, st, wave, lane16);
             if (FUSE) {
                 if (gq() == 0) {
 #pragma unroll
@@ -862,7 +905,7 @@
                     }
             }
         }
-        if constexpr (FOLD && !RGB_DEPTH) mirror_head();
+        if constexpr (FOLD && !RGB_DEPTH && !BLENDED) mirror_head();
     }
 
     if (GRAD) {
@@ -969,6 +1012,12 @@
                 const CompMaps out{A.f_weights ? A.f_weights + ray * WG_SAMPLES : nullptr, A.f_opacity, A.f_rgb_map, A.f_depth, nullptr,
                                    nullptr, nullptr, nullptr, A.f_x_surface, A.rays, A.white_back};
                 composite_ray(CompLdsSrcRgbDepth{fz, false, false}, WG_SAMPLES, cl, ray, out);
+            } else if constexpr (BLENDED) {
+                const CompLdsSrcBlended src{{fz, A.f_surf_normal != nullptr, A.f_mirror_mask != nullptr}, colour};
+                const CompMaps out{A.f_weights ? A.f_weights + ray * WG_SAMPLES : nullptr, A.f_opacity, colour ? A.f_rgb_map : nullptr, A.f_depth,
+                                   A.f_mirror_mask, A.f_surf_normal, nullptr, nullptr, A.f_x_surface, A.rays, A.white_back};
+                composite_ray(src, WG_SAMPLES, cl, ray, out);
+                if (!colour && A.f_rgb_map && cl < 3) A.f_rgb_map[ray * 3 + cl] = 0.f;
             } else {
                 const CompLdsSrc src{fz, A.f_surf_normal != nullptr, A.f_mirror_mask != nullptr};
                 const CompMaps out{A.f_weights ? A.f_weights + ray * WG_SAMPLES : nullptr, A.f_opacity, A.f_rgb_map, A.f_depth, A.f_mirror_mask,
@@ -1003,6 +1052,11 @@
 template <bool ON = true>
 __global__ __launch_bounds__(WG_THREADS, MIN_WAVES_PER_SIMD) void field_split_kernel_rgb_depth(FieldArgs A) {
     field_split_body<false, false, false, ON, ON>(A);
+}
+
+template <bool ON = true>
+__global__ __launch_bounds__(WG_THREADS, MIN_WAVES_PER_SIMD) void field_split_kernel_blended(FieldArgs A) {
+    field_split_body<false, false, false, ON, false, ON>(A);
 }
 
 template <bool UNUSED = false>
@@ -1018,6 +1072,8 @@
     if (sigma_only && !grad) hipLaunchKernelGGL((field_split_kernel<true, false>), grid, block, LDS_BYTES, s, A);
     else if (!sigma_only && !grad && S == 3 && A.fuse == 2) {
         if constexpr (S == 3) hipLaunchKernelGGL((field_split_kernel_rgb_depth<>), grid, block, LDS_BYTES_FUSE, s, A);
+    } else if (!sigma_only && !grad && S == 3 && A.fuse >= 3) {
+        if constexpr (S == 3) hipLaunchKernelGGL((field_split_kernel_blended<>), grid, block, LDS_BYTES_FUSE, s, A);
     } else if (!sigma_only && !grad && S == 3 && A.fuse)
         hipLaunchKernelGGL((field_split_kernel<false, false, false, S == 3>), grid, block, LDS_BYTES_FUSE, s, A);
     else if (!sigma_only && !grad) hipLaunchKernelGGL((field_split_kernel<false, false>), grid, block, LDS_BYTES, s, A);
diff --git a/mirror_nerf_amd/csrc/mnrf_field_split3.hip b/mirror_nerf_amd/csrc/mnrf_field_split3.hip
--- a/mirror_nerf_amd/csrc/mnrf_field_split3.hip
+++ b/mirror_nerf_amd/csrc/mnrf_field_split3.hip
@@ -59,6 +59,7 @@
         (void)hipFuncSetAttribute((const void*)h3::field_split_kernel<false, false, false, true>, hipFuncAttributeMaxDynamicSharedMemorySize,
                                    h3::LDS_BYTES_FUSE);
         (void)hipFuncSetAttribute((const void*)h3::field_split_kernel_rgb_depth<>, hipFuncAttributeMaxDynamicSharedMemorySize, h3::LDS_BYTES_FUSE);
+        (void)hipFuncSetAttribute((const void*)h3::field_split_kernel_blended<>, hipFuncAttributeMaxDynamicSharedMemorySize, h3::LDS_BYTES_FUSE);
         return true;
     }();
     (void)once;
diff --git a/mirror_nerf_amd/csrc/mnrf_layout.h b/mirror_nerf_amd/csrc/mnrf_layout.h
--- a/mirror_nerf_amd/csrc/mnrf_layout.h
+++ b/mirror_nerf_amd/csrc/mnrf_layout.h
@@ -91,6 +91,11 @@
 constexpr int64_t OFF_FOLD_FWD = OFF_SPLIT_HBWD + (int64_t)SPLIT_HBWD_PAIRS * (PAIR_BYTES / 4);
 constexpr int64_t OFF_FOLD_BIAS = OFF_FOLD_FWD + (int64_t)SPLIT_FOLD_PAIRS * (PAIR_BYTES / 4) + SPLIT_TAIL_FLOATS;
 constexpr int64_t PACKED_FLOATS = OFF_FOLD_FWD + (int64_t)FOLD_REGION_PAIRS * (PAIR_BYTES / 4) + SPLIT_TAIL_FLOATS;
+constexpr int FOLD_MIRB_PAIRS = 64 + 4 + 4;
+constexpr int FOLD_POS_MIRB = 1160;
+static_assert(FOLD_POS_MIRB % 8 == 0 && FOLD_MIRB_PAIRS % 8 == 0 && FOLD_POS_DIR % 8 == 0, "the copy is whole chunks of the 48-sample tuning");
+static_assert(OFF_FOLD_FWD + (int64_t)FOLD_POS_MIRB * (PAIR_BYTES / 4) >= OFF_FOLD_BIAS + BIAS_FLOATS, "the copy lies behind the folded bias block");
+static_assert(FOLD_POS_MIRB + FOLD_MIRB_PAIRS <= FOLD_REGION_PAIRS, "the copy fits the reserved region");
 constexpr int TQ_PAIRS = 8;
 constexpr int64_t OFF_TILE_QUEUE = PACKED_FLOATS - 1 - 2 * TQ_PAIRS;
 constexpr int64_t OFF_REDUCE_PAIR = OFF_TILE_QUEUE - 2;
diff --git a/mirror_nerf_amd/csrc/mnrf_render.hip b/mirror_nerf_amd/csrc/mnrf_render.hip
--- a/mirror_nerf_amd/csrc/mnrf_render.hip
+++ b/mirror_nerf_amd/csrc/mnrf_render.hip
@@ -96,6 +96,8 @@
 struct CompGlobalSrc {
     const CompArgs& A;
     long long ray;
+    __device__ __forceinline__ bool has_w() const { return false; }
+    __device__ __forceinline__ float w(int) const { return 0.f; }
     __device__ __forceinline__ bool has_noise() const { return A.noise != nullptr; }
     __device__ __forceinline__ bool has_rgb() const { return A.rgb != nullptr; }
     __device__ __forceinline__ bool has_mirror() const { return A.is_mirror != nullptr; }
diff --git a/mirror_nerf_amd/recursion.py b/mirror_nerf_amd/recursion.py
--- a/mirror_nerf_amd/recursion.py
+++ b/mirror_nerf_amd/recursion.py
@@ -1,6 +1,7 @@
 import ctypes
 import os
 from collections import defaultdict
+import weakref
 from types import SimpleNamespace
 
 import torch
@@ -12,6 +13,8 @@
 from .rendering import render_rays
 
 RAY_FORWARD_OFFSET = 0.1
+BLENDED_BREAK_EVEN = 0.37
+_MIRROR_FRACTION = weakref.WeakKeyDictionary()
 JITTER_RAYS = 262144
 
 PLACE_MIRROR_PRESETS = {
@@ -604,6 +607,10 @@
     one_field = getattr(args, "only_one_field", False)
     fine_epoch = getattr(args, "only_one_field_fine_epoch", 2)
     sel = "fine" if (N_importance > 0 and not one_field) else "coarse"
+    blend_mode = kwargs.get("blended_level", "auto")
+    if blend_mode not in (True, False, "auto"):
+        raise ValueError(f"blended_level must be True, False or 'auto', not {blend_mode!r}")
+    mirror_fraction = _MIRROR_FRACTION.setdefault(models.get(sel, models["coarse"]), {})
 
     def draw(n, dev):
         if noise_iter is not None:
@@ -612,12 +619,17 @@
 
     def stage_a(rays_chunk, level, host_flags=None, slot=0):
         rgb_depth = 1 <= level == args.max_recursive_level and not rough
+        can_blend = bool(level < args.max_recursive_level and trace_flag and test_time and blend_mode is not False
+                         and not (rough or place or subst or objects))
+        evidence = mirror_fraction.get(level)
+        blended = can_blend and (blend_mode is True or (evidence is not None and evidence >= BLENDED_BREAK_EVEN))
+        count_it = can_blend and blend_mode is not True
         r = render_rays(models, embeddings, rays_chunk, N_samples, use_disp, 0, 0, N_importance, chunk,
                         white_back, test_time=test_time,
                         compute_normal=trace_flag and (not args.predict_normal),
                         only_one_field=one_field, only_one_field_fine_epoch=fine_epoch,
                         current_epoch=fine_epoch + 1, _guard=False, _maps_only=maps_only or rgb_depth,
-                        _rgb_depth_only=rgb_depth)
+                        _rgb_depth_only=rgb_depth, _blended_level=blended)
         r[f"rgb_{sel}_reflect"] = torch.zeros_like(r[f"rgb_{sel}"])
         r[f"depth_{sel}_reflect"] = torch.zeros_like(r[f"depth_{sel}"])
         if objects:
@@ -631,13 +643,21 @@
         edit = None
         if place and not last:
             edit = lambda flag: _place_mirror(r, rays_chunk, sel, plane, args.near, flag)
-        pending, any_mirror = None, False
+        pending, any_mirror, counted = None, False, None
         if mask is not None:
             if host_flags is not None and not last and rays_chunk.shape[0]:
                 pending = _threshold_async(mask, host_flags, slot, edit)
+                if count_it:
+                    host = host_counts[slot:slot + 1]
+                    host.copy_(torch.count_nonzero(mask).view(1), non_blocking=True)
+                    ev = torch.cuda.Event()
+                    ev.record()
+                    counted = (host, ev)
             else:
                 any_mirror = _threshold_(mask, want_any=not last, edit=edit)
-        return r, rays_chunk, level, mask, any_mirror, pending
+                if count_it and rays_chunk.shape[0]:
+                    mirror_fraction[level] = (int(torch.count_nonzero(mask).item()) if any_mirror else 0) / rays_chunk.shape[0]
+        return r, rays_chunk, level, mask, any_mirror, pending, counted
 
     def render_object(obj_rays):
         if obj_dnerf is not None:
@@ -652,9 +672,12 @@
         return stage_b(stage_a(rays_chunk, level))
 
     def stage_b(state):
-        r, rays_chunk, level, mask, any_mirror, pending = state
+        r, rays_chunk, level, mask, any_mirror, pending, counted = state
         if pending is not None:
             any_mirror = _flag_ready(pending)
+        if counted is not None:
+            counted[1].synchronize()
+            mirror_fraction[level] = int(counted[0].item()) / rays_chunk.shape[0]
         N = rays_chunk.shape[0]
         dev = rays_chunk.device
         only_in = not (level < 1)
@@ -720,6 +743,7 @@
     starts = list(range(0, rays.shape[0], chunk))
     pipelined = rays.is_cuda and not rough and len(starts) > 1 and os.environ.get("MNRF_EVAL_PIPELINE", "1") != "0"
     host_flags = torch.zeros(2, dtype=torch.int32).pin_memory() if pipelined else None
+    host_counts = torch.zeros(2, dtype=torch.int64).pin_memory() if pipelined else None
     ahead = stage_a(rays[:chunk].contiguous(), 0, host_flags, 0) if (pipelined and starts) else None
     for n_c, i in enumerate(starts):
         if pipelined:
diff --git a/mirror_nerf_amd/rendering.py b/mirror_nerf_amd/rendering.py
--- a/mirror_nerf_amd/rendering.py
+++ b/mirror_nerf_amd/rendering.py
@@ -148,11 +148,13 @@
     has_fine = "fine" in models
     results = {}
 
-    def inference_fused(model, typ, z):
+    def inference_fused(model, typ, z, blended=False):
         from . import mirror_nerf as _mn
         from .weights import folded_of
         if _mn.precision_of(model) != "split" or z.shape[1] != L.mnrf_fused_samples_per_ray():
             return False
+        if blended:
+            return inference_fused_blended(model, typ, z)
         rgb_depth = bool(kwargs.get("_rgb_depth_only"))
         has_m = not rgb_depth and getattr(model, "predict_mirror_mask", True)
         has_n = not rgb_depth and getattr(model, "predict_normal", True)
@@ -184,14 +186,56 @@
             results[f"_x_surface_{typ}"] = xs
         return True
 
+    def inference_fused_blended(model, typ, z):
+        from . import mirror_nerf as _mn
+        from .weights import folded_of
+        if not getattr(model, "predict_mirror_mask", True):
+            return False
+        S = z.shape[1]
+        has_n = getattr(model, "predict_normal", True)
+        per_sample = not kwargs.get("_maps_only")
+        opacity, rgb_map, depth, xs, mask = f(N), f(N, 3), f(N), f(N, 3), f(N)
+        sn = f(N, 3) if has_n else None
+        weights = f(N, S) if per_sample else None
+        pn = f(N, S, 3) if (per_sample and has_n) else None
+        flags = (_lib.MNRF_FUSED_WHITE_BACK if white_back else 0) | _lib.MNRF_FUSED_BLENDED_LEVEL
+        if _mn.LAUNCH_LOG is not None:
+            e0, e1 = torch.cuda.Event(enable_timing=True), torch.cuda.Event(enable_timing=True)
+            e0.record()
+        rc = L.mnrf_field_composite_fused_pn(p(folded_of(model)), N, p(rays), p(z), p(dir_emb), dir_emb.shape[1], flags,
+                                             p(weights), p(opacity), p(rgb_map), p(depth), p(mask), p(sn), p(xs), p(pn),
+                                             _lib.stream())
+        if rc == _lib.MNRF_ERR_UNSUPPORTED:
+            return False
+        _lib.check(rc, "mnrf_field_composite_fused_pn")
+        if _mn.LAUNCH_LOG is not None:
+            e1.record()
+            _mn.LAUNCH_LOG.append((_lib.MNRF_SPLIT_F16 | 0x2000 | 0x8000, N * S, e0, e1))
+        if weights is not None:
+            results[f"weights_{typ}"] = weights
+        results[f"opacity_{typ}"] = opacity
+        results[f"z_vals_{typ}"] = z
+        results[f"rgb_{typ}"] = rgb_map
+        results[f"depth_{typ}"] = depth
+        results[f"mirror_mask_{typ}"] = mask
+        if pn is not None:
+            results[f"pred_normal_{typ}"] = pn
+        if has_n:
+            results[f"surface_normal_{typ}"] = sn
+        results[f"_x_surface_{typ}"] = xs
+        return True
+
     def inference(model, typ, z, noise_key):
         S = z.shape[1]
         sigma_only = typ == "coarse" and test_time and has_fine
         B = N * S
         if train and not sigma_only and N:
             return inference_train(model, typ, z, noise_key)
-        if (kwargs.get("_maps_only") and test_time and not sigma_only and N and not hashgrid and not compute_normal
-                and noise_std == 0 and kwargs.get(noise_key) is None and inference_fused(model, typ, z)):
+        fusable = (test_time and not sigma_only and N and not hashgrid and not compute_normal and noise_std == 0
+                   and kwargs.get(noise_key) is None)
+        if fusable and kwargs.get("_blended_level") and inference_fused(model, typ, z, blended=True):
+            return
+        if kwargs.get("_maps_only") and fusable and inference_fused(model, typ, z):
             return
         if N and hashgrid:
             o = model.field(B, rays=rays, z_vals=z, spr=S, dirs=dir_emb, sigma_only=sigma_only,
```

After: 1.948 million, median of 6. +2.2%, better.
